# Maknee/minigpt4.cpp

Measured on AMD Instinct MI355X. Metric: decode tokens/sec, higher is better.
Workload: dtype i8; 1 GPU; MiniGPT4-13B f16 vision + Vicuna-13B Q5_K_M (wv/w2 Q6_K in 'more-bits' layers, output Q6_K), batch 1 per GPU, greedy decode through the C ABI; n_ctx=2048, context_at_mid_run=646, parallelism=dp1 (independent replicas)

## Files before the change

minigpt4.cpp_amd/csrc/attn_llm_body.hpp:

```cpp
    static_assert((FUSED || !BATCHED) && (BATCHED || !DRAFT), "BATCHED implies FUSED, DRAFT implies BATCHED");
    extern __shared__ __attribute__((aligned(16))) unsigned char smem[];
    constexpr int CH = HD / 8, P = AT_THREADS / CH, RM = DRAFT ? DRAFT_ROWS : 1;
    static_assert(!DRAFT || (RM <= P && RM * (HD / 2) <= AT_THREADS), "one prologue thread per (row, rotated pair); at most one LDS key per partition");
    const int h = blockIdx.x, t = blockIdx.y, tid = threadIdx.x;
    int pos_, p0_ = 0;
    if (BATCHED) {
        const int slot = row_slot[DRAFT ? 0 : t];
        p0_ = n_past[slot]; pos_ = DRAFT ? p0_ + t : p0_;
        if (DRAFT && pos_ >= n_ctx) return;
        kc += (size_t)slot * seq_stride; vc += (size_t)slot * seq_stride;
    } else pos_ = *n_past + t;
    const int pos = pos_, p0 = p0_, T = pos + 1;
    const int Tg = FUSED ? pos : T;
    const int Tpad = (T + 7) & ~7;
    float *sc = reinterpret_cast<float *>(smem);
    __half *ph = reinterpret_cast<__half *>(sc + Tpad);
    __half *qh = ph + Tpad;
    __half *knew = qh + HD, *vnew = knew + RM * HD;
    float *part = reinterpret_cast<float *>(vnew + RM * HD);
    __shared__ float s_red[AT_THREADS / 64];
    __shared__ double s_dred[AT_THREADS / 64];
    const float scale = 1.0f / sqrtf((float)HD);
    const size_t qo = (size_t)t * E + (size_t)h * HD;
    if (FUSED) {
        if (DRAFT) {
            if (tid < (t + 1) * (HD / 2)) {
                const int r = tid / (HD / 2), i = tid % (HD / 2), pr = p0 + r;
                const size_t ro = (size_t)r * E + (size_t)h * HD;
                const float c = cos_tab[(size_t)pr * (HD / 2) + i], s = sin_tab[(size_t)pr * (HD / 2) + i];
                const __half2 kr = rope_rot_h2(kin[ro + 2 * i], kin[ro + 2 * i + 1], c, s);
                const __half2 vr = __floats2half2_rn(vin[ro + 2 * i], vin[ro + 2 * i + 1]);
                st_h2(knew + r * HD + 2 * i, kr); st_h2(vnew + r * HD + 2 * i, vr);
                if (r == t) {
                    st_h2(qh + 2 * i, rope_rot_h2(q[qo + 2 * i], q[qo + 2 * i + 1], c, s));
                    const size_t co = (size_t)pos * E + (size_t)h * HD + 2 * i;
                    st_h2(kc + co, kr); st_h2(vc + co, vr);
                }
            }
        } else if (tid < HD / 2) {
            const int i = tid;
            const float c = cos_tab[(size_t)pos * (HD / 2) + i], s = sin_tab[(size_t)pos * (HD / 2) + i];
            const __half2 qr = rope_rot_h2(q[qo + 2 * i], q[qo + 2 * i + 1], c, s), kr = rope_rot_h2(kin[qo + 2 * i], kin[qo + 2 * i + 1], c, s);
            const __half2 vr = __floats2half2_rn(vin[qo + 2 * i], vin[qo + 2 * i + 1]);
            st_h2(qh + 2 * i, qr); st_h2(knew + 2 * i, kr); st_h2(vnew + 2 * i, vr);
            const size_t co = (size_t)pos * E + (size_t)h * HD + 2 * i;
            st_h2(kc + co, kr); st_h2(vc + co, vr);
        }
    } else {
        for (int i = tid; i < HD; i += AT_THREADS) qh[i] = f2h_rn(q[qo + i]);
    }
    __syncthreads();
    unsigned qreg[HD / 2];
#pragma unroll
    for (int i = 0; i < HD / 8; i++) { const int4 v4 = *reinterpret_cast<const int4 *>(qh + 8 * i); qreg[4 * i] = (unsigned)v4.x; qreg[4 * i + 1] = (unsigned)v4.y; qreg[4 * i + 2] = (unsigned)v4.z; qreg[4 * i + 3] = (unsigned)v4.w; }
    auto dot_row = [&](const __half *kr) {
        int4 kk[HD / 8];
#pragma unroll
        for (int i = 0; i < HD / 8; i++) kk[i] = ld16(kr + 8 * i);
        float s = 0.0f;
#pragma unroll
        for (int i = 0; i < HD / 8; i++) {
            const unsigned w[4] = {(unsigned)kk[i].x, (unsigned)kk[i].y, (unsigned)kk[i].z, (unsigned)kk[i].w};
#pragma unroll
            for (int e = 0; e < 4; e++) { s = fmaf(h2f_bits(w[e] & 0xFFFF), h2f_bits(qreg[4 * i + e] & 0xFFFF), s); s = fmaf(h2f_bits(w[e] >> 16), h2f_bits(qreg[4 * i + e] >> 16), s); }
        }
        return s * scale;
    };
    const int c = tid % CH, p = tid / CH;
    const __half *kb = kc + (size_t)h * HD + 8 * c, *vb = vc + (size_t)h * HD + 8 * c;
    constexpr int NPRE = 16;
    const int gmax = DRAFT ? max(p0 - 1, 0) : 0;
    int4 kpre[NPRE], vpre[NPRE];
#pragma unroll
    for (int i = 0; i < NPRE; i++) kpre[i] = ld16(kb + (size_t)min(p + i * P, DRAFT ? gmax : max(Tg - 1, 0)) * E);
#pragma unroll
    for (int i = 0; i < NPRE; i++) vpre[i] = ld16(vb + (size_t)min(p + i * P, DRAFT ? gmax : max(Tg - 1, 0)) * E);
    int jl = -1;
    int4 kl = make_int4(0, 0, 0, 0), vl = kl;
    if (DRAFT) {
        const int rl = (p - p0) & (P - 1);
        jl = rl < t ? p0 + rl : -1;
        kl = *reinterpret_cast<const int4 *>(knew + min(rl, RM - 1) * HD + 8 * c); vl = *reinterpret_cast<const int4 *>(vnew + min(rl, RM - 1) * HD + 8 * c);
    }
    float qd[8];
    unpack8(*reinterpret_cast<const int4 *>(qh + 8 * c), qd);
    float mx = -INFINITY;
#pragma unroll
    for (int i = 0; i < NPRE; i++) { const int j = p + i * P; const float s = dot16<CH>(DRAFT && j == jl ? kl : kpre[i], qd, scale); if (j < Tg) { if (c == 0) sc[j] = s; mx = fmaxf(mx, s); } }
    for (int j0 = p + NPRE * P; j0 < Tg; j0 += 8 * P) {
        int4 kk[8];
#pragma unroll
        for (int i = 0; i < 8; i++) kk[i] = ld16(kb + (size_t)min(j0 + i * P, DRAFT ? gmax : Tg - 1) * E);
#pragma unroll
        for (int i = 0; i < 8; i++) { const int j = j0 + i * P; const float s = dot16<CH>(DRAFT && j == jl ? kl : kk[i], qd, scale); if (j < Tg) { if (c == 0) sc[j] = s; mx = fmaxf(mx, s); } }
    }
    if (FUSED && tid == AT_THREADS - 1) { const float s = dot_row(knew + (DRAFT ? t : 0) * HD); sc[pos] = s; mx = fmaxf(mx, s); }
    mx = wave_max(mx);
    if ((tid & 63) == 0) s_red[tid >> 6] = mx;
    __syncthreads();
    mx = s_red[0];
#pragma unroll
    for (int i = 1; i < AT_THREADS / 64; i++) mx = fmaxf(mx, s_red[i]);
    double sum = 0.0;
    for (int j = tid; j < T; j += AT_THREADS) { const float v = exp_h(tb.exp, sc[j] - mx); sc[j] = v; sum += (double)v; }
    sum = wave_sum_d(sum);
    if ((tid & 63) == 0) s_dred[tid >> 6] = sum;
    __syncthreads();
    double tot = 0.0;
#pragma unroll
    for (int i = 0; i < AT_THREADS / 64; i++) tot += s_dred[i];
    const float inv = (float)(1.0 / tot);
    for (int j = tid; j < T; j += AT_THREADS) ph[j] = f2h_rn(sc[j] * inv);
    __syncthreads();
    float o[8] = {0, 0, 0, 0, 0, 0, 0, 0};
    auto pv_key = [&](const int4 &vv, const int j) { pv_acc(o, vv, __half2float(ph[j])); };
#pragma unroll
    for (int i = 0; i < NPRE; i++) { const int j = p + i * P; if (j < Tg) pv_key(DRAFT && j == jl ? vl : vpre[i], j); }
    for (int j0 = p + NPRE * P; j0 < Tg; j0 += 8 * P) {
        int4 vv[8];
#pragma unroll
        for (int i = 0; i < 8; i++) vv[i] = ld16(vb + (size_t)min(j0 + i * P, DRAFT ? gmax : Tg - 1) * E);
#pragma unroll
        for (int i = 0; i < 8; i++) { const int j = j0 + i * P; if (j < Tg) pv_key(DRAFT && j == jl ? vl : vv[i], j); }
    }
    if (FUSED && p == P - 1) {
        const float pj = __half2float(ph[pos]);
#pragma unroll
        for (int e = 0; e < 8; e++) o[e] = fmaf(__half2float(vnew[(DRAFT ? t : 0) * HD + 8 * c + e]), pj, o[e]);
    }
#pragma unroll
    for (int e = 0; e < 8; e++) part[p * HD + 8 * c + e] = o[e];
    __syncthreads();
    for (int i = tid; i < HD; i += AT_THREADS) { float s = 0.0f;
#pragma unroll 8
        for (int pp = 0; pp < P; pp++) s += part[pp * HD + i];
        out[qo + i] = s; }
```

minigpt4.cpp_amd/csrc/engine.cpp:

```cpp
#include "engine.hpp"
#include "dist.hpp"
#include "draft.hpp"
#include "quantize.hpp"
#include "imageio.hpp"

#include <algorithm>
#include <optional>
#include <unistd.h>
#include <chrono>
#include <thread>
#include <cmath>
#include <cstring>

namespace mg4 {

int device_count_noexcept() {
    int n = 0;
    if (hipGetDeviceCount(&n) != hipSuccess) { (void)hipGetLastError(); return 0; }
    return n;
}
void DeviceArena::alloc(size_t bytes) {
    release();
    if (virt) base = reinterpret_cast<uint8_t *>((uintptr_t)1 << 40);
    else { HIP_CHECK(hipMalloc((void **)&base, bytes)); HIP_CHECK(hipMemset(base, 0, bytes)); HIP_CHECK(hipDeviceSynchronize()); }
    cap = bytes; used = 0; layout_hash = 1469598103934665603ull;
}
void DeviceArena::release() { if (base && !virt) HIP_IGNORE(hipFree(base)); base = nullptr; cap = used = 0; }
uint8_t *DeviceArena::take(size_t bytes, size_t align) {
    const size_t off = (used + align - 1) / align * align;
    if (off + bytes > cap) throw HipError{hipErrorOutOfMemory, "arena overflow", __FILE__, __LINE__};
    used = off + bytes;
    for (uint64_t v : {(uint64_t)off, (uint64_t)bytes}) for (int i = 0; i < 8; i++) { layout_hash ^= (v >> (8 * i)) & 0xFF; layout_hash *= 1099511628211ull; }
    return base + off;
}
template <typename T> T *Engine::upload_raw(DeviceArena &a, const void *src, size_t bytes) {
    uint8_t *d = a.take(bytes);
    if (moves_data()) HIP_CHECK(hipMemcpy(d, src, bytes, hipMemcpyHostToDevice));
    return reinterpret_cast<T *>(d);
}

void preprocess_image_device(hipStream_t s, const uint8_t *rgb, int w, int h, float *out_chw) {
    constexpr int OUT = 224;
    const float mean[3] = {(float)0.48145466, (float)0.4578275, (float)0.40821073}, sd[3] = {(float)0.26862954, (float)0.26130258, (float)0.27577711};
    auto table = [&](int in, ResampleCoeffs &c) {
        if (in != OUT) { precompute_bicubic_8bpc(in, OUT, c); return; }
        c.in_size = c.out_size = OUT; c.ksize = 1; c.first.resize(OUT); c.count.assign(OUT, 1); c.kk.assign(OUT, 1 << 22);
        for (int i = 0; i < OUT; i++) c.first[(size_t)i] = i;
    };
    ResampleCoeffs ch, cv;
    table(w, ch); table(h, cv);
    struct Dev { void *p = nullptr; ~Dev() { if (p) HIP_IGNORE(hipFree(p)); } };
    Dev d_src, d_tmp, d_out, d_tab;
    const size_t src_bytes = (size_t)w * h * 3, tmp_bytes = (size_t)h * OUT * 3, out_bytes = (size_t)3 * OUT * OUT * 4;
    std::vector<int> tab;
    tab.insert(tab.end(), ch.first.begin(), ch.first.end()); tab.insert(tab.end(), ch.count.begin(), ch.count.end()); tab.insert(tab.end(), ch.kk.begin(), ch.kk.end());
    const size_t voff = tab.size();
    tab.insert(tab.end(), cv.first.begin(), cv.first.end()); tab.insert(tab.end(), cv.count.begin(), cv.count.end()); tab.insert(tab.end(), cv.kk.begin(), cv.kk.end());
    HIP_CHECK(hipMalloc(&d_src.p, src_bytes)); HIP_CHECK(hipMalloc(&d_tmp.p, tmp_bytes)); HIP_CHECK(hipMalloc(&d_out.p, out_bytes)); HIP_CHECK(hipMalloc(&d_tab.p, tab.size() * 4));
    HIP_CHECK(hipMemcpyAsync(d_src.p, rgb, src_bytes, hipMemcpyHostToDevice, s));
    HIP_CHECK(hipMemcpyAsync(d_tab.p, tab.data(), tab.size() * 4, hipMemcpyHostToDevice, s));
    const int *t = static_cast<const int *>(d_tab.p);
    launch_resample_h(static_cast<const uint8_t *>(d_src.p), w, h, t, t + OUT, t + 2 * OUT, ch.ksize, static_cast<uint8_t *>(d_tmp.p), OUT, s);
    launch_resample_v_norm(static_cast<const uint8_t *>(d_tmp.p), OUT, t + voff, t + voff + OUT, t + voff + 2 * OUT, cv.ksize, static_cast<float *>(d_out.p), OUT, mean, sd, s);
    HIP_CHECK(hipMemcpyAsync(out_chw, d_out.p, out_bytes, hipMemcpyDeviceToHost, s));
    HIP_CHECK(hipStreamSynchronize(s));
}

void Engine::release_buffers() {
    for (Conversation &c : conv_) { if (c.graph) HIP_IGNORE(hipGraphExecDestroy(c.graph)); c.graph = nullptr; }
    for (hipGraphExec_t &g : batch_graph_) { if (g) HIP_IGNORE(hipGraphExecDestroy(g)); g = nullptr; }
    spec_drop_graphs();
    if (h_argmax_) HIP_IGNORE(hipHostFree(h_argmax_));
    if (h_bstage_) HIP_IGNORE(hipHostFree(h_bstage_));
    if (h_logits_) HIP_IGNORE(hipHostFree(h_logits_));
    if (h_seg_) HIP_IGNORE(hipHostFree(h_seg_));
    h_argmax_ = nullptr; h_bstage_ = nullptr; h_logits_ = nullptr; h_seg_ = nullptr; logits_host_slot_ = -1;
    buf_arena_.release();
}
Engine::~Engine() {
    if (trace_file_) { fclose(trace_file_); trace_file_ = nullptr; }
    if (stream_hung_) {
        llm_arena_.abandon(); vis_arena_.abandon(); buf_arena_.abandon(); ri_arena_.abandon(); vgen_arena_.abandon();
        return;
    }
    if (stream_) HIP_IGNORE(hipStreamSynchronize(stream_));
    for (auto &e : site_events_) { HIP_IGNORE(hipEventDestroy(e.a)); HIP_IGNORE(hipEventDestroy(e.b)); }
    if (stage_) HIP_IGNORE(hipFree(stage_));
    prefix_free();
    score_free();
    topn_free();
    pen_free();
    spec_free();
    release_buffers();
    if (stream_) HIP_IGNORE(hipStreamDestroy(stream_));
}
void Engine::sync() { (void)flush(); HIP_CHECK(hipStreamSynchronize(stream_)); }

int Engine::init(const std::string &vision_path, const std::string &llm_path, int seed, int n_ctx, int n_batch) {
    const int ndev = device_count_noexcept();
    if (ndev <= 0) { set_last_error("no HIP device visible: the MI355X engine has no CPU fallback"); MG4_ERR("%s", last_error().c_str()); return E_LoadLanguageModel; }
    DistEnv dist; { std::string derr; if (parse_dist_env(dist, derr)) { set_last_error(derr); MG4_ERR("%s", derr.c_str()); return E_LoadLanguageModel; } }
    const char *dv = getenv("MINIGPT4_DEVICE");
    if (!dv) dv = getenv("LOCAL_RANK");
    device_ = dv ? atoi(dv) % ndev : (dist.active() && dist.world > 1 ? dist.rank % ndev : 0);
    if (!dv && dist.active() && dist.world > 1) MG4_INFO("no MINIGPT4_DEVICE / LOCAL_RANK: rank %d takes device %d", dist.rank, device_);
    HIP_CHECK(hipSetDevice(device_));
    hipDeviceProp_t prop;
    HIP_CHECK(hipGetDeviceProperties(&prop, device_));
    MG4_INFO("device %d: %s (%s), %d CUs, %.1f GiB", device_, prop.name, prop.gcnArchName, prop.multiProcessorCount, prop.totalGlobalMem / 1073741824.0);
    if (strncmp(prop.gcnArchName, "gfx950", 6) != 0) {
        set_last_error(std::string("device ") + prop.gcnArchName + " is not gfx950 (MI355X): this library carries gfx950 code objects only"); MG4_ERR("%s", last_error().c_str());
        return E_LoadLanguageModel;
    }
    HIP_CHECK(hipStreamCreateWithFlags(&stream_, hipStreamNonBlocking));
    n_ctx_ = n_ctx > 0 ? n_ctx : 2048;
    n_batch_ = n_batch > 0 ? n_batch : 512;
    max_rows_ = std::max(n_batch_, 32);
    use_graph_ = !(getenv("MINIGPT4_NO_GRAPH") && atoi(getenv("MINIGPT4_NO_GRAPH")));
    max_chunk_ = max_rows_;
    if (getenv("MINIGPT4_ATTN_PREFILL_W8")) set_attn_prefill_w8(atoi(getenv("MINIGPT4_ATTN_PREFILL_W8")));
    if (const char *dc = getenv("MINIGPT4_DEFER_COMBINE")) defer_combine_ = atoi(dc) != 0;
    if (const char *fp = getenv("MINIGPT4_F16_PAIR")) f16_pair_ = atoi(fp);
    batch_mix_ = !(getenv("MINIGPT4_BATCH_MIX") && atoi(getenv("MINIGPT4_BATCH_MIX")) == 0);
    if (const char *e = getenv("MINIGPT4_ATTN_SPLIT_T")) attn_split_t_ = atoi(e);
    n_cus_ = prop.multiProcessorCount;
    if (const char *e = getenv("MINIGPT4_MMQH")) set_mmqh(atoi(e));
    if (const char *e = getenv("MINIGPT4_COMPUTED_TABLES")) computed_tables_ = atoi(e) != 0;
    if (const char *e = getenv("MINIGPT4_RI_FUSE")) ri_fuse_ = atoi(e) != 0;
    if (const char *e = getenv("MINIGPT4_RI_W2")) ri_w2_ = atoi(e) != 0;
    if (const char *e = getenv("MINIGPT4_RI_WO")) ri_wo_ = atoi(e) != 0;
    if (const char *e = getenv("MINIGPT4_RI")) use_ri_ = atoi(e) != 0;
    set_ri_cus(prop.multiProcessorCount);
    if (const char *e = getenv("MINIGPT4_QF_FOLD")) qf_fold_ = atoi(e) != 0;
    if (const char *e = getenv("MINIGPT4_ATTN_QT")) set_attn_vit_qt(atoi(e));
    if (const char *e = getenv("MINIGPT4_SPLITK_XCD")) set_gemm_splitk_xcd(atoi(e));
    if (const char *e = getenv("MINIGPT4_SPLITK_PROJ")) splitk_proj_ = std::max(1, std::min(SPLITK_MAX, atoi(e)));
    if (const char *e = getenv("MINIGPT4_SPLITK_FC2")) splitk_fc2_ = std::max(1, std::min(SPLITK_MAX, atoi(e)));
    if (const char *e = getenv("MINIGPT4_FUSE")) fuse_mask_ = atoi(e);
    if (const char *e = getenv("MINIGPT4_F16_KS")) set_gemm_tuning(-1, atoi(e));
    if (const char *e = getenv("MINIGPT4_PAIR_SILU_COMPUTED")) pair_silu_computed_ = atoi(e) != 0;
    if (const char *e = getenv("MINIGPT4_COMPUTED_GELU")) computed_gelu_ = atoi(e) != 0;
    if (const char *e = getenv("MINIGPT4_QKV_HEAD_MAJOR")) qkv_head_major_ = atoi(e) != 0;
    if (const char *e = getenv("MINIGPT4_QF_SPLITK")) qf_splitk_ = atoi(e) != 0;
    if (const char *e = getenv("MINIGPT4_KV_HOIST")) kv_hoist_ = atoi(e) != 0;
    set_matvec_tuning(0, 0, prop.multiProcessorCount);
    if (const char *ns = getenv("MINIGPT4_CONVERSATIONS")) conv_.assign((size_t)std::max(1, std::min(MAX_CONVERSATIONS, atoi(ns))), Conversation{});
    sampler_.seed(seed);
    if (const char *tf = getenv("MINIGPT4_PARITY_TRACE")) { if (*tf) trace_file_ = fopen(tf, "wb"); }
    parity_ = trace_file_ || (getenv("MINIGPT4_PARITY") && atoi(getenv("MINIGPT4_PARITY")));
    pen_mode_ = getenv("MINIGPT4_PENALTIES") && atoi(getenv("MINIGPT4_PENALTIES"));
    if (const char *lm = getenv("MINIGPT4_LOAD")) load_mode_ = !strcmp(lm, "recv") ? LOAD_RECV : LOAD_FULL;
    if (dist.active()) load_mode_ = dist.rank != 0 ? LOAD_RECV : LOAD_FULL;
    int load_err = E_None;
    auto t0 = std::chrono::steady_clock::now();
    try {
        load_err = load_llm(llm_path);
        auto t1 = std::chrono::steady_clock::now();
        if (!load_err) MG4_INFO("LLM model init took %lld ms to complete", (long long)std::chrono::duration_cast<std::chrono::milliseconds>(t1 - t0).count());
        if (!load_err) load_err = load_vision(vision_path);
        auto t2 = std::chrono::steady_clock::now();
        if (!load_err) MG4_INFO("Loading minigpt4 model took %lld ms to complete", (long long)std::chrono::duration_cast<std::chrono::milliseconds>(t2 - t1).count());
        if (!load_err) { alloc_buffers(); if (load_mode_ == LOAD_FULL) { fold_qformer_constants(); if (conv_.size() > 1) build_ri_planes(); } }
    } catch (const HipError &e) {
        if (!dist.active()) throw;
        set_last_error(std::string("load failed: ") + e.what + " (" + hipGetErrorString(e.code) + ")"); load_err = E_LoadLanguageModel;
    }
    if (stage_) { HIP_IGNORE(hipFree(stage_)); stage_ = nullptr; stage_cap_ = 0; }
    if (dist.active()) { if (int e = native_broadcast(dist.world, dist.rank, dist.id_file, dist.timeout_s, load_err)) return load_err ? load_err : e; }
    return load_err;
}

int Engine::native_broadcast(int world, int rank, const std::string &id_file, int timeout_s, int local_err) {
    std::string err;
    auto fail = [&](const std::string &what) {
        if (rank == 0) unlink(id_file.c_str());
        set_last_error("weight broadcast (rank " + std::to_string(rank) + " of " + std::to_string(world) + "): " + what); MG4_ERR("%s", last_error().c_str()); return (int)E_LoadLanguageModel; };
    struct Holder { Rccl *r = new Rccl; ~Holder() { if (r && !r->poisoned()) delete r; } } holder;
    Rccl &rccl = *holder.r;
    if (rccl.open(err)) return fail(err);
    uint8_t id[128];
    if (rank == 0) { unlink(id_file.c_str()); if (rccl.unique_id(id, err) || publish_unique_id(id_file, id, err)) return fail(err); }
    else if (await_unique_id(id_file, id, timeout_s, err, process_start_epoch_s())) return fail(err);
    if (rccl.init(world, rank, id, timeout_s, err)) return fail(err);
    if (rank == 0) unlink(id_file.c_str());
    const auto t0 = std::chrono::steady_clock::now();
    auto wait_stream = [&](const char *what) -> bool {
        const auto w0 = std::chrono::steady_clock::now();
        for (;;) {
            const hipError_t q = hipStreamQuery(stream_);
            if (q == hipSuccess) return true;
            if (q != hipErrorNotReady) { (void)hipGetLastError(); err = std::string(what) + ": " + hipGetErrorString(q); return false; }
            if (std::chrono::steady_clock::now() - w0 > std::chrono::seconds(timeout_s)) {
                rccl.poison(); stream_hung_ = true;
                err = std::string(what) + " did not complete within " + std::to_string(timeout_s) + " s (a peer left the exchange?)"; return false;
            }
            std::this_thread::sleep_for(std::chrono::microseconds(200));
        }
    };
    struct Words { Rccl &r; unsigned long long *d = nullptr, *h = nullptr; ~Words() { if (r.poisoned()) return; if (d) HIP_IGNORE(hipFree(d)); if (h) HIP_IGNORE(hipHostFree(h)); } } words{rccl};
    HIP_CHECK(hipMalloc((void **)&words.d, 128));
    HIP_CHECK(hipHostMalloc((void **)&words.h, 256, hipHostMallocDefault));
    unsigned long long *const d_words = words.d;
    auto agree = [&](const unsigned long long mine[4], bool ok_here, const char *what) -> bool {
        unsigned long long *const v = words.h, *const r = words.h + 16;
        for (int i = 0; i < 4; i++) { v[i] = mine[i]; v[4 + i] = ~mine[i]; }
        v[8] = ok_here ? 0ull : 1ull;
        v[9] = ok_here ? 0ull : (unsigned long long)(rank + 1);
        HIP_CHECK(hipMemcpyAsync(d_words, v, 80, hipMemcpyHostToDevice, stream_));
        if (rccl.allreduce_max_u64(d_words, 10, stream_, err)) return false;
        HIP_CHECK(hipMemcpyAsync(r, d_words, 80, hipMemcpyDeviceToHost, stream_));
        if (!wait_stream(what)) return false;
        if (r[8]) { err = std::string("rank ") + std::to_string((long long)r[9] - 1) + " failed before \"" + what + "\"" + (ok_here ? "" : " (this rank: " + last_error() + ")"); return false; }
        for (int i = 0; i < 4; i++) if (r[i] != ~r[4 + i]) {
            char b[256]; snprintf(b, sizeof b, "%s differ between the ranks (word %d: max %llx, min %llx; this rank %llx)", what, i, r[i], ~r[4 + i], mine[i]); err = b; return false; }
        return true;
    };
    if (const char *st = getenv("MINIGPT4_DIST_TEST_STALL_MS")) launch_stall((unsigned)std::max(0, atoi(st)), stream_);
    const ArenaPlan pl = arena_plan();
    const unsigned long long plan_words[4] = {(unsigned long long)pl.llm_bytes, (unsigned long long)pl.vision_bytes, (unsigned long long)pl.llm_hash, (unsigned long long)pl.vision_hash};
    if (!agree(plan_words, local_err == 0, "arena layouts (sizes / layout hashes)")) return fail(err);
    if (rccl.broadcast(llm_arena_.base, llm_arena_.used, 0, stream_, err) || rccl.broadcast(vis_arena_.base, vis_arena_.used, 0, stream_, err)) return fail(err);
    if (!wait_stream("the arena broadcast")) return fail(err);
    dist_bcast_ms_ = std::chrono::duration<float, std::milli>(std::chrono::steady_clock::now() - t0).count();
    bool derived_ok = true;
    try { if (load_mode_ == LOAD_RECV) weights_received(); } catch (const HipError &e) { derived_ok = false; set_last_error(std::string("weights_received: ") + e.what); }
    unsigned long long sums[4] = {0ull, 0ull, 0ull, 0ull};
    if (derived_ok) { sums[0] = device_checksum(llm_arena_.base, llm_arena_.used, stream_); sums[1] = device_checksum(vis_arena_.base, vis_arena_.used, stream_); }
    if (!agree(sums, derived_ok, "arena contents (checksums) after the broadcast")) return fail(err);
    dist_world_ = world; dist_rank_ = rank;
    MG4_INFO("rank %d of %d: weight arenas %s in %.1f ms (%.2f GB, RCCL)", rank, world, rank ? "received" : "broadcast", dist_bcast_ms_, (llm_arena_.used + vis_arena_.used) / 1e9);
    return E_None;
}

int Engine::weights_received() {
    if (load_mode_ != LOAD_RECV) return 0;
    load_mode_ = LOAD_FULL;
    const size_t NQ = (size_t)v_nq_;
    for (size_t b = 0; b < (size_t)VISION_BATCH_MAX; b++) HIP_CHECK(hipMemcpy(vi_qtok_rep_ + b * NQ * 768, v_qtok_, NQ * 768 * 4, hipMemcpyDeviceToDevice));
    fold_qformer_constants();
    if (conv_.size() > 1) build_ri_planes();
    return 0;
}
int Engine::plan_arenas(const std::string &vision_path, const std::string &llm_path, ArenaPlan &out) {
    Engine e;
    e.load_mode_ = LOAD_PLAN;
    e.llm_arena_.virt = e.vis_arena_.virt = true;
    if (int err = e.load_llm(llm_path)) return err;
    if (int err = e.load_vision(vision_path)) return err;
    out = e.arena_plan();
    return 0;
}

static int effective_type(int t) { return t == GT_Q3_K ? GT_Q6_K : t; }
static bool tensor_type_loadable(int t) { return qweight_supported(effective_type(t)); }
static size_t effective_nbytes(const TensorMeta &t) { return t.type == GT_Q3_K ? t.nbytes / 110 * 210 : t.nbytes; }

void Engine::upload_qweight(const TensorMeta &t0, const uint8_t *file_base0, QWeight &w) {
    TensorMeta t = t0;
    const uint8_t *file_base = file_base0;
    std::vector<uint8_t> conv;
    if (t0.type == GT_Q3_K) {
        conv.resize(moves_data() ? effective_nbytes(t0) : 0);
        if (moves_data()) q3k_to_q6k(file_base0 + t0.offset, conv.data(), t0.nbytes / 110);
        t.type = GT_Q6_K; t.nbytes = effective_nbytes(t0); t.offset = 0; file_base = conv.data();
    }
    const int cols = (int)t.ne[0], rows = (int)t.ne[1];
    QWeight plan;
    const size_t need = plan_qweight(t.type, rows, cols, plan, nullptr);
    uint8_t *base = llm_arena_.take(need);
    plan_qweight(t.type, rows, cols, w, base);
    if (!moves_data()) return;
    if (t.type == GT_F16 || t.type == GT_F32) { HIP_CHECK(hipMemcpy(base, file_base + t.offset, t.nbytes, hipMemcpyHostToDevice)); return; }
    if (t.nbytes > stage_cap_) throw HipError{hipErrorOutOfMemory, "staging buffer too small", __FILE__, __LINE__};
    HIP_CHECK(hipMemcpy(stage_, file_base + t.offset, t.nbytes, hipMemcpyHostToDevice));
    launch_repack(stage_, w, stream_);
    HIP_CHECK(hipStreamSynchronize(stream_));
}

int Engine::load_llm(const std::string &path) {
    if (int e = llm_.load(path)) { MG4_ERR("failed to parse %s: %s", path.c_str(), last_error().c_str()); return e; }
    tok_.init(llm_);
    const int E = (int)llm_.n_embd, L = (int)llm_.n_layer, V = (int)llm_.n_vocab, F = (int)llm_.n_ff();
    const int hd = E / (int)llm_.n_head;
    if (!attn_head_size_supported(hd)) { set_last_error("unsupported head size (supported: 32, 64, 128)"); return E_LoadLanguageModel; }
    if (parity_) attn_ref_prepare();
    auto ctx_too_long = [&](const char *which, int lim) {
        set_last_error(std::string(which) + "n_ctx " + std::to_string(n_ctx_) + " exceeds what the attention kernel's LDS score rows hold (" + std::to_string(lim) + ")");
        MG4_ERR("%s", last_error().c_str());
        return (int)E_LoadLanguageModel;
    };
    if (parity_ && n_ctx_ > attn_ref_max_ctx(hd)) return ctx_too_long("MINIGPT4_PARITY (oracle-order kernel): ", attn_ref_max_ctx(hd));
    if (n_ctx_ > attn_max_ctx(hd)) return ctx_too_long("", attn_max_ctx(hd));
    MG4_INFO("llm: n_vocab %d n_embd %d n_head %u n_layer %d n_ff %d n_ctx %d", V, E, llm_.n_head, L, F, n_ctx_);
    auto need = [&](const std::string &name, int64_t ne0, int64_t ne1) -> const TensorMeta * {
        const TensorMeta *t = llm_.find(name);
        if (!t) { set_last_error("LLM file: missing tensor " + name); return nullptr; }
        if (t->ne[0] != ne0 || (ne1 ? (t->ne.size() != 2 || t->ne[1] != ne1) : t->ne.size() != 1)) { set_last_error("LLM file: bad shape for " + name); return nullptr; }
        if (ne1 == 0 && t->type != GT_F32) { set_last_error("LLM file: " + name + " must be f32"); return nullptr; }
        if (ne1 && !tensor_type_loadable(t->type)) { set_last_error(std::string("LLM file: tensor type ") + gt_name(t->type) + " of " + name + " is not supported by the gfx950 kernels"); return nullptr; }
        return t;
    };
    size_t total = 0, max_raw = 0;
    QWeight tmp;
    std::vector<std::pair<std::string, std::pair<int64_t, int64_t>>> mats;
    mats.push_back({"output.weight", {E, V}});
    for (int i = 0; i < L; i++) {
        const std::string p = "layers." + std::to_string(i) + ".";
        for (const char *w : {"attention.wq.weight", "attention.wk.weight", "attention.wv.weight", "attention.wo.weight"}) mats.push_back({p + w, {E, E}});
        mats.push_back({p + "feed_forward.w1.weight", {E, F}});
        mats.push_back({p + "feed_forward.w2.weight", {F, E}});
        mats.push_back({p + "feed_forward.w3.weight", {E, F}});
    }
    wbytes_token_ = 0;
    for (auto &m : mats) {
        const TensorMeta *t = need(m.first, m.second.first, m.second.second);
        if (!t) { MG4_ERR("%s", last_error().c_str()); return E_LoadLanguageModel; }
        total += plan_qweight(effective_type(t->type), (int)t->ne[1], (int)t->ne[0], tmp, nullptr) + 256;
        if (t->type != GT_F16 && t->type != GT_F32) max_raw = std::max(max_raw, effective_nbytes(*t));
        wbytes_token_ += effective_nbytes(*t);
    }
    const TensorMeta *tt = llm_.find("tok_embeddings.weight");
    if (!tt || tt->ne.size() != 2 || tt->ne[0] != E || tt->ne[1] != V || !tensor_type_loadable(tt->type)) { set_last_error("LLM file: bad tok_embeddings.weight"); MG4_ERR("%s", last_error().c_str()); return E_LoadLanguageModel; }
    total += effective_nbytes(*tt) + 256;
    wbytes_token_ += gt_nbytes(effective_type(tt->type), (size_t)E);
    for (int i = 0; i < L; i++) for (const char *n : {"attention_norm.weight", "ffn_norm.weight"}) if (!need("layers." + std::to_string(i) + "." + n, E, 0)) { MG4_ERR("%s", last_error().c_str()); return E_LoadLanguageModel; }
    if (!need("norm.weight", E, 0)) { MG4_ERR("%s", last_error().c_str()); return E_LoadLanguageModel; }
    total += (size_t)(2 * L + 1) * ((size_t)E * 4 + 256);
    wbytes_token_ += (size_t)(2 * L + 1) * E * 4;
    llm_arena_.alloc(total + 4096);
    if (max_raw && moves_data()) { HIP_CHECK(hipMalloc((void **)&stage_, max_raw)); stage_cap_ = max_raw; }
    const uint8_t *fb = llm_.mf.data;
    upload_qweight(*llm_.find("output.weight"), fb, output_);
    layers_.resize((size_t)L);
    for (int i = 0; i < L; i++) {
        const std::string p = "layers." + std::to_string(i) + ".";
        LayerW &lw = layers_[(size_t)i];
        upload_qweight(*llm_.find(p + "attention.wq.weight"), fb, lw.wq);
        upload_qweight(*llm_.find(p + "attention.wk.weight"), fb, lw.wk);
        upload_qweight(*llm_.find(p + "attention.wv.weight"), fb, lw.wv);
        upload_qweight(*llm_.find(p + "attention.wo.weight"), fb, lw.wo);
        upload_qweight(*llm_.find(p + "feed_forward.w1.weight"), fb, lw.w1);
        upload_qweight(*llm_.find(p + "feed_forward.w2.weight"), fb, lw.w2);
        upload_qweight(*llm_.find(p + "feed_forward.w3.weight"), fb, lw.w3);
        const TensorMeta *an = llm_.find(p + "attention_norm.weight"), *fn = llm_.find(p + "ffn_norm.weight");
        lw.attn_norm = upload_raw<float>(llm_arena_, fb + an->offset, an->nbytes);
        lw.ffn_norm = upload_raw<float>(llm_arena_, fb + fn->offset, fn->nbytes);
    }
    const TensorMeta *nt = llm_.find("norm.weight");
    norm_ = upload_raw<float>(llm_arena_, fb + nt->offset, nt->nbytes);
    if (tt->type == GT_Q3_K) {
        std::vector<uint8_t> conv(moves_data() ? effective_nbytes(*tt) : 0);
        if (moves_data()) q3k_to_q6k(fb + tt->offset, conv.data(), tt->nbytes / 110);
        tok_raw_ = upload_raw<uint8_t>(llm_arena_, conv.data(), effective_nbytes(*tt));
    } else tok_raw_ = upload_raw<uint8_t>(llm_arena_, fb + tt->offset, tt->nbytes);
    tok_type_ = effective_type(tt->type);
    MG4_INFO("llm weights: %.1f MB in HBM, %.3f GB streamed per decoded token", llm_arena_.used / 1048576.0, wbytes_token_ / 1e9);
    return E_None;
}

int Engine::load_vision(const std::string &path) {
    if (int e = vis_.load(path)) { MG4_ERR("failed to parse %s (%s)", path.c_str(), last_error().c_str()); return e; }
    auto fail = [&](const std::string &msg, int code) { set_last_error("vision file: " + msg); MG4_ERR("%s", last_error().c_str()); return code; };
    const TensorMeta *pos = vis_.find("visual_encoder", "pos_embed");
    if (!pos || pos->ne.size() != 2 || pos->type != GT_F32) return fail("missing/bad visual_encoder.pos_embed", E_LoadModelFileHeader);
    v_D_ = (int)pos->ne[0];
    if (pos->ne[1] != 257 || v_D_ % 88 || v_D_ % 16) return fail("pos_embed must be [D,257] with D a multiple of 88 and 16 (head size 88 is hard-coded in the reference, minigpt4.cpp:1271)", E_LoadModelFileHeader);
    v_heads_ = v_D_ / 88;
    if (vis_.config_int("encoder_width", v_D_) != v_D_) return fail("config Qformer.encoder_width disagrees with pos_embed", E_LoadModelFileHeader);
    v_depth_ = 0;
    while (vis_.find("visual_encoder", "blocks." + std::to_string(v_depth_) + ".norm1.weight")) v_depth_++;
    if (!v_depth_) return fail("no ViT blocks", E_LoadModelFileHeader);
    const TensorMeta *fc1 = vis_.find("visual_encoder", "blocks.0.mlp.fc1.weight");
    if (!fc1 || fc1->ne.size() != 2) return fail("missing blocks.0.mlp.fc1.weight", E_LoadModelFileHeader);
    v_M_ = (int)fc1->ne[1];
    const TensorMeta *qt = vis_.find("query_tokens", "weight");
    if (!qt || qt->ne.size() != 2 || qt->ne[0] != 768 || qt->type != GT_F32) return fail("bad query_tokens.weight", E_LoadModelFileHeader);
    v_nq_ = (int)qt->ne[1];
    if (vis_.config_int("query_length", v_nq_) != v_nq_) return fail("query_embeds_length != query_length", E_LoadModelFileHeader);
    {
        const long long ql = vis_.config_int("num_hidden_layers", 12);
        if (ql < 1 || ql > 64 || v_nq_ < 1 || v_nq_ > 256) return fail("num_hidden_layers / query_length out of range", E_LoadModelFileHeader);
        v_ql_ = (int)ql;
    }
    const TensorMeta *lp = vis_.find("llama_proj", "weight");
    if (!lp || lp->ne.size() != 2 || lp->ne[0] != 768) return fail("bad llama_proj.weight", E_LoadModelFileHeader);
    v_out_ = (int)lp->ne[1];
    const TensorMeta *iq = vis_.find("Qformer", "bert.encoder.layer.0.intermediate_query.dense.weight");
    if (!iq || iq->ne.size() != 2) return fail("missing intermediate_query", E_LoadModelFileHeader);
    v_qi_ = (int)iq->ne[1];
    if (v_M_ % 16 || v_qi_ % 16) return fail("MLP widths must be multiples of 16", E_LoadModelFileHeader);

    v_generic_ = false;
    for (auto &m : vis_.models) for (auto &t : m.second) {
        const TensorMeta &tm = t.second;
        const bool is_lin = tm.ne.size() == 2 && tm.name.size() >= 6 && tm.name.compare(tm.name.size() - 6, 6, "weight") == 0 && m.first != "query_tokens" && tm.name != "pos_embed" &&
                            tm.name.find("orm") == std::string::npos && tm.name != "patch_embed.proj.weight" && tm.name.find("embeddings") == std::string::npos;
        if (is_lin && tm.type != GT_F16) v_generic_ = true;
    }
    size_t total = 0;
    for (auto &m : vis_.models) for (auto &t : m.second) total += effective_nbytes(t.second) + 512 + (v_generic_ ? 2048 : 0);
    total += (size_t)v_D_ * 592 * 2 + (size_t)v_depth_ * 3 * v_D_ * 4 + (1 << 20);
    vis_arena_.alloc(total);
    const uint8_t *fb = vis_.mf.data;
    bool ok = true; std::string bad;
    auto f32v = [&](const std::string &model, const std::string &name, int64_t n) -> float * {
        const TensorMeta *t = vis_.find(model, name);
        if (!t || t->type != GT_F32 || t->nelements() != n) { ok = false; bad = model + "." + name; return nullptr; }
        return upload_raw<float>(vis_arena_, fb + t->offset, t->nbytes);
    };
    auto f16m = [&](const std::string &model, const std::string &name, int64_t n_in, int64_t n_out) -> const TensorMeta * {
        const TensorMeta *t = vis_.find(model, name);
        if (!t || t->ne.size() < 2 || t->nelements() != n_in * n_out) { ok = false; bad = model + "." + name; return nullptr; }
        if (t->type != GT_F16 && !v_generic_) { ok = false; bad = model + "." + name + " (unexpected type " + gt_name(t->type) + ")"; return nullptr; }
        return t;
    };
    auto up16 = [&](const TensorMeta *t) -> __half * { return t && !v_generic_ ? upload_raw<__half>(vis_arena_, fb + t->offset, t->nbytes) : nullptr; };
    auto concat16 = [&](const std::vector<const TensorMeta *> &ts) -> __half * {
        if (v_generic_) return nullptr;
        size_t bytes = 0; for (auto t : ts) { if (!t) return nullptr; bytes += t->nbytes; }
        uint8_t *d = vis_arena_.take(bytes); size_t off = 0;
        for (auto t : ts) { if (moves_data()) HIP_CHECK(hipMemcpy(d + off, fb + t->offset, t->nbytes, hipMemcpyHostToDevice)); off += t->nbytes; }
        return reinterpret_cast<__half *>(d);
    };
    auto concat32 = [&](const std::vector<std::pair<const char *, std::string>> &names, int64_t each) -> float * {
        uint8_t *d = vis_arena_.take((size_t)each * 4 * names.size()); size_t off = 0;
        for (auto &nm : names) { const TensorMeta *t = vis_.find(nm.first, nm.second);
            if (!t || t->type != GT_F32 || t->nelements() != each) { ok = false; bad = nm.second; return nullptr; }
            if (moves_data()) HIP_CHECK(hipMemcpy(d + off, fb + t->offset, t->nbytes, hipMemcpyHostToDevice)); off += t->nbytes; }
        return reinterpret_cast<float *>(d);
    };
    const int D = v_D_, M = v_M_;
    const char *VE = "visual_encoder";
    v_cls_ = f32v(VE, "cls_token", D);
    v_pos_ = f32v(VE, "pos_embed", (int64_t)D * 257);
    v_patch_b_ = f32v(VE, "patch_embed.proj.bias", D);
    const TensorMeta *pw = f16m(VE, "patch_embed.proj.weight", 588, D);
    if (pw && pw->type != GT_F16) { ok = false; bad = "visual_encoder.patch_embed.proj.weight (the conv kernel is always F16: convert.py:113-117, and minigpt4_quantize_model skips it)"; pw = nullptr; }
// ... 255 lines not shown
            const QWeight *Wp[1] = {W[i]}; float *Yp[1] = {y[i]}; const float *Rp[1] = {res ? res[i] : nullptr};
            if (!(N == 1 && use_v2_ && launch_matvec_set(Wp, Yp, Rp, 1, act_, s))) launch_mul_mat(*W[i], act_, N, y[i], ldy, res ? res[i] : nullptr, s);
        }
    }
    if (kept.ks > 1) {
        SlabSrc m = kept; m.mixed = true; m.n = 3;
        m.y[2] = y[0]; m.res[2] = res ? res[0] : nullptr;
        if (pend_.ks > 1) { m.mbase[2] = pend_.mbase[0]; m.mks[2] = pend_.mks[0]; } else { m.mbase[2] = y[0]; m.mks[2] = 1; }
        pend_ = m;
    }
    return silu_pair;
}
void Engine::mul_mat(const QWeight &W, int N, float *y, int ldy, const float *residual, hipStream_t s, const Prep *prep, bool fuse, const char *site, bool defer_ok, bool keep_pending) {
    const QWeight *Wp[1] = {&W}; float *Yp[1] = {y}; const float *Rp[1] = {residual};
    mul_mat_set(Wp, Yp, Rp, 1, N, ldy, s, prep, fuse, false, site, defer_ok, keep_pending);
}

bool Engine::mixed_qkv(const LayerW &L, hipStream_t s, bool fuse) {
    if (!use_v2_) return false;
    const int E = (int)llm_.n_embd;
    const QWeight *W1[2] = {&L.wq, &L.wk}, *W2[1] = {&L.wv}; float *Y1[2] = {q_, k_}, *Y2[1] = {v_};
    if (act_mask_for(L.wq.type) != ACT_Q8K || act_mask_for(L.wv.type) != ACT_Q8K) return false;
    SiteScope sc(this, "qkv", (double)(L.wq.bytes + L.wk.bytes + L.wv.bytes), s);
    if (fuse && matvec_prologue_supported(L.wq.type, E)) { if (launch_matvec_mixed(W1, Y1, 2, W2, Y2, 1, act_, s, 1, x_, L.attn_norm)) return true; }
    launch_rms_quant(x_, L.attn_norm, 1, E, act_, ACT_Q8K, s);
    if (launch_matvec_mixed(W1, Y1, 2, W2, Y2, 1, act_, s)) return true;
    const bool keep = prof_on_; prof_on_ = false;
    mul_mat_set(W1, Y1, nullptr, 2, 1, E, s, nullptr, false); mul_mat(L.wv, 1, v_, E, nullptr, s, nullptr, false);
    prof_on_ = keep;
    return true;
}

void Engine::forward_ref(const Pass &p, hipStream_t s) {
    if (p.seg) throw HipError{hipErrorInvalidValue, "forward_ref: a packed chunk reached the parity pass (parity mode evaluates one conversation per pass)", __FILE__, __LINE__};
    const int N = p.N;
    const int E = (int)llm_.n_embd, F = (int)llm_.n_ff(), H = (int)llm_.n_head, hd = E / H, V = (int)llm_.n_vocab;
    const size_t C = (size_t)n_ctx_, sl = (size_t)cur_;
    int *const d_npast = d_npast_ + sl, *const d_argmax = d_argmax_ + sl, *const d_feed = d_feed_ + sl;
    float *const logits = logits_ + sl * (size_t)V;
    launch_get_rows(tok_type_, tok_raw_, E, p.feed ? d_feed : d_tokens_, N, x_, s);
    auto tr = [&](const char *what, int il, const float *p, size_t n) {
        if (!trace_file_) return;
        hipStreamCaptureStatus st = hipStreamCaptureStatusNone; HIP_IGNORE(hipStreamIsCapturing(s, &st));
        if (st != hipStreamCaptureStatusNone) return;
        std::vector<float> h(n);
        HIP_CHECK(hipMemcpyAsync(h.data(), p, n * 4, hipMemcpyDeviceToHost, s)); HIP_CHECK(hipStreamSynchronize(s));
        char name[32]; memset(name, 0, sizeof name); snprintf(name, sizeof name, "%s.%d", what, il);
        const long long cnt = (long long)n;
        fwrite(name, 1, 32, trace_file_); fwrite(&cnt, 8, 1, trace_file_); fwrite(h.data(), 4, n, trace_file_); fflush(trace_file_);
    };
    tr("embd", -1, x_, (size_t)N * E);
    const int t_max = n_ctx_;
    auto ref_set = [&](std::initializer_list<const QWeight *> Ws, std::initializer_list<float *> Ys, const float *res) {
        const WeightSet m(Ws, Ys, res);
        for (int done = 0, run; done < m.n; done += run) {
            run = same_run(m.W, m.n, done);
            const float *const *R = res ? m.R + done : nullptr;
            const bool ok = N == 1 ? launch_mul_mat_ref_set(m.W + done, m.Y + done, R, run, act_, s)
                                   : N >= 5 && launch_mmq2_set(m.W + done, m.Y + done, R, run, act_, N, m.W[done]->rows, s, nullptr, 1);
            if (!ok) for (int i = 0; i < run; i++) launch_mul_mat_ref(*m.W[done + i], act_, N, m.Y[done + i], m.W[done + i]->rows, res, s);
        }
    };
    const bool fused_row = N == 1 && !trace_file_;
    auto fused_set = [&](std::initializer_list<const QWeight *> Ws, std::initializer_list<float *> Ys, const float *res, int pro, const float *px, const float *pw) -> bool {
        if (!fused_row) return false;
        WeightSet m(Ws, Ys, res);
        if (pro != 0 && !matvec_prologue_supported(m.W[0]->type, m.W[0]->cols)) return false;
        if (same_shape(m.W, m.n)) return launch_matvec_set(m.W, m.Y, res ? m.R : nullptr, m.n, act_, s, pro, px, pw, &tabs_, MATVEC_EPI_REF);
        if (m.n == 3 && !res && same_shape(m.W, 2) && m.W[2]->cols == m.W[0]->cols && (pro == 0 || pro == 1))
            return launch_matvec_mixed(m.W, m.Y, 2, m.W + 2, m.Y + 2, 1, act_, s, pro, px, pw, MATVEC_EPI_REF);
        return false;
    };
    for (size_t il = 0; il < layers_.size(); il++) {
        const LayerW &L = layers_[il];
        __half *kc = kc_ + (sl * layers_.size() + il) * C * E, *vc = vc_ + (sl * layers_.size() + il) * C * E;
        if (!fused_set({&L.wq, &L.wk, &L.wv}, {q_, k_, v_}, nullptr, 1, x_, L.attn_norm)) {
            launch_rms_quant(x_, L.attn_norm, N, E, act_, act_mask_for(L.wq.type) | act_mask_for(L.wk.type) | act_mask_for(L.wv.type), s, true);
            ref_set({&L.wq, &L.wk, &L.wv}, {q_, k_, v_}, nullptr);
        }
        tr("q", (int)il, q_, (size_t)N * E); tr("k", (int)il, k_, (size_t)N * E); tr("v", (int)il, v_, (size_t)N * E);
        if (N == 1 && !trace_file_) launch_attn_ref_fused(q_, k_, v_, kc, vc, H, hd, d_npast, t_max, cos_, sin_, tabs_, att_, s);
        else { launch_rope_kv(q_, k_, v_, N, H, hd, d_npast, cos_, sin_, kc, vc, s); launch_attn_ref(q_, kc, vc, N, H, hd, d_npast, t_max, tabs_, att_, s); }
        tr("q_rope", (int)il, q_, (size_t)N * E); tr("att", (int)il, att_, (size_t)N * E);
        if (!fused_set({&L.wo}, {x_}, x_, 2, att_, nullptr)) {
            launch_silu_mul_quant(att_, nullptr, N, E, act_, act_mask_for(L.wo.type), tabs_, s);
            ref_set({&L.wo}, {x_}, x_);
        }
        tr("x_attn", (int)il, x_, (size_t)N * E);
        if (!fused_set({&L.w1, &L.w3}, {h1_, h3_}, nullptr, 1, x_, L.ffn_norm)) {
            launch_rms_quant(x_, L.ffn_norm, N, E, act_, act_mask_for(L.w1.type) | act_mask_for(L.w3.type), s, true);
            ref_set({&L.w1, &L.w3}, {h1_, h3_}, nullptr);
        }
        tr("h1", (int)il, h1_, (size_t)N * F); tr("h3", (int)il, h3_, (size_t)N * F);
        launch_silu_mul_quant(h1_, h3_, N, F, act_, act_mask_for(L.w2.type), tabs_, s);
        if (!fused_set({&L.w2}, {x_}, x_, 0, nullptr, nullptr)) ref_set({&L.w2}, {x_}, x_);
        tr("x_ffn", (int)il, x_, (size_t)N * E);
    }
    if (p.score) score_rows(*p.score, s);
    if (!(N == 1 && fused_set({&output_}, {logits}, nullptr, 1, x_, norm_))) {
        launch_rms_quant(x_ + (size_t)(N - 1) * E, norm_, 1, E, act_, act_mask_for(output_.type), s, true);
        const QWeight *Wo[1] = {&output_}; float *Yo[1] = {logits};
        if (!launch_mul_mat_ref_set(Wo, Yo, nullptr, 1, act_, s)) launch_mul_mat_ref(output_, act_, 1, logits, V, nullptr, s);
    }
    launch_argmax(logits, V, d_argmax, d_scratch_, s);
    launch_advance(d_npast, N, d_feed, d_argmax, s);
    HIP_CHECK(hipMemcpyAsync(h_argmax_ + sl, d_argmax, 4, hipMemcpyDeviceToHost, s));
}
void Engine::set_parity(bool on) {
    if (on == parity_) return;
    if (on && llm_.n_head > 0) {
        const int hd = (int)(llm_.n_embd / llm_.n_head), lim = attn_ref_max_ctx(hd);
        if (n_ctx_ > lim) throw HipError{hipErrorInvalidValue, "parity mode: n_ctx exceeds what the oracle-order attention kernel's LDS rows hold (attn_ref_max_ctx)", __FILE__, __LINE__};
        attn_ref_prepare();
    }
    HIP_CHECK(hipStreamSynchronize(stream_));
    for (Conversation &c : conv_) { if (c.graph) HIP_IGNORE(hipGraphExecDestroy(c.graph)); c.graph = nullptr; }
    for (hipGraphExec_t &g : batch_graph_) { if (g) HIP_IGNORE(hipGraphExecDestroy(g)); g = nullptr; }
    spec_drop_graphs();
    parity_ = on;
    prefix_empty();
}

void Engine::forward(const Pass &p, hipStream_t s) {
    pend_ = SlabSrc{}; xh_override_ = nullptr;
    if (parity_) { forward_ref(p, s); return; }
    const int N = p.N;
    const int E = (int)llm_.n_embd, F = (int)llm_.n_ff(), H = (int)llm_.n_head, hd = E / H, V = (int)llm_.n_vocab;
    const size_t C = (size_t)n_ctx_, sl = (size_t)cur_;
    int *const d_npast = d_npast_ + sl, *const d_argmax = d_argmax_ + sl, *const d_feed = d_feed_ + sl;
    float *const logits = logits_ + sl * (size_t)V;
    const SegChunk *const sg = p.seg;
    const size_t seq_stride = layers_.size() * C * (size_t)E;
    const bool dec = N == 1 && !sg;
    { SiteScope sc(this, "embed", (double)gt_nbytes(tok_type_, (size_t)E) * N, s); launch_get_rows(tok_type_, tok_raw_, E, p.feed ? d_feed : d_tokens_, N, x_, s); }
    auto fz = [&](int bit) { return dec && (fuse_mask_ >> bit & 1); };
    for (size_t il = 0; il < layers_.size(); il++) {
        const LayerW &L = layers_[il];
        const size_t sl_c = sg ? 0 : sl;
        __half *kc = kc_ + (sl_c * layers_.size() + il) * C * E, *vc = vc_ + (sl_c * layers_.size() + il) * C * E;
        const Prep p_attn{1, x_, L.attn_norm}, p_att{2, att_, nullptr}, p_ffn{1, x_, L.ffn_norm}, p_silu{3, h1_, h3_};
        {
            const QWeight *W3[3] = {&L.wq, &L.wk, &L.wv}; float *Y3[3] = {q_, k_, v_};
            if (L.wv.type == L.wq.type) mul_mat_set(W3, Y3, nullptr, 3, N, E, s, &p_attn, fz(0), false, "qkv", !dec);
            else if (fz(6) && L.wk.type == L.wq.type && mixed_qkv(L, s, fz(0))) {}
            else if (act_mask_for(L.wv.type) == act_mask_for(L.wq.type) && !fz(0)) {
                prep_rms(x_, L.attn_norm, N, E, act_mask_for(L.wq.type), s);
                mul_mat_set(W3, Y3, nullptr, 2, N, E, s, nullptr, false, false, "qk", !dec); mul_mat(L.wv, N, v_, E, nullptr, s, nullptr, false, "v", !dec, !dec);
            } else { mul_mat_set(W3, Y3, nullptr, 2, N, E, s, &p_attn, fz(0), false, "qk"); mul_mat(L.wv, N, v_, E, nullptr, s, &p_attn, fz(0), "v"); }
        }
        bool att_in_xh = false;
        std::optional<SiteScope> att_sc;
        if (prof_on_) att_sc.emplace(this, "attention", 4.0 * (double)E * (sg ? sg->key_rows : (double)(conv_[sl].n_committed + N)), s);
        if (dec && p.split) launch_attn_llm_split(q_, k_, v_, kc, vc, H, hd, d_npast, n_ctx_, cos_, sin_, tabs_dec_, att_, attn_ws_, attn_splits_, s);
        else if (dec) launch_attn_llm(q_, k_, v_, kc, vc, 1, H, hd, d_npast, n_ctx_, cos_, sin_, tabs_dec_, att_, true, s);
        else {
            if (pend_.ks > 1 && pend_.n == 3 && pend_.y[0] == q_ && pend_.y[1] == k_ && pend_.y[2] == v_ && !pend_.res[0] && !pend_.res[1] && !pend_.res[2] && pend_.stride == (long long)N * E) {
                if (sg) launch_rope_kv_seg_slabs(pend_, N, H, hd, sg->rows, seq_stride, cos_, sin_, kc, vc, s);
                else launch_rope_kv_slabs(pend_, N, H, hd, d_npast, cos_, sin_, kc, vc, s);
                pend_ = SlabSrc{};
            } else {
                flush_pending(s);
                if (sg) launch_rope_kv_seg(q_, k_, v_, N, H, hd, sg->rows, seq_stride, cos_, sin_, kc, vc, s);
                else launch_rope_kv(q_, k_, v_, N, H, hd, d_npast, cos_, sin_, kc, vc, s);
            }
            const bool want_h = (f16_pair_ & 4) && L.wo.type == GT_F16 && N >= 512 && act_.xh && E % 128 == 0;
            if (sg) attn_segments(*sg, kc, vc, want_h, &att_in_xh, s);
            else if (!(attn_prefill_ && launch_attn_prefill(q_, kc, vc, N, H, hd, d_npast, conv_[sl].n_committed + N, tabs_, att_, s, want_h ? act_.xh : nullptr, &att_in_xh)))
                launch_attn_llm(q_, k_, v_, kc, vc, N, H, hd, d_npast, n_ctx_, cos_, sin_, tabs_, att_, false, s);
        }
        att_sc.reset();
        mul_mat(L.wo, N, x_, E, x_, s, att_in_xh ? nullptr : &p_att, fz(1), "wo", !dec);
        bool paired = false;
        bool pair16 = false;
        if (!dec && (f16_pair_ & 1) && N >= 512 && L.w1.type == GT_F16 && L.w3.type == GT_F16 && L.w1.rows == L.w3.rows && L.w1.cols == L.w3.cols && act_.xh &&
            L.w2.type == GT_F16 && E % 128 == 0 && F % 64 == 0) {
            prep_rms(x_, L.ffn_norm, N, E, act_mask_for(GT_F16), s);
            SiteScope sc(this, "w1w3", (double)(L.w1.bytes + L.w3.bytes), s);
            pair16 = launch_gemm_f16_silu_pair(act_.xh, E, reinterpret_cast<const __half *>(L.w1.qs), reinterpret_cast<const __half *>(L.w3.qs), N, F, E, pair_silu_computed_ ? tabs_dec_ : tabs_, nullptr,
                                               reinterpret_cast<__half *>(h1_), F, n_cus_, s);
        }
        if (pair16) {
            xh_override_ = reinterpret_cast<const __half *>(h1_);
            mul_mat(L.w2, N, x_, E, x_, s, nullptr, false, "w2", true);
            continue;
        }
        if (L.w1.type == L.w3.type) { const QWeight *W2[2] = {&L.w1, &L.w3}; float *Y2[2] = {h1_, h3_}; paired = mul_mat_set(W2, Y2, nullptr, 2, N, F, s, &p_ffn, fz(2), fz(5), "w1w3", !dec); }
        else if (act_mask_for(L.w1.type) == act_mask_for(L.w3.type) && !fz(2)) {
            prep_rms(x_, L.ffn_norm, N, E, act_mask_for(L.w1.type), s);
            mul_mat(L.w1, N, h1_, F, nullptr, s, nullptr, false, "w1"); mul_mat(L.w3, N, h3_, F, nullptr, s, nullptr, false, "w3");
        } else { mul_mat(L.w1, N, h1_, F, nullptr, s, &p_ffn, fz(2), "w1"); mul_mat(L.w3, N, h3_, F, nullptr, s, &p_ffn, fz(2), "w3"); }
        const Prep p_h{2, h1_, nullptr};
        mul_mat(L.w2, N, x_, E, x_, s, paired ? &p_h : &p_silu, fz(3), "w2", !dec);
    }
    flush_pending(s);
    if (p.score) score_rows(*p.score, s);
    if (sg) {
        if (sg->n_end > 0) {
            launch_gather_rows(x_, sg->last, sg->n_end, E, att_, s);
            const Prep p_last{1, att_, norm_};
            mul_mat(output_, sg->n_end, blogits_, V, nullptr, s, &p_last, false, "output");
            SiteScope sc(this, "finish", (double)V * 4 * sg->n_end, s);
            launch_seg_finish(blogits_, V, sg->n_end, sg->fin, d_npast_, d_argmax_, d_feed_, logits_, s);
        }
        return;
    }
    const Prep p_out{1, x_ + (size_t)(N - 1) * E, norm_};
    mul_mat(output_, 1, logits, V, nullptr, s, &p_out, fz(4), "output");
    { SiteScope sc(this, "argmax", (double)V * 4, s); launch_argmax(logits, V, d_argmax, d_scratch_, s); }
    { SiteScope sc(this, "advance", 0.0, s); launch_advance(d_npast, N, d_feed, d_argmax, s); }
    HIP_CHECK(hipMemcpyAsync(h_argmax_ + sl, d_argmax, 4, hipMemcpyDeviceToHost, s));
}

void Engine::forward_batch(int B, hipStream_t s, bool verify) {
    pend_ = SlabSrc{}; xh_override_ = nullptr;
    batch_path_ = BatchPath{}; batch_path_.rows = B;
    const int E = (int)llm_.n_embd, F = (int)llm_.n_ff(), H = (int)llm_.n_head, hd = E / H, V = (int)llm_.n_vocab;
    const size_t C = (size_t)n_ctx_, seq_stride = layers_.size() * C * (size_t)E;
    auto ri_serves = [&](std::initializer_list<const QWeight *> Ws) {
        if (!ri_ready_ || B < 3 || B > 4) return false;
        const QWeight *w0 = *Ws.begin();
        if (!same_shape(Ws.begin(), (int)Ws.size())) return false;
        int groups = 0;
        for (const QWeight *w : Ws) { if (!ri_of(w)) return false; groups += w->rows / 64; }
        if (ri_w2_ && B == 4 && Ws.size() == 1 && w0->cols >= 8192 && ri_ksplit(groups, w0->cols, ri_ws_) > 1) return true;
        return groups >= 128;
    };
    auto mm = [&](std::initializer_list<const QWeight *> Ws, std::initializer_list<float *> ys, const float *res0, int ld, const float *px = nullptr, const float *pw = nullptr) {
        WeightSet m(Ws, ys, res0);
        const int n = m.n;
        const QWeight *const *W = m.W; float *const *y = m.Y; const float *const *r = m.R;
        const bool same = same_shape(W, n);
        if (ri_wo_ && px && !pw && n == 1 && ri_ready_ && B >= 3 && B <= 4 && ri_of(W[0])) {
            const RiPlanes *rp[1] = {ri_of(W[0])};
            if (launch_matvec_ri(W, rp, y, res0 ? r : nullptr, 1, act_, B, ld, s, px, nullptr, W[0]->cols, RiWorkspace{})) { batch_path_.ri++; batch_path_.ri_plain++; return; }
        }
        if (ri_serves(Ws) && (!px || pw)) {
            const RiPlanes *rp[3]; for (int k = 0; k < n; k++) rp[k] = ri_of(W[k]);
            if (launch_matvec_ri(W, rp, y, res0 ? r : nullptr, n, act_, B, ld, s, px, pw, W[0]->cols, ri_ws_)) {
                batch_path_.ri++; if (ri_ksplit(n * (W[0]->rows / 64), W[0]->cols, ri_ws_) > 1) batch_path_.ri_ksplit++;
                return;
            }
        }
        if (same && B <= batch_rows_max_) {
            bool ok = true;
            for (int t0 = 0; t0 < B && ok; t0 += 4) {
                const int K = W[0]->cols;
                ActQ A = act_;
                A.q8k += (size_t)t0 * K; A.dk += (size_t)t0 * (K / 256); A.bsk += (size_t)t0 * (K / 16); A.bsq += (size_t)t0 * (K / 16); A.q80 += (size_t)t0 * K;
                A.d0 += (size_t)t0 * (K / 32); A.d1 += (size_t)t0 * (K / 32); A.s1 += (size_t)t0 * (K / 32); A.sum0 += (size_t)t0 * (K / 32);
                float *yo[3]; const float *ro[3];
                for (int k = 0; k < n; k++) { yo[k] = y[k] + (size_t)t0 * ld; ro[k] = r[k] ? r[k] + (size_t)t0 * ld : nullptr; }
                ok = launch_matvec_rows(W, yo, res0 ? ro : nullptr, n, A, std::min(4, B - t0), ld, s, px ? px + (size_t)t0 * K : nullptr, pw, K);
                if (!ok && t0) throw HipError{hipErrorInvalidValue, "multi-row mat-vec refused a pass it had accepted", __FILE__, __LINE__};
            }
            if (ok) { batch_path_.dot4++; return; }
        }
        if (px) {
            const int K = W[0]->cols; int mask = 0;
            for (int k = 0; k < n; k++) mask |= act_mask_for(W[k]->type);
            if (pw) launch_rms_quant(px, pw, B, K, act_, mask, s); else launch_silu_mul_quant(px, nullptr, B, K, act_, mask, tabs_, s);
        }
        for (int k = 0; k < n; k++) { launch_mul_mat(*W[k], act_, B, y[k], ld, r[k], s); batch_path_.mul_mat++; }
    };
    auto rows_pro = [&](std::initializer_list<const QWeight *> Ws, bool plain = false) {
        if (ri_serves(Ws)) return !plain && ri_fuse_;
        if (batch_fuse_ == 0 || B > batch_rows_max_ || B > 4 || (batch_fuse_ < 0 && B > 2 && !plain)) return false;
        const QWeight *w0 = *Ws.begin();
        return same_shape(Ws.begin(), (int)Ws.size()) && matvec_rows_prologue_ok(w0->type, w0->cols);
    };
    auto attn = [&](__half *kc, __half *vc) {
        if (verify) launch_attn_llm_draft(q_, k_, v_, kc, vc, B, H, hd, d_npast_, d_bslot_, seq_stride, n_ctx_, cos_, sin_, tabs_dec_, att_, s);
        else launch_attn_llm_batched(q_, k_, v_, kc, vc, B, H, hd, d_npast_, d_bslot_, seq_stride, n_ctx_, cos_, sin_, tabs_dec_, att_, s);
    };
    float *const row_logits = verify ? spec_logits_ : blogits_;
    launch_get_rows(tok_type_, tok_raw_, E, d_btok_, B, x_, s);
    for (size_t il = 0; il < layers_.size(); il++) {
        const LayerW &L = layers_[il];
        __half *kc = kc_ + il * C * E, *vc = vc_ + il * C * E;
        auto qkv_mixed = [&](bool pro) {
            if (!batch_mix_ || B > batch_rows_max_ || B > 4 || L.wk.type != L.wq.type || L.wv.type == L.wq.type) return false;
            const QWeight *W1[2] = {&L.wq, &L.wk}, *W2[1] = {&L.wv};
            float *y1[2] = {q_, k_}, *y2[1] = {v_};
            if (!pro && ri_ready_ && B >= 3 && ri_of(&L.wq) && ri_of(&L.wk) && ri_of(&L.wv) && (L.wq.rows + L.wk.rows + L.wv.rows) / 64 >= 128) {
                const RiPlanes *r1[2] = {ri_of(&L.wq), ri_of(&L.wk)}, *r2[1] = {ri_of(&L.wv)};
                if (launch_matvec_ri_mixed(W1, r1, y1, 2, W2, r2, y2, 1, act_, B, E, s)) { batch_path_.ri_mix++; return true; }
            }
            const bool ok = launch_matvec_rows_mixed(W1, y1, 2, W2, y2, 1, act_, B, E, s, pro ? x_ : nullptr, pro ? L.attn_norm : nullptr, E);
            if (ok) batch_path_.dot4_mix++;
            return ok;
        };
        if (B > batch_rows_max_ && batch_sets_) {
            batch_path_.sets++;
            const Prep p_attn{1, x_, L.attn_norm}, p_att{2, att_, nullptr}, p_ffn{1, x_, L.ffn_norm}, p_silu{3, h1_, h3_};
            const QWeight *W3[3] = {&L.wq, &L.wk, &L.wv}; float *Y3[3] = {q_, k_, v_};
            if (L.wv.type == L.wq.type && L.wk.type == L.wq.type) mul_mat_set(W3, Y3, nullptr, 3, B, E, s, &p_attn, false, false, "qkv");
            else {
                prep_rms(x_, L.attn_norm, B, E, act_mask_for(L.wq.type) | act_mask_for(L.wk.type) | act_mask_for(L.wv.type), s);
                if (L.wk.type == L.wq.type) { mul_mat_set(W3, Y3, nullptr, 2, B, E, s, nullptr, false, false, "qk"); mul_mat(L.wv, B, v_, E, nullptr, s, nullptr, false, "v"); }
                else { mul_mat(L.wq, B, q_, E, nullptr, s, nullptr, false, "q"); mul_mat(L.wk, B, k_, E, nullptr, s, nullptr, false, "k"); mul_mat(L.wv, B, v_, E, nullptr, s, nullptr, false, "v"); }
            }
            flush_pending(s);
            attn(kc, vc);
            mul_mat(L.wo, B, x_, E, x_, s, &p_att, false, "wo", true);
            if (L.w1.type == L.w3.type) { const QWeight *W2[2] = {&L.w1, &L.w3}; float *Y2[2] = {h1_, h3_}; mul_mat_set(W2, Y2, nullptr, 2, B, F, s, &p_ffn, false, false, "w1w3", true); }
            else { prep_rms(x_, L.ffn_norm, B, E, act_mask_for(L.w1.type) | act_mask_for(L.w3.type), s); mul_mat(L.w1, B, h1_, F, nullptr, s, nullptr, false, "w1"); mul_mat(L.w3, B, h3_, F, nullptr, s, nullptr, false, "w3"); }
            mul_mat(L.w2, B, x_, E, x_, s, &p_silu, false, "w2", true);
            continue;
        }
        if (L.wv.type == L.wq.type && L.wk.type == L.wq.type && rows_pro({&L.wq, &L.wk, &L.wv})) mm({&L.wq, &L.wk, &L.wv}, {q_, k_, v_}, nullptr, E, x_, L.attn_norm);
        else if (L.wk.type == L.wq.type && rows_pro({&L.wq, &L.wk}) && rows_pro({&L.wv})) {
            if (!qkv_mixed(true)) { mm({&L.wq, &L.wk}, {q_, k_}, nullptr, E, x_, L.attn_norm); mm({&L.wv}, {v_}, nullptr, E, x_, L.attn_norm); }
        } else {
            launch_rms_quant(x_, L.attn_norm, B, E, act_, act_mask_for(L.wq.type) | act_mask_for(L.wk.type) | act_mask_for(L.wv.type), s);
            if (L.wv.type == L.wq.type && L.wk.type == L.wq.type) mm({&L.wq, &L.wk, &L.wv}, {q_, k_, v_}, nullptr, E);
            else if (qkv_mixed(false)) {}
            else if (L.wk.type == L.wq.type) { mm({&L.wq, &L.wk}, {q_, k_}, nullptr, E); mm({&L.wv}, {v_}, nullptr, E); }
            else { mm({&L.wq}, {q_}, nullptr, E); mm({&L.wk}, {k_}, nullptr, E); mm({&L.wv}, {v_}, nullptr, E); }
        }
        attn(kc, vc);
        if (rows_pro({&L.wo}, true)) mm({&L.wo}, {x_}, x_, E, att_, nullptr);
        else { launch_silu_mul_quant(att_, nullptr, B, E, act_, act_mask_for(L.wo.type), tabs_, s); mm({&L.wo}, {x_}, x_, E); }
        if (L.w1.type == L.w3.type && rows_pro({&L.w1, &L.w3})) mm({&L.w1, &L.w3}, {h1_, h3_}, nullptr, F, x_, L.ffn_norm);
        else {
            launch_rms_quant(x_, L.ffn_norm, B, E, act_, act_mask_for(L.w1.type) | act_mask_for(L.w3.type), s);
            if (L.w1.type == L.w3.type) mm({&L.w1, &L.w3}, {h1_, h3_}, nullptr, F);
            else { mm({&L.w1}, {h1_}, nullptr, F); mm({&L.w3}, {h3_}, nullptr, F); }
        }
        launch_silu_mul_quant(h1_, h3_, B, F, act_, act_mask_for(L.w2.type), tabs_dec_, s);
        mm({&L.w2}, {x_}, x_, E);
    }
    if (B <= batch_rows_max_ && ri_fuse_ && ri_serves({&output_})) mm({&output_}, {row_logits}, nullptr, V, x_, norm_);
    else {
        prep_rms(x_, norm_, B, E, act_mask_for(output_.type), s);
        mm({&output_}, {row_logits}, nullptr, V);
    }
    if (verify) launch_draft_finish(spec_logits_, V, B, d_btok_, d_bslot_, d_npast_, d_argmax_, d_feed_, logits_, spec_res_, s);
    else launch_batch_finish(blogits_, V, B, d_bslot_, d_npast_, d_argmax_, d_feed_, logits_, s);
}

template <class F> void Engine::capture_graph(hipGraphExec_t &out, F &&enqueue) {
    hipGraph_t g = nullptr;
    HIP_CHECK(hipStreamBeginCapture(stream_, hipStreamCaptureModeThreadLocal));
    try { enqueue(); }
    catch (...) { HIP_IGNORE(hipStreamEndCapture(stream_, &g)); if (g) HIP_IGNORE(hipGraphDestroy(g)); out = nullptr; throw; }
    HIP_CHECK(hipStreamEndCapture(stream_, &g));
    HIP_CHECK(hipGraphInstantiate(&out, g, nullptr, nullptr, 0));
    HIP_CHECK(hipGraphDestroy(g));
}
size_t Engine::upload_embd_runs(const int *tok, int m, const float *embd, float *x_dst) {
    const size_t E = llm_.n_embd;
    size_t er = 0;
    for (int i = 0; i < m;) {
        if (tok[i] >= 0) { i++; continue; }
        int j = i; while (j < m && tok[j] < 0) j++;
        HIP_CHECK(hipMemcpyAsync(x_dst + (size_t)i * E, embd + er * E, (size_t)(j - i) * E * 4, hipMemcpyHostToDevice, stream_));
        er += (size_t)(j - i); i = j;
    }
    return er;
}

bool Engine::weights_missing() const {
    if (load_mode_ != LOAD_RECV) return false;
    set_last_error("the context was loaded in receive mode (MINIGPT4_LOAD=recv) and its weight arenas have not been filled: broadcast them, then call minigpt4_amd_weights_received");
    MG4_ERR("%s", last_error().c_str());
    return true;
}
int Engine::eval_chunk(const int *row_tok, int N, const float *embd, const ScoreReq *score) {
    if (N <= 0) return 0;
    if (weights_missing()) return 1;
    Conversation &cv = conv_[(size_t)cur_];
    if (logits_host_slot_ == cur_) logits_host_slot_ = -1;
    launch_set_int(d_npast_ + cur_, cv.n_committed, stream_);
    if (N == 1 && row_tok[0] >= 0) {
        launch_set_int(d_feed_ + cur_, row_tok[0], stream_);
        const Pass p = decode_pass(cv, score);
        if (use_graph_ && !prof_on_ && !trace_file_ && !score) {
            if (cv.graph && cv.graph_split != p.split) { HIP_IGNORE(hipGraphExecDestroy(cv.graph)); cv.graph = nullptr; }
            cv.graph_split = p.split;
            if (!cv.graph) capture_graph(cv.graph, [&] { forward(p, stream_); });
            HIP_CHECK(hipGraphLaunch(cv.graph, stream_));
        } else {
            forward(p, stream_);
        }
    } else {
        HIP_CHECK(hipMemcpyAsync(d_tokens_, row_tok, (size_t)N * 4, hipMemcpyHostToDevice, stream_));
        upload_embd_runs(row_tok, N, embd, x_);
        HIP_CHECK(hipStreamSynchronize(stream_));
        Pass p{N}; p.score = score;
        forward(p, stream_);
    }
    cv.n_committed += N; cv.has_logits = true;
    cv.hist.insert(cv.hist.end(), row_tok, row_tok + N);
    return 0;
}

int Engine::flush() {
    Conversation &cv = conv_[(size_t)cur_];
    if (cv.pend_tok.empty()) return 0;
    const int E = (int)llm_.n_embd;
    const PrefixPlan plan = prefix_lookup(&cur_, 1);
    size_t er = 0;
    for (size_t i = (size_t)plan.m[0]; i < cv.pend_tok.size(); i += (size_t)max_chunk_) {
        const int n = (int)std::min((size_t)max_chunk_, cv.pend_tok.size() - i);
        size_t ne = 0; for (int k = 0; k < n; k++) ne += cv.pend_tok[i + k] < 0;
        const int rc = eval_chunk(cv.pend_tok.data() + i, n, cv.pend_embd.data() + er * E);
        er += ne;
        if (rc) { cv.drop_queue(); return rc; }
    }
    cv.pend_tok.clear(); cv.pend_embd.clear();
    prefix_commit(plan);
    return 0;
}

int Engine::set_prefix_cache(int max_rows) {
    if (max_rows < 0) { set_last_error("set_prefix_cache: max_rows < 0"); return 1; }
    max_rows = std::min(max_rows, n_ctx_);
    HIP_CHECK(hipStreamSynchronize(stream_));
    prefix_empty(); pfx_ = PrefixInfo{};
    if (max_rows == pfx_max_) return 0;
    prefix_free();
    if (max_rows == 0) return 0;
    const size_t bytes = layers_.size() * (size_t)max_rows * llm_.n_embd * sizeof(__half);
    HIP_CHECK(hipMalloc((void **)&pfx_k_, bytes));
    if (hipError_t e = hipMalloc((void **)&pfx_v_, bytes); e != hipSuccess) { HIP_IGNORE(hipFree(pfx_k_)); pfx_k_ = nullptr; HIP_CHECK(e); }
    pfx_max_ = max_rows;
// ... 1010 lines not shown
```

minigpt4.cpp_amd/csrc/engine.hpp:

```cpp
#pragma once
#include <memory>
#include <string>
#include <vector>

#include "common.hpp"
#include "formats.hpp"
#include "kernels.hpp"
#include "sampler.hpp"

namespace mg4 {

struct DeviceArena {
    uint8_t *base = nullptr;
    size_t cap = 0, used = 0;
    bool virt = false;
    uint64_t layout_hash = 1469598103934665603ull;
    void alloc(size_t bytes);
    void release();
    uint8_t *take(size_t bytes, size_t align = 256);
    void abandon() { base = nullptr; cap = used = 0; }
    ~DeviceArena() { release(); }
};


// ... 69 lines not shown

    static constexpr int DRAFT_MAX = DRAFT_ROWS - 1;
    int set_speculation(int max_draft);
    int verify_draft(const int *draft, int n_draft, int *ids_out, int *n_out, int *row_greedy, int *n_sent = nullptr);
    int decode_lookup(const int *corpus, int n_corpus, int max_tokens, int ngram_max, int ngram_min, int n_draft, int *tokens_out, int *n_tokens, int *stats);

    void set_penalties(bool on) { pen_mode_ = on; }
    bool penalties() const { return pen_mode_; }
    int set_conversation_penalties(int slot, const PenParams &p);
    int set_logit_bias(const int *ids, const float *bias, int n);
    int token_history(int *out, int cap);
    struct PenInfo { int mode = 0, launches = 0, host_rows = 0, last_entries = 0; };
    PenInfo penalty_info() const { PenInfo i = pen_info_; i.mode = pen_mode_; return i; }

    int decode_loop(int steps, int *tokens_out, float *ms_total);
    int profile_sites(int steps, std::string &json);
    float last_encode_ms() const { return last_encode_ms_; }
    void set_parity(bool on);
    bool parity() const { return parity_; }

private:
    int load_llm(const std::string &path);
    int load_vision(const std::string &path);
    void alloc_buffers();
    void forward_batch(int B, hipStream_t s, bool verify = false);
    int spec_max_ = 0; float *spec_logits_ = nullptr; int *spec_res_ = nullptr, *spec_hres_ = nullptr; std::vector<hipGraphExec_t> spec_graph_;
    bool pen_mode_ = false; PenInfo pen_info_;
    uint8_t *pen_d_ = nullptr, *pen_h_ = nullptr; int *pen_out_d_ = nullptr, *pen_out_h_ = nullptr;
    std::vector<float> pen_row_;
    void pen_alloc();
    void pen_free();
    struct Conversation;
    int pen_table(const Conversation &cv, std::vector<PenEntry> &tab) const;
    void pen_pick(const int *slots, int n, int *ids);
    int greedy_raw();
    void spec_drop_graphs();
    void spec_free();
    struct SegChunk {
        int n_seg = 0, n_end = 0;
        int h_segs[4 * MAX_CONVERSATIONS];
        AttnSegs att;
        const int *rows = nullptr, *fin = nullptr, *last = nullptr;
        double key_rows = 0;
    };
    struct ScoreReq { const int *targets = nullptr; float *logprob = nullptr; int *greedy = nullptr; float *greedy_logprob = nullptr; int first = 0, end = 0; float *h_logits = nullptr;
                      int top_n = 0; };
    struct Pass { int N; bool feed = false; bool split = false; const SegChunk *seg = nullptr; const ScoreReq *score = nullptr; };
    void forward(const Pass &p, hipStream_t s);
    void forward_ref(const Pass &p, hipStream_t s);
    int eval_chunk(const int *row_tok, int N, const float *embd, const ScoreReq *score = nullptr);
    ScoreReq score_request(const std::vector<int> &targets, int top_n, float *h_logits);
    size_t upload_embd_runs(const int *tok, int m, const float *embd, float *x_dst);
    template <class F> void capture_graph(hipGraphExec_t &out, F &&enqueue);
    struct SelectScope { Engine *e; int keep; explicit SelectScope(Engine *e_) : e(e_), keep(e_->cur_) {} ~SelectScope() { e->cur_ = keep; } };
    int check_slots(const int *slots, int n) const;
    void drop_queues(const int *slots, int n) { for (int i = 0; i < n; i++) conv_[(size_t)slots[i]].drop_queue(); }
    float *score_buf_ = nullptr, *score_lp_ = nullptr, *score_glp_ = nullptr; int *score_tgt_ = nullptr, *score_greedy_ = nullptr; int score_cap_ = 0;
    void score_alloc();
    void score_free();
    void score_rows(const ScoreReq &rq, hipStream_t s);
    void score_entry0(int slot, int idx, int target, float *logprob, int *greedy, float *greedy_logprob, float *logits_out, const TopOut *top = nullptr);
    int score_tokens_impl(const char *name, const int *tokens, int n, float *logprob, int *greedy, float *greedy_logprob, float *logits_out, const TopOut *top);
    int *topn_d_ = nullptr, *topn_h_ = nullptr, *topn_in_ = nullptr, *topn_hin_ = nullptr; int topn_cap_ = 0; hipEvent_t topn_ev_ = nullptr;
    int topn_map_[MAX_CONVERSATIONS], topn_m_ = 0;
    int *topn_ids() const { return topn_d_; }
    float *topn_lp() const { return reinterpret_cast<float *>(topn_d_ + (size_t)topn_cap_ * TOPN_MAX); }
    int *topn_rank() const { return topn_d_ + 2 * (size_t)topn_cap_ * TOPN_MAX; }
    float *topn_tlp() const { return reinterpret_cast<float *>(topn_rank() + topn_cap_); }
    void topn_alloc();
    void topn_free();
    void topn_slots_launch(const int *slots, int n, int top_n, const int *targets);
    void topn_slots_collect(int n, int top_n, int *top_ids, float *top_lp, float *logprob, int *rank);
    struct ScoreOut { int off[MAX_CONVERSATIONS]; float *logprob; int *greedy; float *greedy_logprob; };
    int prefill_packed(const int *slots, int n, const ScoreOut *so = nullptr);
    void attn_segments(const SegChunk &sg, __half *kc, __half *vc, bool want_h, bool *att_in_xh, hipStream_t s);
    static constexpr int SEG_FIN = 4 * MAX_CONVERSATIONS, SEG_LAST = SEG_FIN + 2 * MAX_CONVERSATIONS, SEG_ROWS = SEG_LAST + MAX_CONVERSATIONS;
    size_t seg_ints() const { return (size_t)SEG_ROWS + 2 * (size_t)max_rows_ + 4 * ((size_t)max_rows_ + MAX_CONVERSATIONS); }
    int *d_seg_ = nullptr, *h_seg_ = nullptr;
    struct Prep { int kind; const float *x; const float *w; };
    void mul_mat(const QWeight &W, int N, float *y, int ldy, const float *residual, hipStream_t s, const Prep *prep, bool fuse, const char *site = "matmul", bool defer_ok = false, bool keep_pending = false);
    bool mul_mat_set(const QWeight *const *W, float *const *y, const float *const *res, int n, int N, int ldy, hipStream_t s, const Prep *prep, bool fuse, bool silu_pair = false, const char *site = "matmul", bool defer_ok = false, bool keep_pending = false);
    SlabSrc pend_; bool defer_combine_ = true;
    const __half *xh_override_ = nullptr; int f16_pair_ = 7;
    bool batch_sets_ = true;
    void flush_pending(hipStream_t s);
    void prep_rms(const float *x, const float *w, int N, int K, int mask, hipStream_t s);
    void upload_qweight(const TensorMeta &t, const uint8_t *file_base, QWeight &w);
    template <typename T> T *upload_raw(DeviceArena &a, const void *src, size_t bytes);


    int native_broadcast(int world, int rank, const std::string &id_file, int timeout_s, int local_err = 0);
    int dist_world_ = 1, dist_rank_ = 0; float dist_bcast_ms_ = 0.0f;
    LoadMode load_mode_ = LOAD_FULL;
    bool moves_data() const { return load_mode_ == LOAD_FULL; }
    bool weights_missing() const;
    int device_ = 0;
    hipStream_t stream_ = nullptr;
    int n_ctx_ = 2048, n_batch_ = 512, max_rows_ = 512;
    struct Conversation {
        int n_past = 0;
        int n_committed = 0;
        std::vector<int> pend_tok; std::vector<float> pend_embd;
        hipGraphExec_t graph = nullptr;
        bool graph_split = false;
        std::vector<int> hist;
        PenParams pen; std::vector<int> bias_id; std::vector<float> bias_val;
        bool has_logits = false;
        void drop_queue() { pend_tok.clear(); pend_embd.clear(); n_past = n_committed; }
    };
    std::vector<Conversation> conv_ = std::vector<Conversation>(1);
    Pass decode_pass(const Conversation &cv, const ScoreReq *score = nullptr) const { Pass p{1, true, attn_split_t_ > 0 && cv.n_committed + 1 > attn_split_t_}; p.score = score; return p; }
    int cur_ = 0;
    int shift_keep_ = -1;
    __half *pfx_k_ = nullptr, *pfx_v_ = nullptr; int pfx_max_ = 0; std::vector<int> pfx_ids_; PrefixInfo pfx_;
    void prefix_empty() { pfx_ids_.clear(); }
    void prefix_free();
    static int token_run(const Conversation &cv) { int r = 0; while (r < (int)cv.pend_tok.size() && cv.pend_tok[(size_t)r] >= 0) r++; return r; }
    struct PrefixPlan { int m[MAX_CONVERSATIONS] = {0}, hit[MAX_CONVERSATIONS], n_hit = 0, rows = 0, reused = 0; bool looked = false; int cap_slot = -1; std::vector<int> cap_ids; };
    PrefixPlan prefix_lookup(const int *slots, int n);
    void prefix_commit(const PrefixPlan &plan);
    void prefix_copy_in(const int *slots, int n, int n_rows);
    void prefix_capture(int slot, const std::vector<int> &ids);
    bool shift_allows(int n) const { return shift_keep_ >= 0 && n <= n_ctx_ - shift_keep_; }
    int make_room(int n);
    bool defer_ = true; int max_chunk_ = 512;
    void release_buffers();

    LLMFile llm_;
    Tokenizer tok_;
    Sampler sampler_;
    struct LayerW { float *attn_norm = nullptr, *ffn_norm = nullptr; QWeight wq, wk, wv, wo, w1, w2, w3; };
    bool mixed_qkv(const LayerW &L, hipStream_t s, bool fuse);
    std::vector<LayerW> layers_;
    float *norm_ = nullptr;
    QWeight output_;
    uint8_t *tok_raw_ = nullptr; int tok_type_ = -1;
    DeviceArena llm_arena_, vis_arena_, buf_arena_;
    bool stream_hung_ = false;
    uint8_t *stage_ = nullptr; size_t stage_cap_ = 0;
    size_t wbytes_token_ = 0;
    __half *kc_ = nullptr, *vc_ = nullptr;
    float *cos_ = nullptr, *sin_ = nullptr;
    Tables tabs_;
    Tables tabs_dec_, tabs_vis_;
    float *x_ = nullptr, *q_ = nullptr, *k_ = nullptr, *v_ = nullptr, *att_ = nullptr, *h1_ = nullptr, *h3_ = nullptr, *logits_ = nullptr;
    ActQ act_;
    int *d_npast_ = nullptr, *d_argmax_ = nullptr, *d_feed_ = nullptr;
    int *d_tokens_ = nullptr; void *d_scratch_ = nullptr;
    int *d_btok_ = nullptr, *d_bslot_ = nullptr, *d_bpos_ = nullptr; float *blogits_ = nullptr;
    std::vector<hipGraphExec_t> batch_graph_;
    int *h_argmax_ = nullptr, *h_bstage_ = nullptr; float *h_logits_ = nullptr; int logits_host_slot_ = -1;
    bool use_graph_ = true, use_v2_ = true, attn_prefill_ = true, parity_ = false;
    FILE *trace_file_ = nullptr;
    void *attn_ws_ = nullptr; int attn_splits_ = 6; int attn_split_t_ = 768; int attn_splits_forced_ = 0;
    int batch_rows_max_ = 4; int batch_fuse_ = -1; int n_cus_ = 256;
    bool computed_tables_ = true;
    bool pair_silu_computed_ = true;
    bool computed_gelu_ = true;
    bool ri_w2_ = true;
    bool ri_wo_ = false;
    bool use_ri_ = true, ri_ready_ = false, ri_fuse_ = false;
    DeviceArena ri_arena_;
    BatchPath batch_path_;
    RiWorkspace ri_ws_;
    std::vector<std::pair<const QWeight *, RiPlanes>> ri_map_;
    const RiPlanes *ri_of(const QWeight *w) const { for (const auto &e : ri_map_) if (e.first == w) return &e.second; return nullptr; }
    void build_ri_planes();
    bool batch_mix_ = true;
    static constexpr int FUSE_DEFAULT = 87; int fuse_mask_ = FUSE_DEFAULT;
    bool prof_on_ = false;
    struct SiteEv { hipEvent_t a, b; const char *site; std::string kernel; double bytes; size_t p0 = 0, p1 = 0; };
    std::vector<SiteEv> site_events_;
    void site_begin(const char *site, double bytes, hipStream_t s);
    void site_end(hipStream_t s) noexcept;
    struct SiteScope { Engine *e; hipStream_t s; SiteScope(Engine *e_, const char *site, double bytes, hipStream_t s_) : e(e_), s(s_) { e->site_begin(site, bytes, s); } ~SiteScope() { e->site_end(s); } };

    VisionFile vis_;
    int v_D_ = 0, v_depth_ = 0, v_M_ = 0, v_heads_ = 0, v_ql_ = 0, v_qi_ = 0, v_nq_ = 32, v_out_ = 0;
    struct VBlock { float *n1w, *n1b, *n2w, *n2b, *qkv_b, *proj_b, *fc1_b, *fc2_b; __half *qkv_w, *proj_w, *fc1_w, *fc2_w; };
    struct QAtt { __half *q_w = nullptr, *kv_w = nullptr, *dense_w = nullptr; float *q_b = nullptr, *kv_b = nullptr, *dense_b = nullptr, *ln_w = nullptr, *ln_b = nullptr; };
    struct QLayer { QAtt self, cross; bool has_cross = false; int cross_idx = -1; __half *inter_w, *out_w; float *inter_b, *out_b, *oln_w, *oln_b; };
    std::vector<VBlock> vblocks_;
    std::vector<QLayer> qlayers_;
    float *v_cls_ = nullptr, *v_pos_ = nullptr, *v_patch_b_ = nullptr, *v_lnv_w_ = nullptr, *v_lnv_b_ = nullptr, *v_qtok_ = nullptr, *v_qeln_w_ = nullptr, *v_qeln_b_ = nullptr, *v_proj_b_ = nullptr;
    __half *v_patch_w_ = nullptr, *v_proj_w_ = nullptr;
    static constexpr int SPLITK_MAX = 12; int splitk_proj_ = 1, splitk_fc2_ = 4;
    float *vi_slab_ = nullptr, *vi_qtok_rep_ = nullptr;
    float *vi_img_ = nullptr, *vi_pe_ = nullptr, *vi_x_ = nullptr, *vi_qkv_ = nullptr, *vi_hs_ = nullptr, *vi_a1_ = nullptr, *vi_a2_ = nullptr, *vi_d_ = nullptr, *vi_qq_ = nullptr, *vi_kv_ = nullptr, *vi_out_ = nullptr;
    __half *vi_patches_ = nullptr, *vi_ln_h_ = nullptr, *vi_att_h_ = nullptr, *vi_mlp_h_ = nullptr, *vi_img_h_ = nullptr, *vi_hs_h_ = nullptr, *vi_a1_h_ = nullptr, *vi_a2_h_ = nullptr, *vi_ctx_h_ = nullptr, *vi_im_h_ = nullptr;
    float last_encode_ms_ = 0;
    bool qf_skinny_ = true;
    __half *v_kv_all_w_ = nullptr; float *v_kv_all_b_ = nullptr; int v_ncross_ = 0;
    float *vi_c_a1_ = nullptr, *vi_c_qq_ = nullptr; __half *vi_c_a1_h_ = nullptr;
    bool qf_fold_ = true, qf_folded_ = false, kv_hoist_ = true;
    void fold_qformer_constants();
    bool qf_splitk_ = true;
    bool qkv_head_major_ = true;
    void qf_dense_ln(const __half *A, int lda, const __half *W, int K, const float *bias, const float *residual, const float *ln_w, const float *ln_b, float *out, __half *out_h,
                     int rows, hipStream_t s);

    bool v_generic_ = false;
    struct GLin { QWeight w; };
    struct GBlock { GLin qkv, proj, fc1, fc2; };
    struct GAtt { GLin q, k, v, dense; };
    struct GQLayer { GAtt self, cross; GLin inter, out; };
    std::vector<GBlock> gblocks_; std::vector<GQLayer> gql_; GLin gproj_;
    DeviceArena vgen_arena_;
    ActQ vact_;
    float *vg_ln_ = nullptr, *vg_att_ = nullptr, *vg_mlp_ = nullptr, *vg_img_ = nullptr, *vg_tmp_ = nullptr, *vg_ctx_ = nullptr, *vg_im_ = nullptr;
    int load_vision_generic();
    void alloc_vision_generic();
    int encode_images_generic(const float *const *chw, int B, float *const *out);
    int encode_images_ref(const float *const *chw, int B, float *const *out);
    void build_vision_views();
    void glinear(const GLin &L, const float *x, int rows, const float *bias, bool gelu, const float *residual, float *out, hipStream_t s);
};

int device_count_noexcept();

void preprocess_image_device(hipStream_t s, const uint8_t *rgb, int w, int h, float *out_chw);

}
```

minigpt4.cpp_amd/csrc/kernels.hpp:

```cpp
#pragma once
#include <vector>

#include "common.hpp"
#include "penalty.hpp"

namespace mg4 {

struct Tables {
    const __half *gelu = nullptr, *silu = nullptr, *exp = nullptr;
    int exp_neg_n = 0;
};

size_t plan_qweight(int type, int rows, int cols, QWeight &w, uint8_t *base);
void launch_repack(const uint8_t *raw, const QWeight &w, hipStream_t s);
bool qweight_supported(int type);

void launch_rms_quant(const float *x, const float *w, int N, int K, const ActQ &A, int mask, hipStream_t s, bool sequential_sum = false);
void launch_silu_mul_quant(const float *a, const float *b, int N, int K, const ActQ &A, int mask, const Tables &tb, hipStream_t s);

void launch_mul_mat(const QWeight &W, const ActQ &A, int N, float *y, int ldy, const float *residual, hipStream_t s);

void launch_mul_mat_ref(const QWeight &W, const ActQ &A, int N, float *y, int ldy, const float *residual, hipStream_t s);
bool launch_mul_mat_ref_set(const QWeight *const *W, float *const *y, const float *const *res, int n, const ActQ &A, hipStream_t s);
bool matvec_prologue_supported(int type, int cols);
void set_mmq_enabled(int v);
int mmq_enabled();
bool mmq2_supported(int type, int rows, int cols);
struct SlabSrc { const float *ws = nullptr; int ks = 0; long long stride = 0; int n = 0; float *y[3] = {nullptr, nullptr, nullptr}; const float *res[3] = {nullptr, nullptr, nullptr};
                 const float *mbase[3] = {nullptr, nullptr, nullptr}; int mks[3] = {0, 0, 0}; bool mixed = false; };
void launch_slab_flush(const SlabSrc &src, hipStream_t s);
void launch_rms_quant_slabs(const SlabSrc &src, const float *w, int N, int K, const ActQ &A, int mask, hipStream_t s);
void launch_silu_mul_quant_slabs(const SlabSrc &src, int N, int K, const ActQ &A, int mask, const Tables &tb, hipStream_t s);
void launch_rope_kv_slabs(const SlabSrc &src, int N, int n_head, int hd, const int *n_past, const float *cos_tab, const float *sin_tab, __half *kcache, __half *vcache, hipStream_t s);
bool launch_mmq2_set(const QWeight *const *W, float *const *y, const float *const *residual, int n, const ActQ &A, int N, int ldy, hipStream_t s, SlabSrc *defer = nullptr,
                     int force_ks = 0);
void set_mmq2_cus(int cus);
void set_mmqh(int v);
int mmqh_enabled();
bool mmq3_supported(int type, int rows, int cols);
size_t mmq3_plane_bytes(int rows, int cols, size_t *hi_off = nullptr);
void launch_mmq3_build(const QWeight &W, uint8_t *planes, hipStream_t s);
bool launch_mmq3_set(const QWeight *const *W, const uint8_t *const *planes, float *const *y, const float *const *residual, int n, const ActQ &A, int N, int ldy, hipStream_t s, SlabSrc *defer = nullptr);
int probe_tn_mfma(int rows, int cols, int TN, int iters, int n_sets, int check, int cus, float *us_per_launch, float *rel_diff);
void set_mmq3_waves(int nw);
void set_mmq3_tuning(int cus, int ks);
void set_mmq2_tuning(int tt, int fill_pct, int ks);
void set_gemm_splitk_xcd(int on);
void set_gemm_tuning(int big_min_m, int f16_ks, int arm = -1, int sk_arm = -1);
void set_f16_gemm(int v);
void launch_slab_reduce(const float *slabs, int n_slabs, long long slab_stride, const float *residual, float *y, size_t n, hipStream_t s);
bool launch_gemm_f16_silu_pair(const __half *A, int lda, const __half *W1, const __half *W3, int M, int N, int K, const Tables &tb, float *out, __half *out_h, int ldo, int cus, hipStream_t s);
bool launch_gemm_f16_set(const __half *A, int lda, const __half *const *W, int n, int M, int N, int K, float *const *y, const float *const *residual, int ldo, float *ws,
                         size_t ws_floats, int cus, hipStream_t s, SlabSrc *defer = nullptr);

bool launch_matvec_set(const QWeight *const *W, float *const *y, const float *const *residual, int n, const ActQ &A, hipStream_t s, int pro = 0, const float *px = nullptr,
                       const float *pw = nullptr, const Tables *tb = nullptr, int epi = 0);
constexpr int MATVEC_EPI_REF = 2;
bool matvec_silu_pair_supported(int type, int cols);
bool launch_matvec_rows(const QWeight *const *W, float *const *y, const float *const *residual, int n, const ActQ &A, int N, int ldy, hipStream_t s, const float *px = nullptr,
                        const float *pw = nullptr, int ldx = 0);
bool matvec_rows_prologue_ok(int type, int K);
bool ri_supported(int type, int rows, int cols);
size_t ri_plan(int type, int rows, int cols, RiPlanes &p, uint8_t *base);
void launch_ri_build(const QWeight &w, const RiPlanes &p, hipStream_t s);
struct RiWorkspace { float *slabs = nullptr; size_t slab_floats = 0; unsigned *tickets = nullptr; int n_tickets = 0; };
bool launch_matvec_ri(const QWeight *const *W, const RiPlanes *const *ri, float *const *y, const float *const *residual, int n, const ActQ &A, int N, int ldy, hipStream_t s,
                      const float *px = nullptr, const float *pw = nullptr, int ldx = 0, const RiWorkspace &ws = RiWorkspace{});
bool launch_matvec_ri_mixed(const QWeight *const *Wa, const RiPlanes *const *ria, float *const *ya, int na, const QWeight *const *Wb, const RiPlanes *const *rib, float *const *yb, int nb,
                            const ActQ &A, int N, int ldy, hipStream_t s);
void set_ri_cus(int cus);
int ri_ksplit(int total_groups, int K, const RiWorkspace &ws);
bool launch_matvec_mixed(const QWeight *const *W1, float *const *y1, int n1, const QWeight *const *W2, float *const *y2, int n2, const ActQ &A, hipStream_t s, int pro = 0,
                         const float *px = nullptr, const float *pw = nullptr, int epi = 0);
bool launch_matvec_rows_mixed(const QWeight *const *W1, float *const *y1, int n1, const QWeight *const *W2, float *const *y2, int n2, const ActQ &A, int N, int ldy, hipStream_t s,
                              const float *px = nullptr, const float *pw = nullptr, int ldx = 0);
void set_matvec_tuning(int waves_per_cu, int fat_threads, int cus);
void kernel_name_tracing(bool on);
const char *last_kernel_name();
void reset_kernel_name();
size_t launch_probe_count();
float launch_probe_us(size_t first, size_t last);
int read_matvec_timeline(unsigned long long *out, int max_workgroups);
int read_attn_timeline(unsigned long long *out, int max_workgroups);
int read_vision_timeline(unsigned long long *out, int max_workgroups);

void launch_get_rows(int type, const uint8_t *raw_table, int K, const int *tokens, int N, float *out, hipStream_t s);

void launch_rope_kv(float *q, const float *k, const float *v, int N, int n_head, int hd, const int *n_past, const float *cos_tab,
                    const float *sin_tab, __half *kcache, __half *vcache, hipStream_t s);
void rope_tables(int n_ctx, int hd, std::vector<float> &cos_out, std::vector<float> &sin_out);
void launch_kv_shift(__half *kc_slot, __half *vc_slot, int n_layer, int n_ctx, int E, int hd, int n_keep, int n_discard, int n_rows, const float *cos_tab,
                     const float *sin_tab, hipStream_t s);
constexpr int KV_COPY_MAX_DST = 64;
struct KvCopyDst { __half *k[KV_COPY_MAX_DST]; __half *v[KV_COPY_MAX_DST]; };
void launch_kv_copy(const __half *src_k, const __half *src_v, int src_rows, const KvCopyDst &dst, int n_dst, int dst_rows, int n_layer, int E, int n_rows, hipStream_t s);
void launch_attn_llm(float *q, const float *k, const float *v, __half *kcache, __half *vcache, int N, int n_head, int hd, const int *n_past, int n_ctx,
                     const float *cos_tab, const float *sin_tab, const Tables &tb, float *out, bool fused, hipStream_t s);
size_t attn_split_workspace_bytes(int n_head, int hd, int n_ctx, int splits);
int attn_split_count(int n_head, int cus);
void launch_attn_llm_split(float *q, const float *k, const float *v, __half *kcache, __half *vcache, int n_head, int hd, const int *n_past, int n_ctx, const float *cos_tab,
                           const float *sin_tab, const Tables &tb, float *out, void *ws, int splits, hipStream_t s);
void launch_attn_llm_batched(float *q, const float *k, const float *v, __half *kcache, __half *vcache, int B, int n_head, int hd, const int *n_past, const int *row_slot,
                             size_t seq_stride, int n_ctx, const float *cos_tab, const float *sin_tab, const Tables &tb, float *out, hipStream_t s);
void launch_batch_finish(const float *logits, int n_vocab, int B, const int *row_slot, int *n_past, int *argmax, int *feed, float *slot_logits, hipStream_t s);
void launch_batch_begin(int *n_past, const int *row_slot, const int *row_pos, int B, hipStream_t s);
constexpr int DRAFT_ROWS = 8;
void launch_attn_llm_draft(float *q, const float *k, const float *v, __half *kcache, __half *vcache, int R, int n_head, int hd, const int *n_past, const int *row_slot,
                           size_t seq_stride, int n_ctx, const float *cos_tab, const float *sin_tab, const Tables &tb, float *out, hipStream_t s);
void launch_draft_begin(int *n_past, const int *row_slot, const int *row_pos, hipStream_t s);
void launch_draft_finish(const float *logits, int n_vocab, int R, const int *tok, const int *row_slot, int *n_past, int *argmax, int *feed, float *slot_logits, int *res, hipStream_t s);
void launch_rope_kv_seg(float *q, const float *k, const float *v, int N, int n_head, int hd, const int *rows, size_t seq_stride, const float *cos_tab, const float *sin_tab,
                        __half *kcache, __half *vcache, hipStream_t s);
void launch_rope_kv_seg_slabs(const SlabSrc &src, int N, int n_head, int hd, const int *rows, size_t seq_stride, const float *cos_tab, const float *sin_tab, __half *kcache, __half *vcache,
                              hipStream_t s);
struct AttnSegs { const int *segs = nullptr; const int *tiles[2] = {nullptr, nullptr}; int n_tiles[2] = {0, 0}; int t_max = 0; size_t seq_stride = 0; };
int attn_seg_tiles(const int *segs, int n_seg, int qt, int *out);
bool launch_attn_prefill_seg(const float *q, const __half *kcache, const __half *vcache, const AttnSegs &sg, int n_head, int hd, const Tables &tb, float *out, hipStream_t s,
                             __half *out_h = nullptr, bool *wrote_h = nullptr);
void launch_seg_finish(const float *logits, int n_vocab, int B, const int *fin, int *n_past, int *argmax, int *feed, float *slot_logits, hipStream_t s);
void launch_gather_rows(const float *src, const int *idx, int n, int E, float *dst, hipStream_t s);
void launch_logprob_rows(const float *logits, int ld, int n_vocab, int rows, const int *targets, float *logprob, int *greedy, float *greedy_logprob, hipStream_t s);
constexpr int TOPN_MAX = 64;
bool launch_topn_rows(const float *logits, int ld, int n_vocab, int rows, const int *row_index, int top_n, const int *targets, int *ids, float *logprobs, int *rank,
                      float *target_logprob, hipStream_t s);
bool launch_pen_pick(const float *logits, int ld, int n_vocab, int n_rows, const PenRow *rows, const PenEntry *table, int *picked, float *adjusted, hipStream_t s);
bool launch_attn_prefill(const float *q, const __half *kcache, const __half *vcache, int N, int n_head, int hd, const int *n_past, int t_max, const Tables &tb, float *out, hipStream_t s, __half *out_h = nullptr, bool *wrote_h = nullptr);
void launch_attn_ref(const float *q, const __half *kcache, const __half *vcache, int N, int n_head, int hd, const int *n_past, int t_max, const Tables &tb, float *out, hipStream_t s);
void launch_attn_ref_fused(const float *q, const float *k, const float *v, __half *kcache, __half *vcache, int n_head, int hd, const int *n_past, int t_max, const float *cos_tab, const float *sin_tab,
                           const Tables &tb, float *out, hipStream_t s);
void set_attn_prefill_f16(int v);
int attn_prefill_form();
int attn_prefill_f16();
void set_attn_prefill_form(int v);
void set_attn_prefill_w8(int v);
bool attn_head_size_supported(int hd);
void attn_ref_prepare();
int attn_ref_max_ctx(int hd);
int attn_max_ctx(int hd);
int attn_draft_max_ctx(int hd);
void launch_argmax(const float *logits, int n, int *out, void *scratch , hipStream_t s);
void launch_add_inplace(float *x, const float *y, size_t n, hipStream_t s);
void launch_set_int(int *p, int v, hipStream_t s);
void launch_stall(unsigned ms, hipStream_t s);
uint64_t device_checksum(const void *p, size_t bytes, hipStream_t s);
void launch_fill_u16(void *p, size_t n, unsigned short v, hipStream_t s);
void launch_advance(int *n_past, int n, int *tok0, const int *argmax, hipStream_t s);
void launch_delay(int us, hipStream_t s);

void launch_gemm_f16(const __half *A, int lda, const __half *W, int ldw, int M, int N, int K, const float *bias, const float *residual,
                     bool gelu, const Tables &tb, float *out, __half *out_h, int ldo, hipStream_t s);
void launch_gemm_f16_head_major(const __half *A, int lda, const __half *W, int ldw, int M, int N, int K, const float *bias, const Tables &tb, float *out, int D, int hd, hipStream_t s);
bool launch_gemm_f16_skinny(const __half *A, int lda, const __half *W, int ldw, int M, int N, int K, const float *bias, const float *residual, bool gelu, const Tables &tb,
                            float *out, __half *out_h, int ldo, hipStream_t s);
bool launch_gemm_f16_skinny_splitk(const __half *A, int lda, const __half *W, int ldw, int M, int N, int K, int slices, float *slabs, size_t slab_stride, int ldo, hipStream_t s);
void launch_lin_epilogue(const float *y, const float *bias, const float *residual, bool gelu, const Tables &tb, int rows, int n, float *out, __half *out_h, hipStream_t s);
void launch_layernorm(const float *x, const float *w, const float *b, int rows, int n, float *out, __half *out_h, hipStream_t s, bool sequential_sums = false);
void launch_attn_vref(const float *q, int ldq, const float *k, const float *v, int ldk, int nq, int nk, int heads, int hd, float q_prescale, float score_div, const Tables &tb,
                      float *out, int ldo, hipStream_t s, int batch = 1);
bool launch_gemm_f16_arm(int arm, const __half *A, int lda, const __half *W, int ldw, int M, int N, int K, const float *bias, const float *residual, bool gelu, const Tables &tb,
                         float *out, __half *out_h, int ldo, hipStream_t s);
bool launch_gemm_f16_splitk_arm(int arm, const __half *A, int lda, const __half *W, int ldw, int M, int N, int K, int slices, float *slabs, size_t slab_stride, int ldo, hipStream_t s);
int gemm_split_slices(int K, int want);
void launch_gemm_f16_splitk(const __half *A, int lda, const __half *W, int ldw, int M, int N, int K, int slices, float *slabs, size_t slab_stride, int ldo, hipStream_t s);
void launch_splitk_reduce_ln(const float *slabs, int n_slabs, size_t slab_stride, const float *bias, const float *residual, int rows, int n, float *x_out, const float *ln_w,
                             const float *ln_b, float *ln_out, __half *ln_out_h, hipStream_t s);
void set_attn_vit_qt(int qt);
void launch_attn_f32(const float *q, int ldq, const float *k, const float *v, int ldk, int nq, int nk, int heads, int hd, float q_prescale,
                     float score_div, const Tables &tb, float *out, __half *out_h, int ldo, hipStream_t s, int batch = 1, int head_stride_q = 0, int head_stride_kv = 0)   ;
void launch_im2col(const float *image, __half *patches, int ldp, hipStream_t s, int batch = 1);
void launch_assemble_embeddings(const float *cls, const float *pe, const float *pos, int D, float *x, hipStream_t s, int batch = 1);
void launch_f32_to_f16(const float *x, __half *y, size_t n, hipStream_t s);

void launch_resample_h(const uint8_t *src, int W, int H, const int *first, const int *count, const int *kk, int ksize, uint8_t *dst, int OW, hipStream_t s);
void launch_resample_v_norm(const uint8_t *src, int OW, const int *first, const int *count, const int *kk, int ksize, float *out, int OH, const float mean[3], const float std[3],
                            hipStream_t s);

}
```

minigpt4.cpp_amd/csrc/llm_kernels.hip:

```cpp
#include "kernels.hpp"
#include "devutil.hpp"

#include <algorithm>
#include <cstdarg>
#include <cstring>
#include <tuple>
#include <type_traits>
#include <vector>
#include <hip/hip_ext.h>

namespace mg4 {

static bool g_kname_on = false;
static char g_kname[192] = "";
struct LaunchProbe { hipEvent_t start, stop; };
static std::vector<LaunchProbe> g_probes;
static size_t g_probe_next = 0;
void kernel_name_tracing(bool on) {
    g_kname_on = on; g_kname[0] = 0;
    if (on) { for (auto &p : g_probes) { HIP_IGNORE(hipEventDestroy(p.start)); HIP_IGNORE(hipEventDestroy(p.stop)); } g_probes.clear(); g_probe_next = 0; }
}
void reset_kernel_name() { g_kname[0] = 0; }
const char *last_kernel_name() { return g_kname; }
size_t launch_probe_count() { return g_probes.size(); }
// ... 1433 lines not shown
}
void rope_tables(int n_ctx, int hd, std::vector<float> &c, std::vector<float> &s) {
    const size_t C = (size_t)n_ctx, P = (size_t)hd / 2;
    c.assign(C * P, 0.0f); s.assign(C * P, 0.0f);
    const float theta_scale = powf(10000.0f, -2.0f / (float)hd);
    for (size_t p = 0; p < C; p++) { float theta = (float)p; for (size_t i = 0; i < P; i++) { c[p * P + i] = cosf(theta); s[p * P + i] = sinf(theta); theta *= theta_scale; } }
}

constexpr int KV_SHIFT_ROWS = 8, KV_SHIFT_THREADS = 64;
__global__ __launch_bounds__(KV_SHIFT_THREADS) void k_kv_shift(__half *__restrict__ kc, __half *__restrict__ vc, int n_layer, int n_ctx, int E, int hd, int n_keep,
                                                             int n_discard, int n_rows, const float *__restrict__ cos_tab, const float *__restrict__ sin_tab) {
    const int G = E / 8;
    const long long per = (long long)n_layer * G;
    const long long lane = (long long)blockIdx.x * KV_SHIFT_THREADS + threadIdx.x;
    if (lane >= 2 * per) return;
    const bool is_k = lane < per;
    const long long lg = is_k ? lane : lane - per;
    const int layer = (int)(lg / G), g = (int)(lg % G);
    __half *col = (is_k ? kc : vc) + (size_t)layer * n_ctx * E + (size_t)g * 8;
    float c[4] = {1.0f, 1.0f, 1.0f, 1.0f}, s[4] = {0.0f, 0.0f, 0.0f, 0.0f};
    if (is_k) {
        const size_t t0 = (size_t)n_discard * (hd / 2) + (size_t)((g * 8) % hd) / 2;
#pragma unroll
        for (int j = 0; j < 4; j++) { c[j] = cos_tab[t0 + j]; s[j] = sin_tab[t0 + j]; }
    }
    const int b = min(n_discard, KV_SHIFT_ROWS);
    for (int r0 = n_keep + n_discard; r0 < n_rows; r0 += b) {
        const int nb = min(b, n_rows - r0);
        uint4 buf[KV_SHIFT_ROWS];
#pragma unroll
        for (int t = 0; t < KV_SHIFT_ROWS; t++) if (t < nb) buf[t] = *reinterpret_cast<const uint4 *>(col + (size_t)(r0 + t) * E);
#pragma unroll
        for (int t = 0; t < KV_SHIFT_ROWS; t++) {
            if (t >= nb) continue;
            uint4 u = buf[t];
            if (is_k) {
                unsigned w[4] = {u.x, u.y, u.z, u.w};
#pragma unroll
                for (int j = 0; j < 4; j++) {
                    const float2 kf = __half22float2(*reinterpret_cast<const __half2 *>(&w[j]));
                    const double k0 = kf.x, k1 = kf.y, cj = c[j], sj = s[j];
                    const __half2 r = __floats2half2_rn((float)(k0 * cj + k1 * sj), (float)(k1 * cj - k0 * sj));
                    w[j] = *reinterpret_cast<const unsigned *>(&r);
                }
                u = make_uint4(w[0], w[1], w[2], w[3]);
            }
            *reinterpret_cast<uint4 *>(col + (size_t)(r0 + t - n_discard) * E) = u;
        }
    }
}
void launch_kv_shift(__half *kc_slot, __half *vc_slot, int n_layer, int n_ctx, int E, int hd, int n_keep, int n_discard, int n_rows, const float *cos_tab,
                     const float *sin_tab, hipStream_t s) {
    if (n_discard < 1 || n_keep < 0 || n_keep + n_discard >= n_rows) return;
    if (n_rows > n_ctx || n_discard > n_ctx - 1 || E % 8 || hd % 8 || E % hd) throw HipError{hipErrorInvalidValue, "launch_kv_shift: bad shape", __FILE__, __LINE__};
    note_kernel("k_kv_shift");
    const long long lanes = 2LL * n_layer * (E / 8);
    hipLaunchKernelGGL(k_kv_shift, dim3((unsigned)((lanes + KV_SHIFT_THREADS - 1) / KV_SHIFT_THREADS)), dim3(KV_SHIFT_THREADS), 0, s, kc_slot, vc_slot, n_layer, n_ctx, E, hd,
                       n_keep, n_discard, n_rows, cos_tab, sin_tab);
}

constexpr int KV_COPY_PIECES = 4, KV_COPY_THREADS = 256;
struct KvPiece { uint4 data; size_t off; int sel; };
__device__ __forceinline__ KvPiece kv_piece_load(const __half *src_k, const __half *src_v, unsigned i0, unsigned total, unsigned per, unsigned n_layer, unsigned src_rows,
                                                 unsigned dst_rows, unsigned E) {
    const unsigned i = i0 < total ? i0 : 0u;
    const unsigned run = i / per, within = i - run * per;
    const bool is_v = run >= n_layer;
    const unsigned layer = is_v ? run - n_layer : run;
    KvPiece p;
    p.data = *reinterpret_cast<const uint4 *>((is_v ? src_v : src_k) + (size_t)layer * src_rows * E + (size_t)within * 8);
    p.off = (size_t)layer * dst_rows * E + (size_t)within * 8;
    p.sel = i0 < total ? (is_v ? 2 : 1) : 0;
    return p;
}
__device__ __forceinline__ void kv_piece_store(const KvPiece &p, __half *dk, __half *dv) {
    if (p.sel) *reinterpret_cast<uint4 *>((p.sel == 2 ? dv : dk) + p.off) = p.data;
}
__global__ __launch_bounds__(KV_COPY_THREADS) void k_kv_copy(const __half *src_k, const __half *src_v, unsigned src_rows, const KvCopyDst dst, int n_dst, unsigned dst_rows,
                                                           unsigned n_layer, unsigned E, unsigned n_rows) {
    static_assert(KV_COPY_PIECES == 4, "the four pieces are named");
    const unsigned per = n_rows * (E / 8);
    const unsigned total = 2u * n_layer * per;
    const unsigned first = blockIdx.x * (KV_COPY_PIECES * KV_COPY_THREADS) + threadIdx.x;
    const KvPiece p0 = kv_piece_load(src_k, src_v, first, total, per, n_layer, src_rows, dst_rows, E);
    const KvPiece p1 = kv_piece_load(src_k, src_v, first + KV_COPY_THREADS, total, per, n_layer, src_rows, dst_rows, E);
    const KvPiece p2 = kv_piece_load(src_k, src_v, first + 2 * KV_COPY_THREADS, total, per, n_layer, src_rows, dst_rows, E);
    const KvPiece p3 = kv_piece_load(src_k, src_v, first + 3 * KV_COPY_THREADS, total, per, n_layer, src_rows, dst_rows, E);
    for (int d = 0; d < n_dst; d++) {
        __half *const dk = dst.k[d], *const dv = dst.v[d];
        kv_piece_store(p0, dk, dv); kv_piece_store(p1, dk, dv); kv_piece_store(p2, dk, dv); kv_piece_store(p3, dk, dv);
    }
}
void launch_kv_copy(const __half *src_k, const __half *src_v, int src_rows, const KvCopyDst &dst, int n_dst, int dst_rows, int n_layer, int E, int n_rows, hipStream_t s) {
    auto bad = [](const char *what) { throw HipError{hipErrorInvalidValue, what, __FILE__, __LINE__}; };
    if (!src_k || !src_v || n_dst < 1 || n_dst > KV_COPY_MAX_DST || n_layer < 1 || E < 8 || E % 8 || src_rows < 1 || dst_rows < 1 || n_rows < 0) bad("launch_kv_copy: bad shape");
    if (n_rows > src_rows || n_rows > dst_rows) bad("launch_kv_copy: n_rows exceeds a region's row count");
    auto aligned = [](const __half *p) { return (uintptr_t)p % 16 == 0; };
    if (!aligned(src_k) || !aligned(src_v)) bad("launch_kv_copy: a region is not 16-byte aligned");
    const size_t src_n = (size_t)n_layer * src_rows * E, dst_n = (size_t)n_layer * dst_rows * E;
    auto overlap = [](const __half *a, size_t na, const __half *b, size_t nb) { const uintptr_t x = (uintptr_t)a, y = (uintptr_t)b; return x < y + 2 * nb && y < x + 2 * na; };
    for (int d = 0; d < n_dst; d++) {
        if (!dst.k[d] || !dst.v[d]) bad("launch_kv_copy: bad shape");
        if (!aligned(dst.k[d]) || !aligned(dst.v[d])) bad("launch_kv_copy: a region is not 16-byte aligned");
        for (const __half *p : {dst.k[d], dst.v[d]}) if (overlap(p, dst_n, src_k, src_n) || overlap(p, dst_n, src_v, src_n)) bad("launch_kv_copy: a destination overlaps the source");
    }
    if (n_rows == 0) return;
    const unsigned long long total = 2ull * n_layer * n_rows * (E / 8);
    if (total >= (1ull << 31)) bad("launch_kv_copy: bad shape");
    note_kernel("k_kv_copy");
    const unsigned per_block = KV_COPY_PIECES * KV_COPY_THREADS;
    hipLaunchKernelGGL(k_kv_copy, dim3((unsigned)((total + per_block - 1) / per_block)), dim3(KV_COPY_THREADS), 0, s, src_k, src_v, (unsigned)src_rows, dst, n_dst, (unsigned)dst_rows,
                       (unsigned)n_layer, (unsigned)E, (unsigned)n_rows);
}

constexpr int AT_THREADS = 512;
__device__ __forceinline__ float2 rope_rot(float x0, float x1, float c, float s) { return make_float2(x0 * c - x1 * s, x0 * s + x1 * c); }
__device__ __forceinline__ __half2 rope_rot_h2(float x0, float x1, float c, float s) { const float2 r = rope_rot(x0, x1, c, s); return __floats2half2_rn(r.x, r.y); }
__device__ __forceinline__ void st_h2(__half *p, __half2 v) { *reinterpret_cast<__half2 *>(p) = v; }
__device__ __forceinline__ void unpack8(const int4 &v, float (&f)[8]) {
    const unsigned w[4] = {(unsigned)v.x, (unsigned)v.y, (unsigned)v.z, (unsigned)v.w};
#pragma unroll
    for (int e = 0; e < 4; e++) { f[2 * e] = h2f_bits(w[e] & 0xFFFF); f[2 * e + 1] = h2f_bits(w[e] >> 16); }
}
template <int CH> __device__ __forceinline__ float dot16(const int4 &kk, const float (&qd)[8], float scale) {
    float kf[8], s = 0.0f;
    unpack8(kk, kf);
#pragma unroll
    for (int e = 0; e < 8; e++) s = fmaf(kf[e], qd[e], s);
    s += dpp_f<0xB1>(s); s += dpp_f<0x4E>(s);
    if (CH >= 8) s += dpp_f<0x141>(s);
    if (CH >= 16) s += dpp_f<0x140>(s);
    return s * scale;
}
__device__ __forceinline__ void pv_acc(float (&o)[8], const int4 &vv, float pj) {
    const unsigned w[4] = {(unsigned)vv.x, (unsigned)vv.y, (unsigned)vv.z, (unsigned)vv.w};
#pragma unroll
    for (int e = 0; e < 4; e++) { o[2 * e] = fmaf(h2f_bits(w[e] & 0xFFFF), pj, o[2 * e]); o[2 * e + 1] = fmaf(h2f_bits(w[e] >> 16), pj, o[2 * e + 1]); }
}
static size_t attn_lds_bytes(int n_ctx, int hd, int rows) {
    const int Tpad = (n_ctx + 7) & ~7;
    return (size_t)Tpad * 6 + (size_t)hd * 2 + (size_t)2 * rows * hd * 2 + (size_t)(AT_THREADS / (hd / 8)) * hd * 4 + 64;
}
static int attn_ctx_that_fits(int hd, int rows) { int n = 0; while (attn_lds_bytes(n + 8, hd, rows) + 256  <= 160 * 1024) n += 8; return n; }
int attn_max_ctx(int hd) { return attn_ctx_that_fits(hd, 1); }
int attn_draft_max_ctx(int hd) { return attn_ctx_that_fits(hd, DRAFT_ROWS); }

template <int HD, bool FUSED, bool BATCHED = false>
__global__ __launch_bounds__(AT_THREADS) void k_attn_llm(float *__restrict__ q, const float *__restrict__ kin, const float *__restrict__ vin, __half *__restrict__ kc,
                                                         __half *__restrict__ vc, int E, const int *__restrict__ n_past, const float *__restrict__ cos_tab,
                                                         const float *__restrict__ sin_tab, const Tables tb, float *__restrict__ out, const int *__restrict__ row_slot = nullptr,
                                                         size_t seq_stride = 0) {
    constexpr bool DRAFT = false;
    constexpr int n_ctx = 0;
#include "attn_llm_body.hpp"
}
template <int HD>
__global__ __launch_bounds__(AT_THREADS) void k_attn_llm_draft(float *__restrict__ q, const float *__restrict__ kin, const float *__restrict__ vin, __half *__restrict__ kc,
                                                               __half *__restrict__ vc, int E, const int *__restrict__ n_past, int n_ctx, const float *__restrict__ cos_tab,
                                                               const float *__restrict__ sin_tab, const Tables tb, float *__restrict__ out, const int *__restrict__ row_slot,
                                                               size_t seq_stride) {
    constexpr bool FUSED = true, BATCHED = true, DRAFT = true;
#include "attn_llm_body.hpp"
}

template <class F> static bool attn_for_head_size(int hd, F &&f) {
    switch (hd) {
    case 32: f(std::integral_constant<int, 32>{}); return true;
    case 64: f(std::integral_constant<int, 64>{}); return true;
    case 128: f(std::integral_constant<int, 128>{}); return true;
    default: return false;
    }
}
template <class F> static void attn_for_head_size_or_throw(int hd, F &&f) {
    if (!attn_for_head_size(hd, f)) throw HipError{hipErrorInvalidValue, "unsupported head size", __FILE__, __LINE__};
}
template <int HD, bool BATCHED, bool DRAFT>
static void launch_attn_body(bool fused, float *q, const float *k, const float *v, __half *kc, __half *vc, int rows, int n_head, const int *n_past, const int *row_slot,
                             size_t seq_stride, int n_ctx, const float *cos_tab, const float *sin_tab, const Tables &tb, float *out, hipStream_t s) {
    const size_t lds = attn_lds_bytes(n_ctx, HD, DRAFT ? DRAFT_ROWS : 1);
    const dim3 grid((unsigned)n_head, (unsigned)rows);
    static bool attr = false;
    if constexpr (DRAFT) {
        if (!attr) { HIP_IGNORE(lds_optin_max(&k_attn_llm_draft<HD>)); attr = true; }
        note_kernel("k_attn_llm_draft<%d>", HD);
        hipLaunchKernelGGL((k_attn_llm_draft<HD>), grid, dim3(AT_THREADS), lds, s, q, k, v, kc, vc, n_head * HD, n_past, n_ctx, cos_tab, sin_tab, tb, out, row_slot, seq_stride);
    } else if constexpr (BATCHED) {
        if (!attr) { HIP_IGNORE(lds_optin_max(&k_attn_llm<HD, true, true>)); attr = true; }
        hipLaunchKernelGGL((k_attn_llm<HD, true, true>), grid, dim3(AT_THREADS), lds, s, q, k, v, kc, vc, n_head * HD, n_past, cos_tab, sin_tab, tb, out, row_slot, seq_stride);
    } else {
        if (!attr) { HIP_IGNORE(lds_optin_max(&k_attn_llm<HD, true>));
                     HIP_IGNORE(lds_optin_max(&k_attn_llm<HD, false>)); attr = true; }
        note_kernel("k_attn_llm<%d, %s, false>", HD, fused ? "true" : "false");
        hipLaunchKernelGGL((fused ? k_attn_llm<HD, true> : k_attn_llm<HD, false>), grid, dim3(AT_THREADS), lds, s, q, k, v, kc, vc, n_head * HD, n_past, cos_tab, sin_tab, tb, out,
                           row_slot, seq_stride);
    }
}
void launch_attn_llm(float *q, const float *k, const float *v, __half *kcache, __half *vcache, int N, int n_head, int hd, const int *n_past, int n_ctx,
                     const float *cos_tab, const float *sin_tab, const Tables &tb, float *out, bool fused, hipStream_t s) {
    attn_for_head_size_or_throw(hd, [&](auto tag) {
        launch_attn_body<decltype(tag)::value, false, false>(fused, q, k, v, kcache, vcache, fused ? 1 : N, n_head, n_past, nullptr, 0, n_ctx, cos_tab, sin_tab, tb, out, s); });
}
void launch_attn_llm_batched(float *q, const float *k, const float *v, __half *kcache, __half *vcache, int B, int n_head, int hd, const int *n_past, const int *row_slot,
                             size_t seq_stride, int n_ctx, const float *cos_tab, const float *sin_tab, const Tables &tb, float *out, hipStream_t s) {
    attn_for_head_size_or_throw(hd, [&](auto tag) {
        launch_attn_body<decltype(tag)::value, true, false>(true, q, k, v, kcache, vcache, B, n_head, n_past, row_slot, seq_stride, n_ctx, cos_tab, sin_tab, tb, out, s); });
}
void launch_attn_llm_draft(float *q, const float *k, const float *v, __half *kcache, __half *vcache, int R, int n_head, int hd, const int *n_past, const int *row_slot,
                           size_t seq_stride, int n_ctx, const float *cos_tab, const float *sin_tab, const Tables &tb, float *out, hipStream_t s) {
    if (R < 1 || R > DRAFT_ROWS) throw HipError{hipErrorInvalidValue, "launch_attn_llm_draft: row count out of range", __FILE__, __LINE__};
    attn_for_head_size_or_throw(hd, [&](auto tag) {
        launch_attn_body<decltype(tag)::value, true, true>(true, q, k, v, kcache, vcache, R, n_head, n_past, row_slot, seq_stride, n_ctx, cos_tab, sin_tab, tb, out, s); });
}
constexpr int AS_THREADS = 256;
template <int HD>
__global__ __launch_bounds__(AS_THREADS) void k_attn_split_scores(const float *__restrict__ q, const float *__restrict__ kin, const float *__restrict__ vin, __half *__restrict__ kc,
                                                                   __half *__restrict__ vc, int E, const int *__restrict__ n_past, const float *__restrict__ cos_tab,
                                                                   const float *__restrict__ sin_tab, float *__restrict__ scores, int ld_scores, __half *__restrict__ qrot) {
    constexpr int CH = HD / 8, P = AS_THREADS / CH;
    constexpr int NR = 16;
    const int h = blockIdx.x, sp = blockIdx.y, S = gridDim.y, tid = threadIdx.x;
    const int pos = *n_past, Tg = pos;
    __shared__ __attribute__((aligned(16))) __half qh[HD];
    __shared__ __attribute__((aligned(16))) __half knew[HD];
    const float scale = 1.0f / sqrtf((float)HD);
    const size_t qo = (size_t)h * HD;
    const int c = tid % CH, p = tid / CH;
    const int per = ((Tg + S - 1) / S + P - 1) / P * P;
    const int j_lo = sp * per, j_hi = min(Tg, j_lo + per), j_cl = max(j_hi - 1, 0);
    const __half *kb = kc + (size_t)h * HD + 8 * c;
    int4 kk[NR];
#pragma unroll
    for (int i = 0; i < NR; i++) kk[i] = ld16(kb + (size_t)min(j_lo + p + i * P, j_cl) * E);
    if (tid < HD / 2) {
        const int i = tid;
        const float cs = cos_tab[(size_t)pos * (HD / 2) + i], sn = sin_tab[(size_t)pos * (HD / 2) + i];
        const float2 qf = rope_rot(q[qo + 2 * i], q[qo + 2 * i + 1], cs, sn), kf = rope_rot(kin[qo + 2 * i], kin[qo + 2 * i + 1], cs, sn);
        const __half2 qr = __halves2half2(f2h_rn(qf.x), f2h_rn(qf.y)), kr = __halves2half2(f2h_rn(kf.x), f2h_rn(kf.y));
        st_h2(qh + 2 * i, qr); st_h2(knew + 2 * i, kr);
        if (sp == 0) {
            const __half2 vr = __halves2half2(f2h_rn(vin[qo + 2 * i]), f2h_rn(vin[qo + 2 * i + 1]));
            const size_t co = (size_t)pos * E + (size_t)h * HD + 2 * i;
            st_h2(kc + co, kr); st_h2(vc + co, vr);
            st_h2(qrot + qo + 2 * i, qr);
        }
    }
    __syncthreads();
    float qd[8];
    unpack8(*reinterpret_cast<const int4 *>(qh + 8 * c), qd);
    float *srow = scores + (size_t)h * ld_scores;
    for (int j0 = j_lo + p; j0 < j_hi; j0 += NR * P) {
        int4 nx[NR];
        const bool more = j0 + NR * P < j_hi;
#pragma unroll
        for (int i = 0; i < NR; i++) nx[i] = ld16(kb + (size_t)min(j0 + (NR + i) * P, j_cl) * E);
#pragma unroll
        for (int i = 0; i < NR; i++) { const int j = j0 + i * P; const float s = dot16<CH>(kk[i], qd, scale); if (j < j_hi && c == 0) srow[j] = s; }
        (void)more;
#pragma unroll
        for (int i = 0; i < NR; i++) kk[i] = nx[i];
    }
    if (sp == S - 1 && tid == 0) {
        float s = 0.0f;
        for (int i = 0; i < HD; i++) s = fmaf(__half2float(knew[i]), __half2float(qh[i]), s);
        srow[pos] = s * scale;
    }
}
template <int HD>
__global__ __launch_bounds__(AS_THREADS) void k_attn_split_pv(const float *__restrict__ scores, int ld_scores, const __half *__restrict__ vc, int E, const int *__restrict__ n_past,
                                                               const Tables tb, float *__restrict__ partial, unsigned *__restrict__ arrive, float *__restrict__ out) {
    extern __shared__ __attribute__((aligned(16))) unsigned char smem_sp[];
    constexpr int CH = HD / 8, P = AS_THREADS / CH;
    const int h = blockIdx.x, sp = blockIdx.y, S = gridDim.y, tid = threadIdx.x;
    const int pos = *n_past, T = pos + 1;
    float *sc = reinterpret_cast<float *>(smem_sp);
    float *part = sc + ((T + 3) & ~3);
    __shared__ float s_red[AS_THREADS / 64];
    __shared__ double s_dred[AS_THREADS / 64];
    __shared__ int s_last;
    constexpr int NR = 16;
    const int per = ((T + S - 1) / S + P - 1) / P * P;
    const int j_lo = sp * per, j_hi = min(T, j_lo + per), j_cl = max(j_hi - 1, 0);
    const int c = tid % CH, p = tid / CH;
    const __half *vb = vc + (size_t)h * HD + 8 * c;
    int4 vv[NR];
#pragma unroll
    for (int i = 0; i < NR; i++) vv[i] = ld16(vb + (size_t)min(j_lo + p + i * P, j_cl) * E);
    const float *srow = scores + (size_t)h * ld_scores;
    float mx = -INFINITY;
    for (int j = tid; j < T; j += AS_THREADS) { const float s = srow[j]; sc[j] = s; mx = fmaxf(mx, s); }
    mx = wave_max(mx);
    if ((tid & 63) == 0) s_red[tid >> 6] = mx;
    __syncthreads();
    mx = fmaxf(fmaxf(s_red[0], s_red[1]), fmaxf(s_red[2], s_red[3]));
    double sum = 0.0;
    for (int j0 = tid; j0 < T; j0 += 4 * AS_THREADS) {
        float v[4];
#pragma unroll
        for (int u = 0; u < 4; u++) { const int j = j0 + u * AS_THREADS; v[u] = j < T ? exp_h(tb.exp, sc[j] - mx) : 0.0f; }
#pragma unroll
        for (int u = 0; u < 4; u++) { const int j = j0 + u * AS_THREADS; if (j < T) { sc[j] = v[u]; sum += (double)v[u]; } }
    }
    sum = wave_sum_d(sum);
    if ((tid & 63) == 0) s_dred[tid >> 6] = sum;
    __syncthreads();
    const float inv = (float)(1.0 / (((s_dred[0] + s_dred[1]) + s_dred[2]) + s_dred[3]));
    float o[8] = {0, 0, 0, 0, 0, 0, 0, 0};
    for (int j0 = j_lo + p; j0 < j_hi; j0 += NR * P) {
        int4 nx[NR];
#pragma unroll
        for (int i = 0; i < NR; i++) nx[i] = ld16(vb + (size_t)min(j0 + (NR + i) * P, j_cl) * E);
#pragma unroll
        for (int i = 0; i < NR; i++) {
            const int j = j0 + i * P;
            if (j < j_hi) pv_acc(o, vv[i], __half2float(f2h_rn(sc[j] * inv)));
        }
#pragma unroll
        for (int i = 0; i < NR; i++) vv[i] = nx[i];
    }
#pragma unroll
    for (int e = 0; e < 8; e++) part[p * HD + 8 * c + e] = o[e];
    __syncthreads();
    float *mine = partial + ((size_t)h * S + sp) * HD;
    for (int i = tid; i < HD; i += AS_THREADS) {
        float s = 0.0f;
#pragma unroll 8
        for (int pp = 0; pp < P; pp++) s += part[pp * HD + i];
        __hip_atomic_store(mine + i, s, __ATOMIC_RELAXED, __HIP_MEMORY_SCOPE_AGENT);
    }
    asm volatile("s_waitcnt vmcnt(0)" ::: "memory");
    __syncthreads();
    if (tid == 0) s_last = __hip_atomic_fetch_add(arrive + h, 1u, __ATOMIC_RELAXED, __HIP_MEMORY_SCOPE_AGENT) == (unsigned)(S - 1);
    __syncthreads();
    if (!s_last) return;
    for (int i = tid; i < HD; i += AS_THREADS) {
        float s = 0.0f;
        for (int k = 0; k < S; k++) s += __hip_atomic_load(partial + ((size_t)h * S + k) * HD + i, __ATOMIC_RELAXED, __HIP_MEMORY_SCOPE_AGENT);
        out[(size_t)h * HD + i] = s;
    }
    if (tid == 0) __hip_atomic_store(arrive + h, 0u, __ATOMIC_RELAXED, __HIP_MEMORY_SCOPE_AGENT);
}
size_t attn_split_workspace_bytes(int n_head, int hd, int n_ctx, int splits) {
    return (size_t)n_head * (size_t)((n_ctx + 3) & ~3) * 4 + (size_t)n_head * splits * hd * 4 + (size_t)n_head * hd * 2 + (size_t)n_head * 4 + 1024;
}
int attn_split_count(int n_head, int cus) { return std::max(2, std::min(16, (cus - cus / 16) / std::max(1, n_head))); }
template <int HD>
static void launch_attn_split_hd(float *q, const float *k, const float *v, __half *kc, __half *vc, int n_head, const int *n_past, int n_ctx, const float *cos_tab, const float *sin_tab,
                                 const Tables &tb, float *out, void *ws, int splits, hipStream_t s) {
    const int ld = (n_ctx + 3) & ~3;
    float *scores = reinterpret_cast<float *>(ws);
    float *partial = scores + (size_t)n_head * ld;
    __half *qrot = reinterpret_cast<__half *>(partial + (size_t)n_head * splits * HD);
    unsigned *arrive = reinterpret_cast<unsigned *>(reinterpret_cast<unsigned char *>(qrot) + (((size_t)n_head * HD * 2 + 255) & ~(size_t)255));
    note_kernel("k_attn_split_scores<%d>", HD);
    hipLaunchKernelGGL((k_attn_split_scores<HD>), dim3((unsigned)n_head, (unsigned)splits), dim3(AS_THREADS), 0, s, q, k, v, kc, vc, n_head * HD, n_past, cos_tab, sin_tab, scores, ld, qrot);
    const size_t lds = (size_t)ld * 4 + (size_t)(AS_THREADS / (HD / 8)) * HD * 4 + 64;
    static bool attr = false;
    if (!attr) { HIP_IGNORE(lds_optin_max(&k_attn_split_pv<HD>)); attr = true; }
    note_kernel("k_attn_split_pv<%d>", HD);
    hipLaunchKernelGGL((k_attn_split_pv<HD>), dim3((unsigned)n_head, (unsigned)splits), dim3(AS_THREADS), lds, s, scores, ld, vc, n_head * HD, n_past, tb, partial, arrive, out);
}
void launch_attn_llm_split(float *q, const float *k, const float *v, __half *kcache, __half *vcache, int n_head, int hd, const int *n_past, int n_ctx, const float *cos_tab,
                           const float *sin_tab, const Tables &tb, float *out, void *ws, int splits, hipStream_t s) {
    attn_for_head_size_or_throw(hd, [&](auto tag) { launch_attn_split_hd<decltype(tag)::value>(q, k, v, kcache, vcache, n_head, n_past, n_ctx, cos_tab, sin_tab, tb, out, ws, splits, s); });
}
// ... 947 lines not shown
```

minigpt4.cpp_amd/minigpt4_library.py:

```python
from __future__ import annotations

import ctypes
import enum
import os
from typing import Iterator, List, Optional, Sequence

import numpy as np


class DataType(enum.IntEnum):
    F16 = 0; F32 = 1; I32 = 2; L64 = 3; Q4_0 = 4; Q4_1 = 5; Q5_0 = 6; Q5_1 = 7; Q8_0 = 8; Q8_1 = 9
    Q2_K = 10; Q3_K = 11; Q4_K = 12; Q5_K = 13; Q6_K = 14; Q8_K = 15

    def __str__(self):
        return str(self.name)


class Verbosity(enum.IntEnum):
    SILENT = 0; ERR = 1; INFO = 2; DEBUG = 3


class ImageFormat(enum.IntEnum):
    UNKNOWN = 0; F32 = 1; U8 = 2

# ... 64 lines not shown
            self._declare_test(test)
        return self._test

    @property
    def test_hooks(self):
        return self._hooks()

    def _last_error(self):
        a = self._product.minigpt4_amd_last_error() or b""
        b = (self._test.minigpt4_amd_last_error() or b"") if self._test is not None else b""
        return a + (b" | " if a and b else b"") + b

    def __getattr__(self, name):
        if name == "minigpt4_amd_last_error":
            return self._last_error
        if name in self._hook_names:
            return getattr(self._hooks(), name)
        return getattr(self._product, name)


class MiniGPT4SharedLibrary:

    def __init__(self, shared_library_path: str, test_library_path: Optional[str] = None):
        product = ctypes.cdll.LoadLibrary(shared_library_path)
        if test_library_path is None:
            test_library_path = os.environ.get("MINIGPT4_TEST_LIBRARY", shared_library_path[:-3] + "_test.so" if shared_library_path.endswith(".so") else shared_library_path + "_test")
        self.library = _Symbols(product, test_library_path, self._declare_test_hooks)
        L = product
        P = ctypes.POINTER
        L.minigpt4_model_load.argtypes = [CHAR_PTR, CHAR_PTR, I32, I32, I32, I32, ctypes.c_bool]
        L.minigpt4_model_load.restype = VOID_PTR
        L.minigpt4_image_load_from_file.argtypes = [VOID_PTR, CHAR_PTR, P(MiniGPT4Image), I32]
        L.minigpt4_preprocess_image.argtypes = [VOID_PTR, P(MiniGPT4Image), P(MiniGPT4Image), I32]
        L.minigpt4_encode_image.argtypes = [VOID_PTR, P(MiniGPT4Image), P(MiniGPT4Embedding), SIZE_T]
        L.minigpt4_begin_chat_image.argtypes = [VOID_PTR, P(MiniGPT4Embedding), CHAR_PTR, SIZE_T]
        L.minigpt4_end_chat_image.argtypes = [VOID_PTR, P(ctypes.c_char_p)] + _CHAT_ARGS
        L.minigpt4_system_prompt.argtypes = [VOID_PTR, SIZE_T]
        L.minigpt4_begin_chat.argtypes = [VOID_PTR, CHAR_PTR, SIZE_T]
        L.minigpt4_end_chat.argtypes = [VOID_PTR, P(ctypes.c_char_p)] + _CHAT_ARGS
        L.minigpt4_reset_chat.argtypes = [VOID_PTR]
        L.minigpt4_contains_eos_token.argtypes = [CHAR_PTR]
        L.minigpt4_is_eos.argtypes = [CHAR_PTR]
        L.minigpt4_free.argtypes = [VOID_PTR]
        L.minigpt4_free_image.argtypes = [P(MiniGPT4Image)]
        L.minigpt4_free_embedding.argtypes = [P(MiniGPT4Embedding)]
        L.minigpt4_error_code_to_string.argtypes = [I32]
        L.minigpt4_error_code_to_string.restype = CHAR_PTR
        L.minigpt4_quantize_model.argtypes = [CHAR_PTR, CHAR_PTR, I32]
        L.minigpt4_set_verbosity.argtypes = [I32]
        L.minigpt4_set_verbosity.restype = None
        for name in ("image_load_from_file", "preprocess_image", "encode_image", "begin_chat_image", "end_chat_image", "system_prompt",
                     "begin_chat", "end_chat", "reset_chat", "contains_eos_token", "is_eos", "free", "free_image", "free_embedding", "quantize_model"):
            getattr(L, "minigpt4_" + name).restype = I32
        L.minigpt4_amd_device_count.restype = I32
        L.minigpt4_amd_last_error.restype = CHAR_PTR
        L.minigpt4_amd_build_info.restype = CHAR_PTR
        L.minigpt4_amd_decode_image.argtypes = [CHAR_PTR, SIZE_T, P(MiniGPT4Image)]
        L.minigpt4_amd_decode_image.restype = I32
        for name in ("n_vocab", "n_embd", "n_past", "sync"):
            getattr(L, "minigpt4_amd_" + name).argtypes = [VOID_PTR]
            getattr(L, "minigpt4_amd_" + name).restype = I32
        L.minigpt4_amd_eval_tokens.argtypes = [VOID_PTR, INT_PTR, I32]
        L.minigpt4_amd_eval_embd.argtypes = [VOID_PTR, FLOAT_PTR, I32]
        L.minigpt4_amd_get_logits.argtypes = [VOID_PTR, FLOAT_PTR, SIZE_T]
        L.minigpt4_amd_tokenize.argtypes = [VOID_PTR, CHAR_PTR, I32, INT_PTR, I32]
        L.minigpt4_amd_sample.argtypes = [VOID_PTR, INT_PTR, F32, I32, F32, F32, F32, I32, F32, F32]
        L.minigpt4_amd_decode_loop.argtypes = [VOID_PTR, I32, INT_PTR, FLOAT_PTR]
        L.minigpt4_amd_profile_sites.argtypes = [VOID_PTR, I32, ctypes.c_char_p, SIZE_T]
        L.minigpt4_amd_weight_bytes_per_token.argtypes = [VOID_PTR]
        L.minigpt4_amd_weight_bytes_per_token.restype = ctypes.c_double
        L.minigpt4_amd_last_encode_ms.argtypes = [VOID_PTR]
        L.minigpt4_amd_last_encode_ms.restype = F32
        for name in ("minigpt4_amd_encode_images", "minigpt4_encode_images"):
            getattr(L, name).argtypes = [VOID_PTR, P(MiniGPT4Images), P(MiniGPT4Embeddings), SIZE_T]
        for name in ("minigpt4_amd_free_embeddings", "minigpt4_free_embeddings"):
            getattr(L, name).argtypes = [P(MiniGPT4Embeddings)]
        L.minigpt4_amd_weight_arena.argtypes = [VOID_PTR, I32, P(VOID_PTR), P(SIZE_T)]
        U64P, SZP = P(ctypes.c_uint64), P(ctypes.c_size_t)
        L.minigpt4_amd_plan_arenas.argtypes = [CHAR_PTR, CHAR_PTR, SZP, SZP, U64P, U64P]
        L.minigpt4_amd_arena_plan.argtypes = [VOID_PTR, SZP, SZP, U64P, U64P]
        L.minigpt4_amd_load_mode.argtypes = [VOID_PTR]
        L.minigpt4_amd_weights_received.argtypes = [VOID_PTR]
        L.minigpt4_amd_arena_checksum.argtypes = [VOID_PTR, I32, U64P]
        L.minigpt4_amd_set_parity.argtypes = [VOID_PTR, I32]
        L.minigpt4_amd_dist_info.argtypes = [VOID_PTR, P(I32), P(I32), P(F32)]
        L.minigpt4_amd_dist_info.restype = I32
        L.minigpt4_amd_parity.argtypes = [VOID_PTR]
        L.minigpt4_amd_set_conversations.argtypes = [VOID_PTR, I32]
        L.minigpt4_amd_select_conversation.argtypes = [VOID_PTR, I32]
        L.minigpt4_amd_n_conversations.argtypes = [VOID_PTR]
        L.minigpt4_amd_end_chat_batch.argtypes = [VOID_PTR, INT_PTR, I32, P(ctypes.c_char_p), F32, I32, F32, F32, F32, I32, F32, F32]
        L.minigpt4_amd_eval_batch.argtypes = [VOID_PTR, INT_PTR, I32, INT_PTR, INT_PTR]
        L.minigpt4_amd_prefill_batch.argtypes = [VOID_PTR, INT_PTR, I32]
        L.minigpt4_amd_batch_path.argtypes = [VOID_PTR, INT_PTR]
        L.minigpt4_amd_shift_context.argtypes = [VOID_PTR, I32, I32]
        L.minigpt4_amd_set_context_shift.argtypes = [VOID_PTR, I32]
        L.minigpt4_amd_fork_conversation.argtypes = [VOID_PTR, I32, INT_PTR, I32, I32]
        L.minigpt4_amd_set_prefix_cache.argtypes = [VOID_PTR, I32]
        L.minigpt4_amd_prefix_cache_info.argtypes = [VOID_PTR, INT_PTR]
        L.minigpt4_amd_score_tokens.argtypes = [VOID_PTR, INT_PTR, I32, FLOAT_PTR, INT_PTR, FLOAT_PTR, FLOAT_PTR]
        L.minigpt4_amd_score_batch.argtypes = [VOID_PTR, INT_PTR, I32, INT_PTR, INT_PTR, FLOAT_PTR, INT_PTR, FLOAT_PTR]
        L.minigpt4_amd_token_piece.argtypes = [VOID_PTR, I32]
        L.minigpt4_amd_token_piece.restype = ctypes.c_char_p
        L.minigpt4_amd_top_logprobs.argtypes = [VOID_PTR, INT_PTR, I32, I32, INT_PTR, INT_PTR, FLOAT_PTR, FLOAT_PTR, INT_PTR]
        L.minigpt4_amd_end_chat_batch_top.argtypes = [VOID_PTR, INT_PTR, I32, P(ctypes.c_char_p), F32, I32, F32, F32, F32, I32, F32, F32, I32, INT_PTR, FLOAT_PTR, INT_PTR, INT_PTR,
                                                      FLOAT_PTR]
        L.minigpt4_amd_score_tokens_top.argtypes = [VOID_PTR, INT_PTR, I32, I32, FLOAT_PTR, INT_PTR, INT_PTR, FLOAT_PTR]
        L.minigpt4_amd_set_speculation.argtypes = [VOID_PTR, I32]
        L.minigpt4_amd_verify_draft.argtypes = [VOID_PTR, INT_PTR, I32, INT_PTR, INT_PTR, INT_PTR]
        L.minigpt4_amd_decode_lookup.argtypes = [VOID_PTR, INT_PTR, I32, I32, I32, I32, I32, INT_PTR, INT_PTR, INT_PTR]
        L.minigpt4_amd_set_penalties.argtypes = [VOID_PTR, I32]
        L.minigpt4_amd_conversation_penalties.argtypes = [VOID_PTR, I32, I32, F32, F32, F32, I32]
        L.minigpt4_amd_set_logit_bias.argtypes = [VOID_PTR, INT_PTR, FLOAT_PTR, I32]
        L.minigpt4_amd_token_history.argtypes = [VOID_PTR, INT_PTR, I32]
        L.minigpt4_amd_penalty_info.argtypes = [VOID_PTR, INT_PTR]

    @staticmethod
    def _declare_test_hooks(L):
        P = ctypes.POINTER
        U64P = P(ctypes.c_uint64)
        L.minigpt4_amd_convert_q3k_q6k.argtypes = [VOID_PTR, VOID_PTR, ctypes.c_int64]
        L.minigpt4_amd_test_mul_mat.argtypes = [I32, VOID_PTR, ctypes.c_int64, ctypes.c_int64, FLOAT_PTR, ctypes.c_int64, FLOAT_PTR]
        L.minigpt4_amd_test_mul_mat_ref.argtypes = L.minigpt4_amd_test_mul_mat.argtypes
        L.minigpt4_amd_test_mmq2.argtypes = [I32, VOID_PTR, I32, ctypes.c_int64, ctypes.c_int64, FLOAT_PTR, ctypes.c_int64, FLOAT_PTR, I32, I32, FLOAT_PTR]
        L.minigpt4_amd_test_matvec.argtypes = [I32, VOID_PTR, I32, I32, VOID_PTR, I32, ctypes.c_int64, ctypes.c_int64, FLOAT_PTR, FLOAT_PTR, I32, I32, I32, FLOAT_PTR, FLOAT_PTR]
        L.minigpt4_amd_test_matvec_rows.argtypes = [I32, VOID_PTR, I32, ctypes.c_int64, ctypes.c_int64, FLOAT_PTR, I32, FLOAT_PTR, FLOAT_PTR]
        L.minigpt4_amd_test_quantize.argtypes = [FLOAT_PTR, FLOAT_PTR, ctypes.c_int64, ctypes.c_int64, VOID_PTR, VOID_PTR, VOID_PTR, VOID_PTR, VOID_PTR]
        L.minigpt4_amd_test_gemm_f16.argtypes = [FLOAT_PTR, FLOAT_PTR, FLOAT_PTR, I32, I32, I32, I32, FLOAT_PTR]
        L.minigpt4_amd_test_gemm_f16_skinny.argtypes = L.minigpt4_amd_test_gemm_f16.argtypes
        L.minigpt4_amd_test_gemm_f16_ex.argtypes = [FLOAT_PTR, FLOAT_PTR, FLOAT_PTR, I32, I32, I32, I32, I32, VOID_PTR, FLOAT_PTR]
        L.minigpt4_amd_test_matvec_ex.argtypes = L.minigpt4_amd_test_matvec.argtypes[:-1] + [VOID_PTR, FLOAT_PTR]
        L.minigpt4_amd_test_f16_silu_pair.argtypes = [FLOAT_PTR, VOID_PTR, ctypes.c_int64, ctypes.c_int64, ctypes.c_int64, VOID_PTR, FLOAT_PTR]
        L.minigpt4_amd_test_f16_silu_pair_ex.argtypes = [FLOAT_PTR, VOID_PTR, ctypes.c_int64, ctypes.c_int64, ctypes.c_int64, VOID_PTR, VOID_PTR, FLOAT_PTR]
        L.minigpt4_amd_test_layernorm.argtypes = [FLOAT_PTR, FLOAT_PTR, FLOAT_PTR, I32, I32, I32, FLOAT_PTR, VOID_PTR]
        L.minigpt4_amd_test_splitk_reduce_ln.argtypes = [FLOAT_PTR, I32, ctypes.c_int64, FLOAT_PTR, FLOAT_PTR, I32, I32, I32, FLOAT_PTR, FLOAT_PTR, FLOAT_PTR, FLOAT_PTR, VOID_PTR]
        L.minigpt4_amd_test_gemm_f16_splitk.argtypes = [FLOAT_PTR, FLOAT_PTR, I32, I32, I32, I32, I32, FLOAT_PTR, INT_PTR]
        L.minigpt4_amd_test_gemm_f16_head_major.argtypes = [FLOAT_PTR, FLOAT_PTR, FLOAT_PTR, I32, I32, I32, I32, FLOAT_PTR]
        L.minigpt4_amd_test_im2col.argtypes = [FLOAT_PTR, I32, I32, VOID_PTR]
        L.minigpt4_amd_test_assemble.argtypes = [FLOAT_PTR, FLOAT_PTR, FLOAT_PTR, I32, I32, FLOAT_PTR]
        L.minigpt4_amd_test_lin_epilogue.argtypes = [FLOAT_PTR, FLOAT_PTR, FLOAT_PTR, VOID_PTR, I32, I32, FLOAT_PTR, VOID_PTR]
        L.minigpt4_amd_test_set_gemm_arm.argtypes = [I32, I32]
        L.minigpt4_amd_test_set_gemm_arm.restype = None
        L.minigpt4_amd_test_set_splitk_xcd.argtypes = [I32]
        L.minigpt4_amd_test_set_splitk_xcd.restype = None
        L.minigpt4_amd_test_activation.argtypes = [I32, VOID_PTR, VOID_PTR]
        L.minigpt4_amd_test_attn_f32.argtypes = [FLOAT_PTR, FLOAT_PTR, FLOAT_PTR, I32, I32, I32, I32, I32, F32, F32, I32, I32, VOID_PTR, FLOAT_PTR, VOID_PTR]
        L.minigpt4_amd_test_kv_shift.argtypes = [I32, I32, I32, I32, I32, I32, I32, VOID_PTR, VOID_PTR, FLOAT_PTR]
        L.minigpt4_amd_test_kv_copy.argtypes = [I32, I32, I32, I32, I32, INT_PTR, I32, I32, I32, VOID_PTR, VOID_PTR, FLOAT_PTR]
        L.minigpt4_amd_test_logprob_rows.argtypes = [FLOAT_PTR, I32, I32, I32, INT_PTR, FLOAT_PTR, INT_PTR, FLOAT_PTR, FLOAT_PTR]
        L.minigpt4_amd_test_topn_rows.argtypes = [FLOAT_PTR, I32, I32, I32, INT_PTR, I32, I32, INT_PTR, INT_PTR, FLOAT_PTR, INT_PTR, FLOAT_PTR, FLOAT_PTR]
        L.minigpt4_amd_test_penalise_host.argtypes = [FLOAT_PTR, I32, INT_PTR, I32, I32, I32, F32, F32, F32, I32, INT_PTR, FLOAT_PTR, I32, INT_PTR, I32, INT_PTR]
        L.minigpt4_amd_test_pen_pick.argtypes = [FLOAT_PTR, I32, I32, I32, INT_PTR, I32, INT_PTR, I32, INT_PTR, FLOAT_PTR, FLOAT_PTR]
        L.minigpt4_amd_test_attn_draft.argtypes = [I32, I32, I32, I32, I32, I32, I32, I32, I32, FLOAT_PTR, FLOAT_PTR, FLOAT_PTR, VOID_PTR, VOID_PTR, FLOAT_PTR]
        L.minigpt4_amd_test_ngram_draft.argtypes = [INT_PTR, I32, I32, I32, I32, INT_PTR]
        L.minigpt4_amd_test_attn_prefill_seg.argtypes = [I32, I32, I32, I32, VOID_PTR, VOID_PTR, I32, INT_PTR, FLOAT_PTR, I32, FLOAT_PTR, FLOAT_PTR, INT_PTR, VOID_PTR, VOID_PTR, INT_PTR]
        L.minigpt4_amd_test_rope_kv_seg.argtypes = [I32, I32, I32, I32, I32, INT_PTR, FLOAT_PTR, FLOAT_PTR, FLOAT_PTR, I32, FLOAT_PTR, VOID_PTR, VOID_PTR, FLOAT_PTR, VOID_PTR, VOID_PTR]
        L.minigpt4_amd_last_error.restype = CHAR_PTR
        L.minigpt4_amd_vocab_load.argtypes = [CHAR_PTR]
        L.minigpt4_amd_vocab_load.restype = VOID_PTR
        L.minigpt4_amd_vocab_free.argtypes = [VOID_PTR]
        L.minigpt4_amd_vocab_free.restype = None
        L.minigpt4_amd_vocab_size.argtypes = [VOID_PTR]
        L.minigpt4_amd_vocab_piece.argtypes = [VOID_PTR, I32, INT_PTR]
        L.minigpt4_amd_vocab_piece.restype = VOID_PTR
        L.minigpt4_amd_vocab_tokenize.argtypes = [VOID_PTR, CHAR_PTR, I32, INT_PTR, I32]
        L.minigpt4_amd_inspect_files.argtypes = [CHAR_PTR, CHAR_PTR, INT_PTR, INT_PTR, P(ctypes.c_int64)]
        L.minigpt4_amd_sample_logits.argtypes = [FLOAT_PTR, I32, I32, F32, I32, F32, F32, F32, I32, F32, F32]
        L.minigpt4_amd_resample_coeffs.argtypes = [I32, I32, INT_PTR, INT_PTR, INT_PTR, INT_PTR, SIZE_T]
        L.minigpt4_amd_copy_arenas.argtypes = [VOID_PTR, VOID_PTR]
        L.minigpt4_amd_llm_file_digest.argtypes = [CHAR_PTR, U64P, I32]
        L.minigpt4_amd_quantize_chunk.argtypes = [I32, FLOAT_PTR, VOID_PTR, ctypes.c_int64]
        L.minigpt4_amd_quantize_chunk.restype = ctypes.c_int64
        L.minigpt4_amd_probe_valu.restype = F32
        L.minigpt4_amd_probe_grid_barrier.restype = F32

    def panic_if_error(self, error_code: int) -> None:
        if error_code != 0:
            raise RuntimeError(self.library.minigpt4_error_code_to_string(I32(error_code)))

    def minigpt4_model_load(self, model_path: str, llm_model_path: str, verbosity: int = 1, seed: int = 1337, n_ctx: int = 2048,
                            n_batch: int = 512, numa: int = 0) -> MiniGPT4Context:
        ptr = self.library.minigpt4_model_load(model_path.encode(), llm_model_path.encode(), int(verbosity), seed, n_ctx, n_batch, bool(numa))
        if not ptr:
            raise RuntimeError("minigpt4_model_load failed: " + (self.library.minigpt4_amd_last_error() or b"").decode(errors="replace"))
        return MiniGPT4Context(ptr)

    def minigpt4_image_load_from_file(self, ctx: MiniGPT4Context, path: str, flags: int = 0) -> MiniGPT4Image:
        image = MiniGPT4Image()
        self.panic_if_error(self.library.minigpt4_image_load_from_file(ctx.ptr, path.encode(), ctypes.pointer(image), flags))
        return image

    def minigpt4_preprocess_image(self, ctx: MiniGPT4Context, image: MiniGPT4Image, flags: int = 0) -> MiniGPT4Image:
        out = MiniGPT4Image()
        self.panic_if_error(self.library.minigpt4_preprocess_image(ctx.ptr, ctypes.pointer(image), ctypes.pointer(out), flags))
        return out

    def minigpt4_encode_image(self, ctx: MiniGPT4Context, image: MiniGPT4Image, n_threads: int = 0) -> MiniGPT4Embedding:
        embedding = MiniGPT4Embedding()
        self.panic_if_error(self.library.minigpt4_encode_image(ctx.ptr, ctypes.pointer(image), ctypes.pointer(embedding), n_threads))
        return embedding

    def minigpt4_begin_chat_image(self, ctx: MiniGPT4Context, image_embedding: MiniGPT4Embedding, s: str, n_threads: int = 0):
        self.panic_if_error(self.library.minigpt4_begin_chat_image(ctx.ptr, ctypes.pointer(image_embedding), s.encode(), n_threads))

    def _end(self, fn, ctx, n_threads, temp, top_k, top_p, tfs_z, typical_p, repeat_last_n, repeat_penalty, alpha_presence, alpha_frequency,
             mirostat, mirostat_tau, mirostat_eta, penalize_nl) -> str:
        token = ctypes.c_char_p()
        self.panic_if_error(fn(ctx.ptr, ctypes.byref(token), n_threads, temp, top_k, top_p, tfs_z, typical_p, repeat_last_n, repeat_penalty,
                               alpha_presence, alpha_frequency, mirostat, mirostat_tau, mirostat_eta, penalize_nl))
        return (token.value or b"").decode("utf-8", errors="replace")

    def minigpt4_end_chat_image(self, ctx, n_threads=0, temp=0.8, top_k=40, top_p=0.9, tfs_z=1.0, typical_p=1.0, repeat_last_n=64,
                                repeat_penalty=1.1, alpha_presence=1.0, alpha_frequency=1.0, mirostat=0, mirostat_tau=5.0, mirostat_eta=1.0,
                                penalize_nl=1) -> str:
        return self._end(self.library.minigpt4_end_chat_image, ctx, n_threads, temp, top_k, top_p, tfs_z, typical_p, repeat_last_n, repeat_penalty,
                         alpha_presence, alpha_frequency, mirostat, mirostat_tau, mirostat_eta, penalize_nl)

    def minigpt4_system_prompt(self, ctx: MiniGPT4Context, n_threads: int = 0):
        self.panic_if_error(self.library.minigpt4_system_prompt(ctx.ptr, n_threads))

    def minigpt4_begin_chat(self, ctx: MiniGPT4Context, s: str, n_threads: int = 0):
        self.panic_if_error(self.library.minigpt4_begin_chat(ctx.ptr, s.encode(), n_threads))

    def minigpt4_end_chat(self, ctx, n_threads=0, temp=0.8, top_k=40, top_p=0.9, tfs_z=1.0, typical_p=1.0, repeat_last_n=64, repeat_penalty=1.1,
                          alpha_presence=1.0, alpha_frequency=1.0, mirostat=0, mirostat_tau=5.0, mirostat_eta=1.0, penalize_nl=1) -> str:
        return self._end(self.library.minigpt4_end_chat, ctx, n_threads, temp, top_k, top_p, tfs_z, typical_p, repeat_last_n, repeat_penalty,
                         alpha_presence, alpha_frequency, mirostat, mirostat_tau, mirostat_eta, penalize_nl)

    def minigpt4_reset_chat(self, ctx: MiniGPT4Context):
        self.panic_if_error(self.library.minigpt4_reset_chat(ctx.ptr))

    def minigpt4_contains_eos_token(self, s: str) -> bool:
        return bool(self.library.minigpt4_contains_eos_token(s.encode()))

    def minigpt4_is_eos(self, s: str) -> bool:
        return bool(self.library.minigpt4_is_eos(s.encode()))

    def minigpt4_free(self, ctx: MiniGPT4Context) -> None:
        self.panic_if_error(self.library.minigpt4_free(ctx.ptr))
        ctx.ptr = None

    def minigpt4_free_image(self, image: MiniGPT4Image) -> None:
        self.panic_if_error(self.library.minigpt4_free_image(ctypes.pointer(image)))

    def minigpt4_free_embedding(self, embedding: MiniGPT4Embedding) -> None:
        self.panic_if_error(self.library.minigpt4_free_embedding(ctypes.pointer(embedding)))

    def minigpt4_error_code_to_string(self, error_code: int) -> str:
        return self.library.minigpt4_error_code_to_string(error_code).decode()

    def minigpt4_quantize_model(self, in_path: str, out_path: str, data_type: DataType):
        self.panic_if_error(self.library.minigpt4_quantize_model(in_path.encode(), out_path.encode(), int(data_type)))

    def minigpt4_set_verbosity(self, verbosity: Verbosity):
        self.library.minigpt4_set_verbosity(int(verbosity))

    def amd_device_count(self) -> int:
        return int(self.library.minigpt4_amd_device_count())

    def amd_plan_arenas(self, vision_path: str, llm_path: str) -> dict:
        lb, vb, lh, vh = ctypes.c_size_t(), ctypes.c_size_t(), ctypes.c_uint64(), ctypes.c_uint64()
        rc = self.library.minigpt4_amd_plan_arenas(vision_path.encode(), llm_path.encode(), ctypes.byref(lb), ctypes.byref(vb), ctypes.byref(lh), ctypes.byref(vh))
        if rc:
            raise RuntimeError(f"plan_arenas failed ({rc}): " + self.library.minigpt4_amd_last_error().decode())
        return {"llm_bytes": lb.value, "vision_bytes": vb.value, "llm_hash": lh.value, "vision_hash": vh.value}

    def amd_arena_plan(self, ctx) -> dict:
        lb, vb, lh, vh = ctypes.c_size_t(), ctypes.c_size_t(), ctypes.c_uint64(), ctypes.c_uint64()
        assert self.library.minigpt4_amd_arena_plan(ctx.ptr, ctypes.byref(lb), ctypes.byref(vb), ctypes.byref(lh), ctypes.byref(vh)) == 0
        return {"llm_bytes": lb.value, "vision_bytes": vb.value, "llm_hash": lh.value, "vision_hash": vh.value}

    def amd_arena_checksum(self, ctx, which: int) -> int:
        v = ctypes.c_uint64()
        assert self.library.minigpt4_amd_arena_checksum(ctx.ptr, which, ctypes.byref(v)) == 0
        return int(v.value)

    def amd_dist_info(self, ctx) -> dict:
        w, r, ms = I32(), I32(), F32()
        assert self.library.minigpt4_amd_dist_info(ctx.ptr, ctypes.byref(w), ctypes.byref(r), ctypes.byref(ms)) == 0
        return {"world": w.value, "rank": r.value, "bcast_ms": ms.value}

    def amd_set_parity(self, ctx, on: bool):
        if self.library.minigpt4_amd_set_parity(ctx.ptr, 1 if on else 0):
            raise RuntimeError("minigpt4_amd_set_parity failed")

    def amd_set_conversations(self, ctx, n: int):
        if self.library.minigpt4_amd_set_conversations(ctx.ptr, n):
            raise RuntimeError("set_conversations failed: " + self.library.minigpt4_amd_last_error().decode())

    def amd_select_conversation(self, ctx, slot: int):
        if self.library.minigpt4_amd_select_conversation(ctx.ptr, slot):
            raise RuntimeError("select_conversation: index out of range")

    def amd_end_chat_batch(self, ctx, slots: Sequence[int], temp=0.8, top_k=40, top_p=0.9, tfs_z=1.0, typical_p=1.0, mirostat=0, mirostat_tau=5.0,
                           mirostat_eta=1.0) -> List[str]:
        sl = np.ascontiguousarray(slots, np.int32)
        toks = (ctypes.c_char_p * len(sl))()
        rc = self.library.minigpt4_amd_end_chat_batch(ctx.ptr, sl.ctypes.data_as(INT_PTR), len(sl), toks, temp, top_k, top_p, tfs_z, typical_p, mirostat, mirostat_tau, mirostat_eta)
        if rc:
            raise RuntimeError("end_chat_batch failed: " + self.library.minigpt4_amd_last_error().decode())
        return [(t or b"").decode("utf-8", errors="replace") for t in toks]

    def amd_prefill_batch(self, ctx, slots: Sequence[int]):
        sl = np.ascontiguousarray(slots, np.int32)
        rc = self.library.minigpt4_amd_prefill_batch(ctx.ptr, sl.ctypes.data_as(INT_PTR), len(sl))
        if rc:
# ... 141 lines not shown

    def amd_token_piece(self, ctx, token_id: int) -> Optional[str]:
        p = self.library.minigpt4_amd_token_piece(ctx.ptr, int(token_id))
        return None if p is None else p.decode("utf-8", errors="replace")

    def amd_top_logprobs(self, ctx, slots: Sequence[int], top_n: int = 5, targets: Optional[Sequence[int]] = None) -> dict:
        sl = np.ascontiguousarray(slots, np.int32)
        n, k = len(sl), max(int(top_n), 1)
        tg = None if targets is None else np.ascontiguousarray(targets, np.int32)
        if tg is not None and tg.shape != (n,):
            raise RuntimeError("top_logprobs failed: top_logprobs: one target per slot is required")
        ti, tl, lp, rk = np.zeros((max(n, 1), k), np.int32), np.zeros((max(n, 1), k), np.float32), np.zeros(max(n, 1), np.float32), np.zeros(max(n, 1), np.int32)
        if self.library.minigpt4_amd_top_logprobs(ctx.ptr, sl.ctypes.data_as(INT_PTR), n, int(top_n), None if tg is None else tg.ctypes.data_as(INT_PTR),
                                                  ti.ctypes.data_as(INT_PTR), tl.ctypes.data_as(FLOAT_PTR), lp.ctypes.data_as(FLOAT_PTR), rk.ctypes.data_as(INT_PTR)):
            raise RuntimeError("top_logprobs failed: " + self.library.minigpt4_amd_last_error().decode("utf-8", errors="replace"))
        return dict(top_ids=ti[:n], top_logprobs=tl[:n], logprob=lp[:n], rank=rk[:n])

    def amd_end_chat_batch_top(self, ctx, slots: Sequence[int], top_n: int = 5, temp=0.8, top_k=40, top_p=0.9, tfs_z=1.0, typical_p=1.0, mirostat=0, mirostat_tau=5.0,
                               mirostat_eta=1.0) -> dict:
        sl = np.ascontiguousarray(slots, np.int32)
        n, k = len(sl), max(int(top_n), 1)
        toks = (ctypes.c_char_p * max(n, 1))()
        ids, lp, rk = np.zeros(max(n, 1), np.int32), np.zeros(max(n, 1), np.float32), np.zeros(max(n, 1), np.int32)
        ti, tl = np.zeros((max(n, 1), k), np.int32), np.zeros((max(n, 1), k), np.float32)
        if self.library.minigpt4_amd_end_chat_batch_top(ctx.ptr, sl.ctypes.data_as(INT_PTR), n, toks, temp, top_k, top_p, tfs_z, typical_p, mirostat, mirostat_tau, mirostat_eta,
                                                        int(top_n), ids.ctypes.data_as(INT_PTR), lp.ctypes.data_as(FLOAT_PTR), rk.ctypes.data_as(INT_PTR),
                                                        ti.ctypes.data_as(INT_PTR), tl.ctypes.data_as(FLOAT_PTR)):
            raise RuntimeError("end_chat_batch_top failed: " + self.library.minigpt4_amd_last_error().decode("utf-8", errors="replace"))
        return dict(pieces=[(t or b"").decode("utf-8", errors="replace") for t in toks[:n]], ids=ids[:n], logprob=lp[:n], rank=rk[:n], top_ids=ti[:n], top_logprobs=tl[:n])

    def amd_score_batch(self, ctx, slots: Sequence[int], token_lists: Sequence[Sequence[int]]) -> List[dict]:
        sl = np.ascontiguousarray(slots, np.int32)
        lists = [np.ascontiguousarray(t, np.int32).reshape(-1) for t in token_lists]
        cnt = np.ascontiguousarray([len(t) for t in lists], np.int32)
        tk = np.ascontiguousarray(np.concatenate(lists) if lists else np.zeros(0), np.int32)
        n = max(int(tk.size), 1)
        lp, gr, glp = np.zeros(n, np.float32), np.zeros(n, np.int32), np.zeros(n, np.float32)
        if len(lists) != len(sl):
            raise RuntimeError("score_batch failed: score_batch: one token list per slot is required")
        if self.library.minigpt4_amd_score_batch(ctx.ptr, sl.ctypes.data_as(INT_PTR), len(sl), tk.ctypes.data_as(INT_PTR), cnt.ctypes.data_as(INT_PTR),
                                                 lp.ctypes.data_as(FLOAT_PTR), gr.ctypes.data_as(INT_PTR), glp.ctypes.data_as(FLOAT_PTR)):
            raise RuntimeError("score_batch failed: " + self.library.minigpt4_amd_last_error().decode("utf-8", errors="replace"))
        ends = np.cumsum(cnt)
        return [dict(logprob=lp[e - c:e].copy(), greedy=gr[e - c:e].copy(), greedy_logprob=glp[e - c:e].copy()) for e, c in zip(ends, cnt)]

    def amd_test_logprob_rows(self, logits: np.ndarray, targets: Sequence[int], n_vocab: Optional[int] = None):
        lg = np.ascontiguousarray(logits, np.float32)
        assert lg.ndim == 2
        rows, ld = lg.shape
        nv = ld if n_vocab is None else int(n_vocab)
        tg = np.ascontiguousarray(targets, np.int32)
        assert tg.shape == (rows,)
        lp, gr, glp, ms = np.zeros(rows, np.float32), np.zeros(rows, np.int32), np.zeros(rows, np.float32), ctypes.c_float()
        rc = self.library.minigpt4_amd_test_logprob_rows(lg.ctypes.data_as(FLOAT_PTR), rows, nv, ld, tg.ctypes.data_as(INT_PTR), lp.ctypes.data_as(FLOAT_PTR),
                                                         gr.ctypes.data_as(INT_PTR), glp.ctypes.data_as(FLOAT_PTR), ctypes.byref(ms))
        if rc:
            raise RuntimeError(f"test_logprob_rows rc={rc}: " + self.library.minigpt4_amd_last_error().decode("utf-8", errors="replace"))
        return lp, gr, glp, float(ms.value)

    def amd_test_topn_rows(self, logits: np.ndarray, top_n: int, targets: Sequence[int], n_vocab: Optional[int] = None, row_index: Optional[Sequence[int]] = None):
        lg = np.ascontiguousarray(logits, np.float32)
        assert lg.ndim == 2
        buf_rows, ld = lg.shape
        nv = ld if n_vocab is None else int(n_vocab)
        tg = np.ascontiguousarray(targets, np.int32)
        ri = None if row_index is None else np.ascontiguousarray(row_index, np.int32)
        rows = int(tg.shape[0])
        assert tg.ndim == 1 and (ri is None or ri.shape == (rows,))
        k = max(int(top_n), 1)
        ids, lps = np.zeros((max(rows, 1), k), np.int32), np.zeros((max(rows, 1), k), np.float32)
        rk, tlp, ms = np.zeros(max(rows, 1), np.int32), np.zeros(max(rows, 1), np.float32), ctypes.c_float()
        rc = self.library.minigpt4_amd_test_topn_rows(lg.ctypes.data_as(FLOAT_PTR), buf_rows, nv, ld, None if ri is None else ri.ctypes.data_as(INT_PTR), rows, int(top_n),
                                                      tg.ctypes.data_as(INT_PTR), ids.ctypes.data_as(INT_PTR), lps.ctypes.data_as(FLOAT_PTR), rk.ctypes.data_as(INT_PTR),
                                                      tlp.ctypes.data_as(FLOAT_PTR), ctypes.byref(ms))
        if rc:
            raise RuntimeError(f"test_topn_rows rc={rc}: " + self.library.minigpt4_amd_last_error().decode("utf-8", errors="replace"))
        return ids[:rows], lps[:rows], rk[:rows], tlp[:rows], float(ms.value)

    def amd_test_kv_copy(self, k: np.ndarray, v: np.ndarray, src: int, dsts: Sequence[int], n_rows: int, src_rows: int = 0):
        k = np.ascontiguousarray(k, np.float16).copy()
        v = np.ascontiguousarray(v, np.float16).copy()
        assert k.ndim == 4 and k.shape == v.shape
        d = np.ascontiguousarray(dsts, np.int32)
        ms = ctypes.c_float()
        rc = self.library.minigpt4_amd_test_kv_copy(k.shape[0], k.shape[1], k.shape[2], k.shape[3], int(src), d.ctypes.data_as(INT_PTR), len(d), int(n_rows), int(src_rows),
                                                    k.ctypes.data_as(VOID_PTR), v.ctypes.data_as(VOID_PTR), ctypes.byref(ms))
        if rc:
            raise RuntimeError(f"test_kv_copy rc={rc}: " + self.library.minigpt4_amd_last_error().decode("utf-8", errors="replace"))
        return k, v, float(ms.value)

    def amd_test_kv_copy_ms(self, n_slot: int, n_layer: int, rows: int, n_embd: int, src: int, dsts: Sequence[int], n_rows: int, src_rows: int = 0) -> float:
        d = np.ascontiguousarray(dsts, np.int32)
        ms = ctypes.c_float()
        rc = self.library.minigpt4_amd_test_kv_copy(n_slot, n_layer, rows, n_embd, int(src), d.ctypes.data_as(INT_PTR), len(d), int(n_rows), int(src_rows), None, None, ctypes.byref(ms))
        if rc:
            raise RuntimeError(f"test_kv_copy rc={rc}: " + self.library.minigpt4_amd_last_error().decode("utf-8", errors="replace"))
        return float(ms.value)

    def amd_test_kv_shift(self, k: np.ndarray, v: np.ndarray, n_head: int, n_rows: int, n_keep: int, n_discard: int):
        k = np.ascontiguousarray(k, np.float16).copy()
        v = np.ascontiguousarray(v, np.float16).copy()
        assert k.ndim == 3 and k.shape == v.shape
        ms = ctypes.c_float()
        rc = self.library.minigpt4_amd_test_kv_shift(k.shape[0], k.shape[1], k.shape[2], n_head, n_rows, n_keep, n_discard, k.ctypes.data_as(VOID_PTR),
                                                     v.ctypes.data_as(VOID_PTR), ctypes.byref(ms))
        if rc:
            raise RuntimeError(f"test_kv_shift rc={rc}: " + self.library.minigpt4_amd_last_error().decode("utf-8", errors="replace"))
        return k, v, float(ms.value)

    def amd_test_attn_prefill_seg(self, kc: np.ndarray, vc: np.ndarray, n_head: int, segs, q: np.ndarray, form: int = 0, fp16_rows: bool = False):
        kc, vc = np.ascontiguousarray(kc, np.float16), np.ascontiguousarray(vc, np.float16)
        assert kc.ndim == 3 and kc.shape == vc.shape
        S, C, E = kc.shape
        sg = np.ascontiguousarray(segs, np.int32).reshape(-1, 3)
        q = np.ascontiguousarray(q, np.float32)
        a, b, one = np.zeros_like(q), np.zeros_like(q), ctypes.c_int32()
        ha, hb, wrote = (np.zeros(q.shape, np.uint16), np.zeros(q.shape, np.uint16), (ctypes.c_int32 * 2)()) if fp16_rows else (None, None, None)
        hp = [x.ctypes.data_as(VOID_PTR) if x is not None else None for x in (ha, hb)]
        rc = self.library.minigpt4_amd_test_attn_prefill_seg(n_head, E // n_head, C, S, kc.ctypes.data_as(VOID_PTR), vc.ctypes.data_as(VOID_PTR), len(sg), sg.ctypes.data_as(INT_PTR),
                                                             q.ctypes.data_as(FLOAT_PTR), form, a.ctypes.data_as(FLOAT_PTR), b.ctypes.data_as(FLOAT_PTR), ctypes.byref(one),
                                                             hp[0], hp[1], wrote)
        if rc:
            raise RuntimeError(f"test_attn_prefill_seg rc={rc}: " + self.library.minigpt4_amd_last_error().decode("utf-8", errors="replace"))
        if fp16_rows:
            return a, b, bool(one.value), ha, hb, (bool(wrote[0]), bool(wrote[1]))
        return a, b, bool(one.value)

    def amd_test_rope_kv_seg(self, n_head: int, n_ctx: int, n_slots: int, segs, q: np.ndarray, k: np.ndarray, v: np.ndarray, ks: int = 1):
        q, k, v = (np.ascontiguousarray(x, np.float32) for x in (q, k, v))
        N, E = q.shape
        sg = np.ascontiguousarray(segs, np.int32).reshape(-1, 3)
        out = [np.zeros_like(q), np.zeros((n_slots, n_ctx, E), np.float16), np.zeros((n_slots, n_ctx, E), np.float16),
               np.zeros_like(q), np.zeros((n_slots, n_ctx, E), np.float16), np.zeros((n_slots, n_ctx, E), np.float16)]
        ptr = [o.ctypes.data_as(FLOAT_PTR) if o.dtype == np.float32 else o.ctypes.data_as(VOID_PTR) for o in out]
        rc = self.library.minigpt4_amd_test_rope_kv_seg(n_head, E // n_head, n_ctx, n_slots, len(sg), sg.ctypes.data_as(INT_PTR), q.ctypes.data_as(FLOAT_PTR), k.ctypes.data_as(FLOAT_PTR),
                                                        v.ctypes.data_as(FLOAT_PTR), ks, *ptr)
        if rc:
            raise RuntimeError(f"test_rope_kv_seg rc={rc}: " + self.library.minigpt4_amd_last_error().decode("utf-8", errors="replace"))
        return tuple(out[:3]), tuple(out[3:])

    def amd_test_attn_draft(self, mode: int, q: np.ndarray, k: np.ndarray, v: np.ndarray, kc: np.ndarray, vc: np.ndarray, n_head: int, slot: int, n_past: int,
                            computed_exp: bool = True):
        q, k, v = (np.ascontiguousarray(x, np.float32) for x in (q, k, v))
        kc, vc = np.array(kc, np.uint16, order="C"), np.array(vc, np.uint16, order="C")
        R, E = q.shape
        S, C, _ = kc.shape
        out = np.zeros_like(q)
        rc = self.library.minigpt4_amd_test_attn_draft(int(mode), n_head, E // n_head, C, S, slot, n_past, R, int(computed_exp), q.ctypes.data_as(FLOAT_PTR), k.ctypes.data_as(FLOAT_PTR),
                                                       v.ctypes.data_as(FLOAT_PTR), kc.ctypes.data_as(VOID_PTR), vc.ctypes.data_as(VOID_PTR), out.ctypes.data_as(FLOAT_PTR))
        if rc:
            raise RuntimeError(f"test_attn_draft rc={rc}: " + self.library.minigpt4_amd_last_error().decode("utf-8", errors="replace"))
        return out, kc, vc

    def amd_test_ngram_draft(self, history: Sequence[int], ngram_max: int, ngram_min: int, n_draft: int) -> List[int]:
        h = np.ascontiguousarray(history, np.int32)
        out = np.zeros(max(int(n_draft), 1), np.int32)
        n = self.library.minigpt4_amd_test_ngram_draft(h.ctypes.data_as(INT_PTR) if len(h) else None, len(h), int(ngram_max), int(ngram_min), int(n_draft), out.ctypes.data_as(INT_PTR))
        if n < 0:
            raise ValueError("test_ngram_draft: bad arguments")
        return [int(x) for x in out[:n]]

    def amd_batch_path(self, ctx) -> dict:
        out = (ctypes.c_int32 * 8)()
        if self.library.minigpt4_amd_batch_path(ctx.ptr, out):
            raise RuntimeError("minigpt4_amd_batch_path failed")
        return dict(zip(("rows", "ri", "ri_mix", "ri_ksplit", "dot4", "dot4_mix", "mul_mat", "sets"), [int(x) for x in out]))

    def amd_encode_images(self, ctx, images: Sequence[np.ndarray]) -> List[np.ndarray]:
        arrs = [np.ascontiguousarray(i, dtype=np.float32) for i in images]
        structs = (MiniGPT4Image * len(arrs))(*[array_to_image_struct(a) for a in arrs])
        batch, out = MiniGPT4Images(structs, len(arrs)), MiniGPT4Embeddings()
        self.panic_if_error(self.library.minigpt4_amd_encode_images(ctx.ptr, ctypes.byref(batch), ctypes.byref(out), 0))
        try:
            return [np.ctypeslib.as_array(out.embeddings[i].data, shape=(out.embeddings[i].n_embeddings,)).copy().reshape(32, -1) for i in range(out.n_embeddings)]
        finally:
            self.library.minigpt4_amd_free_embeddings(ctypes.byref(out))

    def amd_decode_image(self, data: bytes) -> MiniGPT4Image:
        image = MiniGPT4Image()
        self.panic_if_error(self.library.minigpt4_amd_decode_image(data, len(data), ctypes.pointer(image)))
        return image

    def amd_eval_tokens(self, ctx, tokens: Sequence[int]):
        t = np.ascontiguousarray(tokens, np.int32)
        self.panic_if_error(self.library.minigpt4_amd_eval_tokens(ctx.ptr, t.ctypes.data_as(INT_PTR), len(t)))

    def amd_eval_embd(self, ctx, embd: np.ndarray):
        e = np.ascontiguousarray(embd, np.float32)
        n_embd = self.library.minigpt4_amd_n_embd(ctx.ptr)
        self.panic_if_error(self.library.minigpt4_amd_eval_embd(ctx.ptr, e.ctypes.data_as(FLOAT_PTR), e.size // n_embd))

    def amd_logits(self, ctx) -> np.ndarray:
        out = np.empty(self.library.minigpt4_amd_n_vocab(ctx.ptr), np.float32)
        assert self.library.minigpt4_amd_get_logits(ctx.ptr, out.ctypes.data_as(FLOAT_PTR), out.size) == 0
        return out

    def amd_tokenize(self, ctx, text: bytes, add_bos: bool = True) -> List[int]:
        cap = len(text) + 8
        out = (ctypes.c_int32 * cap)()
        n = self.library.minigpt4_amd_tokenize(ctx.ptr, text, int(add_bos), out, cap)
        return list(out[:n])

    def amd_decode_loop(self, ctx, steps: int):
        toks = np.zeros(steps, np.int32)
        ms = ctypes.c_float()
        rc = self.library.minigpt4_amd_decode_loop(ctx.ptr, steps, toks.ctypes.data_as(INT_PTR), ctypes.byref(ms))
        if rc:
            raise RuntimeError("decode_loop failed: " + self.library.minigpt4_amd_last_error().decode())
        return toks, float(ms.value)

    def amd_profile_sites(self, ctx, steps: int) -> dict:
        import json as _json
        buf = ctypes.create_string_buffer(1 << 16)
        rc = self.library.minigpt4_amd_profile_sites(ctx.ptr, steps, buf, len(buf))
        if rc:
            raise RuntimeError("profile_sites failed")
        return _json.loads(buf.value.decode())

    def amd_test_mul_mat(self, ggml_type: int, raw_w: np.ndarray, n_in: int, n_out: int, x: np.ndarray, ref: bool = False) -> np.ndarray:
        x = np.ascontiguousarray(x, np.float32).reshape(-1, n_in)
        raw_w = np.ascontiguousarray(raw_w)
        y = np.empty((x.shape[0], n_out), np.float32)
        fn = self.library.minigpt4_amd_test_mul_mat_ref if ref else self.library.minigpt4_amd_test_mul_mat
        rc = fn(ggml_type, raw_w.ctypes.data_as(VOID_PTR), n_in, n_out, x.ctypes.data_as(FLOAT_PTR), x.shape[0],
                                                    y.ctypes.data_as(FLOAT_PTR))
        if rc:
            raise RuntimeError(f"test_mul_mat rc={rc}: " + self.library.minigpt4_amd_last_error().decode())
        return y

    def amd_test_mmq2(self, ggml_type: int, raw_w: np.ndarray, n_mat: int, n_in: int, n_out: int, x: np.ndarray, residual: Optional[np.ndarray] = None, ks: int = 0,
                      generation: int = 2) -> np.ndarray:
        x = np.ascontiguousarray(x, np.float32).reshape(-1, n_in)
        raw_w = np.ascontiguousarray(raw_w)
        N = x.shape[0]
        y = np.empty((n_mat, N, n_out), np.float32)
        r = np.ascontiguousarray(residual, np.float32) if residual is not None else None
        rc = self.library.minigpt4_amd_test_mmq2(ggml_type, raw_w.ctypes.data_as(VOID_PTR), n_mat, n_in, n_out, x.ctypes.data_as(FLOAT_PTR), N,
                                                 r.ctypes.data_as(FLOAT_PTR) if r is not None else None, ks, generation, y.ctypes.data_as(FLOAT_PTR))
        if rc:
            raise RuntimeError(f"amd_test_mmq2 failed ({rc}): " + self.library.minigpt4_amd_last_error().decode())
        return y

    def amd_test_matvec(self, type1: int, raw1: np.ndarray, n1: int, n_in: int, n_out: int, x: np.ndarray, x2: Optional[np.ndarray] = None, prep: int = 2,
                        fuse: bool = False, epi: int = 0, residual: Optional[np.ndarray] = None, type2: int = 0, raw2: Optional[np.ndarray] = None,
                        silu_table: Optional[np.ndarray] = None, computed: bool = False) -> np.ndarray:
        x = np.ascontiguousarray(x, np.float32).reshape(n_in)
        x2c = None if x2 is None else np.ascontiguousarray(x2, np.float32).reshape(n_in)
        raw1 = np.ascontiguousarray(raw1)
        n2 = 0 if raw2 is None else 1
        raw2c = None if raw2 is None else np.ascontiguousarray(raw2)
        res = None if residual is None else np.ascontiguousarray(residual, np.float32).reshape(-1)
        y = np.empty(((1 if epi == 1 else n1 + n2), n_out), np.float32)
        args = [type1, raw1.ctypes.data_as(VOID_PTR), n1, type2, None if raw2c is None else raw2c.ctypes.data_as(VOID_PTR), n2,
                n_in, n_out, x.ctypes.data_as(FLOAT_PTR), None if x2c is None else x2c.ctypes.data_as(FLOAT_PTR), prep, int(fuse), epi,
                None if res is None else res.ctypes.data_as(FLOAT_PTR)]
        if computed or silu_table is not None:
            tab = None if computed else self._table_arg(silu_table)
            rc = self.library.minigpt4_amd_test_matvec_ex(*args, None if tab is None else tab.ctypes.data_as(VOID_PTR), y.ctypes.data_as(FLOAT_PTR))
        else:
            rc = self.library.minigpt4_amd_test_matvec(*args, y.ctypes.data_as(FLOAT_PTR))
        if rc:
            raise RuntimeError(f"test_matvec rc={rc}: " + self.library.minigpt4_amd_last_error().decode())
        return y

    def amd_test_matvec_rows(self, ggml_type: int, raw_w: np.ndarray, n_mat: int, n_in: int, n_out: int, x: np.ndarray, residual: Optional[np.ndarray] = None) -> np.ndarray:
        x = np.ascontiguousarray(x, np.float32).reshape(-1, n_in)
        raw_w = np.ascontiguousarray(raw_w)
        res = None if residual is None else np.ascontiguousarray(residual, np.float32)
        y = np.empty((n_mat, x.shape[0], n_out), np.float32)
        rc = self.library.minigpt4_amd_test_matvec_rows(ggml_type, raw_w.ctypes.data_as(VOID_PTR), n_mat, n_in, n_out, x.ctypes.data_as(FLOAT_PTR), x.shape[0],
                                                        None if res is None else res.ctypes.data_as(FLOAT_PTR), y.ctypes.data_as(FLOAT_PTR))
        if rc:
            raise RuntimeError(f"test_matvec_rows rc={rc}: " + self.library.minigpt4_amd_last_error().decode())
        return y

    def amd_test_matvec_ri(self, ggml_type: int, raw_w: np.ndarray, n_mat: int, n_in: int, n_out: int, x: np.ndarray, residual: Optional[np.ndarray] = None,
                           rms_w: Optional[np.ndarray] = None) -> np.ndarray:
        x = np.ascontiguousarray(x, np.float32).reshape(-1, n_in)
        raw_w = np.ascontiguousarray(raw_w)
        res = None if residual is None else np.ascontiguousarray(residual, np.float32)
        y = np.empty((n_mat, x.shape[0], n_out), np.float32)
        f = self.library.minigpt4_amd_test_matvec_ri
        f.argtypes = [I32, VOID_PTR, I32, ctypes.c_int64, ctypes.c_int64, FLOAT_PTR, I32, FLOAT_PTR, FLOAT_PTR, FLOAT_PTR]
        w = None if rms_w is None else np.ascontiguousarray(rms_w, np.float32)
        rc = f(ggml_type, raw_w.ctypes.data_as(VOID_PTR), n_mat, n_in, n_out, x.ctypes.data_as(FLOAT_PTR), x.shape[0], None if res is None else res.ctypes.data_as(FLOAT_PTR),
               None if w is None else w.ctypes.data_as(FLOAT_PTR), y.ctypes.data_as(FLOAT_PTR))
        if rc:
            raise RuntimeError(f"test_matvec_ri rc={rc}: " + self.library.minigpt4_amd_last_error().decode())
        return y

    def amd_test_matvec_ri_mixed(self, type_a: int, raw_a: np.ndarray, n_a: int, type_b: int, raw_b: np.ndarray, n_b: int, n_in: int, n_out: int, x: np.ndarray) -> np.ndarray:
        x = np.ascontiguousarray(x, np.float32).reshape(-1, n_in)
        raw_a, raw_b = np.ascontiguousarray(raw_a), np.ascontiguousarray(raw_b)
        y = np.empty((n_a + n_b, x.shape[0], n_out), np.float32)
        f = self.library.minigpt4_amd_test_matvec_ri_mixed
        f.argtypes = [I32, VOID_PTR, I32, I32, VOID_PTR, I32, ctypes.c_int64, ctypes.c_int64, FLOAT_PTR, I32, FLOAT_PTR]
        rc = f(type_a, raw_a.ctypes.data_as(VOID_PTR), n_a, type_b, raw_b.ctypes.data_as(VOID_PTR), n_b, n_in, n_out, x.ctypes.data_as(FLOAT_PTR), x.shape[0], y.ctypes.data_as(FLOAT_PTR))
        if rc:
            raise RuntimeError(f"test_matvec_ri_mixed rc={rc}: " + self.library.minigpt4_amd_last_error().decode())
        return y

    def amd_test_quantize(self, x: np.ndarray, rms_w: Optional[np.ndarray] = None):
        x = np.ascontiguousarray(x, np.float32)
        N, K = x.shape
        q8k, dk, bs = np.empty((N, K), np.int8), np.empty((N, K // 256), np.float32), np.empty((N, K // 16), np.int16)
        q80, d0 = np.empty((N, K), np.int8), np.empty((N, K // 32), np.float32)
# ... 256 lines not shown
```

Measured before the change: 344.1 tokens/s.

## Split decode attention across workgroups per head along the value dimension

Adds a third grid dimension to the fused decode attention kernels so that each head is served by up to four workgroups. Every workgroup recomputes the full QK scores and softmax, but accumulates and writes only its slice of the V output. Only workgroup zero writes the new K/V cache entries. By default the split factor is chosen from the head count and CU count, so that a 40-head, batch-1 decode fills more of the 256 CUs. The cost is redundant K reads and score work per head. The long-context split threshold is also raised slightly.

```diff
diff --git a/minigpt4.cpp_amd/csrc/attn_llm_body.hpp b/minigpt4.cpp_amd/csrc/attn_llm_body.hpp
--- a/minigpt4.cpp_amd/csrc/attn_llm_body.hpp
+++ b/minigpt4.cpp_amd/csrc/attn_llm_body.hpp
@@ -3,6 +3,8 @@
     constexpr int CH = HD / 8, P = AT_THREADS / CH, RM = DRAFT ? DRAFT_ROWS : 1;
     static_assert(!DRAFT || (RM <= P && RM * (HD / 2) <= AT_THREADS), "one prologue thread per (row, rotated pair); at most one LDS key per partition");
     const int h = blockIdx.x, t = blockIdx.y, tid = threadIdx.x;
+    constexpr bool VSP = LV != 0;
+    const int lvs = VSP ? __builtin_ctz(gridDim.z) : 0, z = VSP ? (int)blockIdx.z : 0;
     int pos_, p0_ = 0;
     if (BATCHED) {
         const int slot = row_slot[DRAFT ? 0 : t];
@@ -34,7 +36,7 @@
                 if (r == t) {
                     st_h2(qh + 2 * i, rope_rot_h2(q[qo + 2 * i], q[qo + 2 * i + 1], c, s));
                     const size_t co = (size_t)pos * E + (size_t)h * HD + 2 * i;
-                    st_h2(kc + co, kr); st_h2(vc + co, vr);
+                    if (!VSP || z == 0) { st_h2(kc + co, kr); st_h2(vc + co, vr); }
                 }
             }
         } else if (tid < HD / 2) {
@@ -44,7 +46,7 @@
             const __half2 vr = __floats2half2_rn(vin[qo + 2 * i], vin[qo + 2 * i + 1]);
             st_h2(qh + 2 * i, qr); st_h2(knew + 2 * i, kr); st_h2(vnew + 2 * i, vr);
             const size_t co = (size_t)pos * E + (size_t)h * HD + 2 * i;
-            st_h2(kc + co, kr); st_h2(vc + co, vr);
+            if (!VSP || z == 0) { st_h2(kc + co, kr); st_h2(vc + co, vr); }
         }
     } else {
         for (int i = tid; i < HD; i += AT_THREADS) qh[i] = f2h_rn(q[qo + i]);
@@ -70,11 +72,13 @@
     const __half *kb = kc + (size_t)h * HD + 8 * c, *vb = vc + (size_t)h * HD + 8 * c;
     constexpr int NPRE = 16;
     const int gmax = DRAFT ? max(p0 - 1, 0) : 0;
+    const bool own = !VSP || ((c << lvs) / CH == z);
+    const __half *vbo = own ? vb : vc + (size_t)h * HD + 8 * (z * (CH >> lvs));
     int4 kpre[NPRE], vpre[NPRE];
 #pragma unroll
     for (int i = 0; i < NPRE; i++) kpre[i] = ld16(kb + (size_t)min(p + i * P, DRAFT ? gmax : max(Tg - 1, 0)) * E);
 #pragma unroll
-    for (int i = 0; i < NPRE; i++) vpre[i] = ld16(vb + (size_t)min(p + i * P, DRAFT ? gmax : max(Tg - 1, 0)) * E);
+    for (int i = 0; i < NPRE; i++) vpre[i] = ld16(vbo + (size_t)min(own ? p + i * P : p, DRAFT ? gmax : max(Tg - 1, 0)) * E);
     int jl = -1;
     int4 kl = make_int4(0, 0, 0, 0), vl = kl;
     if (DRAFT) {
@@ -119,7 +123,7 @@
     for (int j0 = p + NPRE * P; j0 < Tg; j0 += 8 * P) {
         int4 vv[8];
 #pragma unroll
-        for (int i = 0; i < 8; i++) vv[i] = ld16(vb + (size_t)min(j0 + i * P, DRAFT ? gmax : Tg - 1) * E);
+        for (int i = 0; i < 8; i++) vv[i] = ld16(vbo + (size_t)min(own ? j0 + i * P : p, DRAFT ? gmax : Tg - 1) * E);
 #pragma unroll
         for (int i = 0; i < 8; i++) { const int j = j0 + i * P; if (j < Tg) pv_key(DRAFT && j == jl ? vl : vv[i], j); }
     }
@@ -129,9 +133,9 @@
         for (int e = 0; e < 8; e++) o[e] = fmaf(__half2float(vnew[(DRAFT ? t : 0) * HD + 8 * c + e]), pj, o[e]);
     }
 #pragma unroll
-    for (int e = 0; e < 8; e++) part[p * HD + 8 * c + e] = o[e];
+    for (int e = 0; e < 8; e++) if (own) part[p * HD + 8 * c + e] = o[e];
     __syncthreads();
-    for (int i = tid; i < HD; i += AT_THREADS) { float s = 0.0f;
+    for (int i = (z * HD >> lvs) + tid; i < ((z + 1) * HD >> lvs); i += AT_THREADS) { float s = 0.0f;
 #pragma unroll 8
         for (int pp = 0; pp < P; pp++) s += part[pp * HD + i];
         out[qo + i] = s; }
diff --git a/minigpt4.cpp_amd/csrc/engine.cpp b/minigpt4.cpp_amd/csrc/engine.cpp
--- a/minigpt4.cpp_amd/csrc/engine.cpp
+++ b/minigpt4.cpp_amd/csrc/engine.cpp
@@ -124,6 +124,7 @@
     batch_mix_ = !(getenv("MINIGPT4_BATCH_MIX") && atoi(getenv("MINIGPT4_BATCH_MIX")) == 0);
     if (const char *e = getenv("MINIGPT4_ATTN_SPLIT_T")) attn_split_t_ = atoi(e);
     n_cus_ = prop.multiProcessorCount;
+    if (const char *e = getenv("MINIGPT4_ATTN_VSPLIT")) attn_vsplit_ = atoi(e);
     if (const char *e = getenv("MINIGPT4_MMQH")) set_mmqh(atoi(e));
     if (const char *e = getenv("MINIGPT4_COMPUTED_TABLES")) computed_tables_ = atoi(e) != 0;
     if (const char *e = getenv("MINIGPT4_RI_FUSE")) ri_fuse_ = atoi(e) != 0;
@@ -283,6 +284,11 @@
     const int E = (int)llm_.n_embd, L = (int)llm_.n_layer, V = (int)llm_.n_vocab, F = (int)llm_.n_ff();
     const int hd = E / (int)llm_.n_head;
     if (!attn_head_size_supported(hd)) { set_last_error("unsupported head size (supported: 32, 64, 128)"); return E_LoadLanguageModel; }
+    if (attn_vsplit_ && attn_vsplit_choice((int)llm_.n_head, 1, hd, n_cus_, attn_vsplit_) != attn_vsplit_) {
+        set_last_error("MINIGPT4_ATTN_VSPLIT=" + std::to_string(attn_vsplit_) + ": not a power of two that divides the head size / 8 (" + std::to_string(hd / 8) + ")");
+        MG4_ERR("%s", last_error().c_str());
+        return E_LoadLanguageModel;
+    }
     if (parity_) attn_ref_prepare();
     auto ctx_too_long = [&](const char *which, int lim) {
         set_last_error(std::string(which) + "n_ctx " + std::to_string(n_ctx_) + " exceeds what the attention kernel's LDS score rows hold (" + std::to_string(lim) + ")");
@@ -844,7 +850,7 @@
         std::optional<SiteScope> att_sc;
         if (prof_on_) att_sc.emplace(this, "attention", 4.0 * (double)E * (sg ? sg->key_rows : (double)(conv_[sl].n_committed + N)), s);
         if (dec && p.split) launch_attn_llm_split(q_, k_, v_, kc, vc, H, hd, d_npast, n_ctx_, cos_, sin_, tabs_dec_, att_, attn_ws_, attn_splits_, s);
-        else if (dec) launch_attn_llm(q_, k_, v_, kc, vc, 1, H, hd, d_npast, n_ctx_, cos_, sin_, tabs_dec_, att_, true, s);
+        else if (dec) launch_attn_llm(q_, k_, v_, kc, vc, 1, H, hd, d_npast, n_ctx_, cos_, sin_, tabs_dec_, att_, true, s, attn_form(1));
         else {
             if (pend_.ks > 1 && pend_.n == 3 && pend_.y[0] == q_ && pend_.y[1] == k_ && pend_.y[2] == v_ && !pend_.res[0] && !pend_.res[1] && !pend_.res[2] && pend_.stride == (long long)N * E) {
                 if (sg) launch_rope_kv_seg_slabs(pend_, N, H, hd, sg->rows, seq_stride, cos_, sin_, kc, vc, s);
@@ -961,8 +967,8 @@
         return same_shape(Ws.begin(), (int)Ws.size()) && matvec_rows_prologue_ok(w0->type, w0->cols);
     };
     auto attn = [&](__half *kc, __half *vc) {
-        if (verify) launch_attn_llm_draft(q_, k_, v_, kc, vc, B, H, hd, d_npast_, d_bslot_, seq_stride, n_ctx_, cos_, sin_, tabs_dec_, att_, s);
-        else launch_attn_llm_batched(q_, k_, v_, kc, vc, B, H, hd, d_npast_, d_bslot_, seq_stride, n_ctx_, cos_, sin_, tabs_dec_, att_, s);
+        if (verify) launch_attn_llm_draft(q_, k_, v_, kc, vc, B, H, hd, d_npast_, d_bslot_, seq_stride, n_ctx_, cos_, sin_, tabs_dec_, att_, s, attn_form(B));
+        else launch_attn_llm_batched(q_, k_, v_, kc, vc, B, H, hd, d_npast_, d_bslot_, seq_stride, n_ctx_, cos_, sin_, tabs_dec_, att_, s, attn_form(B));
     };
     float *const row_logits = verify ? spec_logits_ : blogits_;
     launch_get_rows(tok_type_, tok_raw_, E, d_btok_, B, x_, s);
diff --git a/minigpt4.cpp_amd/csrc/engine.hpp b/minigpt4.cpp_amd/csrc/engine.hpp
--- a/minigpt4.cpp_amd/csrc/engine.hpp
+++ b/minigpt4.cpp_amd/csrc/engine.hpp
@@ -245,8 +245,10 @@
     int *h_argmax_ = nullptr, *h_bstage_ = nullptr; float *h_logits_ = nullptr; int logits_host_slot_ = -1;
     bool use_graph_ = true, use_v2_ = true, attn_prefill_ = true, parity_ = false;
     FILE *trace_file_ = nullptr;
-    void *attn_ws_ = nullptr; int attn_splits_ = 6; int attn_split_t_ = 768; int attn_splits_forced_ = 0;
+    void *attn_ws_ = nullptr; int attn_splits_ = 6; int attn_split_t_ = 816; int attn_splits_forced_ = 0;
     int batch_rows_max_ = 4; int batch_fuse_ = -1; int n_cus_ = 256;
+    int attn_vsplit_ = 0;
+    AttnForm attn_form(int rows) const { AttnForm f; f.vsplit = attn_vsplit_ ? attn_vsplit_ : std::max(1, attn_vsplit_choice((int)llm_.n_head, rows, (int)(llm_.n_embd / llm_.n_head), n_cus_, 0)); return f; }
     bool computed_tables_ = true;
     bool pair_silu_computed_ = true;
     bool computed_gelu_ = true;
diff --git a/minigpt4.cpp_amd/csrc/kernels.hpp b/minigpt4.cpp_amd/csrc/kernels.hpp
--- a/minigpt4.cpp_amd/csrc/kernels.hpp
+++ b/minigpt4.cpp_amd/csrc/kernels.hpp
@@ -94,19 +94,22 @@
 constexpr int KV_COPY_MAX_DST = 64;
 struct KvCopyDst { __half *k[KV_COPY_MAX_DST]; __half *v[KV_COPY_MAX_DST]; };
 void launch_kv_copy(const __half *src_k, const __half *src_v, int src_rows, const KvCopyDst &dst, int n_dst, int dst_rows, int n_layer, int E, int n_rows, hipStream_t s);
-void launch_attn_llm(float *q, const float *k, const float *v, __half *kcache, __half *vcache, int N, int n_head, int hd, const int *n_past, int n_ctx,
-                     const float *cos_tab, const float *sin_tab, const Tables &tb, float *out, bool fused, hipStream_t s);
+struct AttnForm { int vsplit = 1; };
+struct AttnLaunched { int grid_z = 1; int form = 0; };
+int attn_vsplit_choice(int n_head, int rows, int hd, int n_cus, int forced);
+AttnLaunched launch_attn_llm(float *q, const float *k, const float *v, __half *kcache, __half *vcache, int N, int n_head, int hd, const int *n_past, int n_ctx,
+                             const float *cos_tab, const float *sin_tab, const Tables &tb, float *out, bool fused, hipStream_t s, const AttnForm &form = {});
 size_t attn_split_workspace_bytes(int n_head, int hd, int n_ctx, int splits);
 int attn_split_count(int n_head, int cus);
 void launch_attn_llm_split(float *q, const float *k, const float *v, __half *kcache, __half *vcache, int n_head, int hd, const int *n_past, int n_ctx, const float *cos_tab,
                            const float *sin_tab, const Tables &tb, float *out, void *ws, int splits, hipStream_t s);
-void launch_attn_llm_batched(float *q, const float *k, const float *v, __half *kcache, __half *vcache, int B, int n_head, int hd, const int *n_past, const int *row_slot,
-                             size_t seq_stride, int n_ctx, const float *cos_tab, const float *sin_tab, const Tables &tb, float *out, hipStream_t s);
+AttnLaunched launch_attn_llm_batched(float *q, const float *k, const float *v, __half *kcache, __half *vcache, int B, int n_head, int hd, const int *n_past, const int *row_slot,
+                                     size_t seq_stride, int n_ctx, const float *cos_tab, const float *sin_tab, const Tables &tb, float *out, hipStream_t s, const AttnForm &form = {});
 void launch_batch_finish(const float *logits, int n_vocab, int B, const int *row_slot, int *n_past, int *argmax, int *feed, float *slot_logits, hipStream_t s);
 void launch_batch_begin(int *n_past, const int *row_slot, const int *row_pos, int B, hipStream_t s);
 constexpr int DRAFT_ROWS = 8;
-void launch_attn_llm_draft(float *q, const float *k, const float *v, __half *kcache, __half *vcache, int R, int n_head, int hd, const int *n_past, const int *row_slot,
-                           size_t seq_stride, int n_ctx, const float *cos_tab, const float *sin_tab, const Tables &tb, float *out, hipStream_t s);
+AttnLaunched launch_attn_llm_draft(float *q, const float *k, const float *v, __half *kcache, __half *vcache, int R, int n_head, int hd, const int *n_past, const int *row_slot,
+                                   size_t seq_stride, int n_ctx, const float *cos_tab, const float *sin_tab, const Tables &tb, float *out, hipStream_t s, const AttnForm &form = {});
 void launch_draft_begin(int *n_past, const int *row_slot, const int *row_pos, hipStream_t s);
 void launch_draft_finish(const float *logits, int n_vocab, int R, const int *tok, const int *row_slot, int *n_past, int *argmax, int *feed, float *slot_logits, int *res, hipStream_t s);
 void launch_rope_kv_seg(float *q, const float *k, const float *v, int N, int n_head, int hd, const int *rows, size_t seq_stride, const float *cos_tab, const float *sin_tab,
diff --git a/minigpt4.cpp_amd/csrc/llm_kernels.hip b/minigpt4.cpp_amd/csrc/llm_kernels.hip
--- a/minigpt4.cpp_amd/csrc/llm_kernels.hip
+++ b/minigpt4.cpp_amd/csrc/llm_kernels.hip
@@ -1609,6 +1609,7 @@
                                                          size_t seq_stride = 0) {
     constexpr bool DRAFT = false;
     constexpr int n_ctx = 0;
+    constexpr int LV = 0;
 #include "attn_llm_body.hpp"
 }
 template <int HD>
@@ -1617,7 +1618,36 @@
                                                                const float *__restrict__ sin_tab, const Tables tb, float *__restrict__ out, const int *__restrict__ row_slot,
                                                                size_t seq_stride) {
     constexpr bool FUSED = true, BATCHED = true, DRAFT = true;
+    constexpr int LV = 0;
 #include "attn_llm_body.hpp"
+}
+template <int HD, bool BATCHED, int LV>
+__global__ __launch_bounds__(AT_THREADS) void k_attn_llm_f(float *__restrict__ q, const float *__restrict__ kin, const float *__restrict__ vin, __half *__restrict__ kc,
+                                                           __half *__restrict__ vc, int E, const int *__restrict__ n_past, const float *__restrict__ cos_tab,
+                                                           const float *__restrict__ sin_tab, const Tables tb, float *__restrict__ out, const int *__restrict__ row_slot,
+                                                           size_t seq_stride) {
+    static_assert(LV != 0, "LV == 0 is k_attn_llm");
+    constexpr bool FUSED = true, DRAFT = false;
+    constexpr int n_ctx = 0;
+#include "attn_llm_body.hpp"
+}
+template <int HD, int LV>
+__global__ __launch_bounds__(AT_THREADS) void k_attn_llm_draft_f(float *__restrict__ q, const float *__restrict__ kin, const float *__restrict__ vin, __half *__restrict__ kc,
+                                                                 __half *__restrict__ vc, int E, const int *__restrict__ n_past, int n_ctx, const float *__restrict__ cos_tab,
+                                                                 const float *__restrict__ sin_tab, const Tables tb, float *__restrict__ out,
+                                                                 const int *__restrict__ row_slot, size_t seq_stride) {
+    static_assert(LV != 0, "LV == 0 is k_attn_llm_draft");
+    constexpr bool FUSED = true, BATCHED = true, DRAFT = true;
+#include "attn_llm_body.hpp"
+}
+constexpr int ATTN_VSPLIT_MAX = 4;
+int attn_vsplit_choice(int n_head, int rows, int hd, int n_cus, int forced) {
+    if (!attn_head_size_supported(hd) || n_head < 1 || rows < 1 || n_cus < 1 || forced < 0) return -1;
+    const int ch = hd / 8;
+    if (forced) return ((forced & (forced - 1)) == 0 && ch % forced == 0) ? forced : -1;
+    int vs = 1;
+    while (2 * vs <= ATTN_VSPLIT_MAX && ch % (2 * vs) == 0 && (long long)n_head * rows * 2 * vs <= n_cus) vs *= 2;
+    return vs;
 }
 
 template <class F> static bool attn_for_head_size(int hd, F &&f) {
@@ -1631,42 +1661,61 @@
 template <class F> static void attn_for_head_size_or_throw(int hd, F &&f) {
     if (!attn_for_head_size(hd, f)) throw HipError{hipErrorInvalidValue, "unsupported head size", __FILE__, __LINE__};
 }
+template <class K> static void attn_optin_once(K kern) { static bool done = false; if (!done) { HIP_IGNORE(lds_optin_max(kern)); done = true; } }
 template <int HD, bool BATCHED, bool DRAFT>
-static void launch_attn_body(bool fused, float *q, const float *k, const float *v, __half *kc, __half *vc, int rows, int n_head, const int *n_past, const int *row_slot,
-                             size_t seq_stride, int n_ctx, const float *cos_tab, const float *sin_tab, const Tables &tb, float *out, hipStream_t s) {
+static AttnLaunched launch_attn_body(bool fused, float *q, const float *k, const float *v, __half *kc, __half *vc, int rows, int n_head, const int *n_past, const int *row_slot,
+                                     size_t seq_stride, int n_ctx, const float *cos_tab, const float *sin_tab, const Tables &tb, float *out, const AttnForm &form, hipStream_t s) {
     const size_t lds = attn_lds_bytes(n_ctx, HD, DRAFT ? DRAFT_ROWS : 1);
-    const dim3 grid((unsigned)n_head, (unsigned)rows);
-    static bool attr = false;
+    const int vs = fused ? form.vsplit : 1, lv = vs > 1 ? 1 : 0;
+    if (attn_vsplit_choice(n_head, rows, HD, 1 << 30, vs) != vs) throw HipError{hipErrorInvalidValue, "decode attention: workgroups per head must be a power of two dividing hd / 8", __FILE__, __LINE__};
+    const dim3 grid((unsigned)n_head, (unsigned)rows, (unsigned)vs);
     if constexpr (DRAFT) {
+        if (lv) { auto kern = &k_attn_llm_draft_f<HD, 1>; attn_optin_once(kern); note_kernel("k_attn_llm_draft_f<%d, 1>", HD);
+                  hipLaunchKernelGGL(kern, grid, dim3(AT_THREADS), lds, s, q, k, v, kc, vc, n_head * HD, n_past, n_ctx, cos_tab, sin_tab, tb, out, row_slot, seq_stride);
+                  return {vs, lv}; }
+        static bool attr = false;
         if (!attr) { HIP_IGNORE(lds_optin_max(&k_attn_llm_draft<HD>)); attr = true; }
         note_kernel("k_attn_llm_draft<%d>", HD);
         hipLaunchKernelGGL((k_attn_llm_draft<HD>), grid, dim3(AT_THREADS), lds, s, q, k, v, kc, vc, n_head * HD, n_past, n_ctx, cos_tab, sin_tab, tb, out, row_slot, seq_stride);
-    } else if constexpr (BATCHED) {
-        if (!attr) { HIP_IGNORE(lds_optin_max(&k_attn_llm<HD, true, true>)); attr = true; }
-        hipLaunchKernelGGL((k_attn_llm<HD, true, true>), grid, dim3(AT_THREADS), lds, s, q, k, v, kc, vc, n_head * HD, n_past, cos_tab, sin_tab, tb, out, row_slot, seq_stride);
     } else {
-        if (!attr) { HIP_IGNORE(lds_optin_max(&k_attn_llm<HD, true>));
-                     HIP_IGNORE(lds_optin_max(&k_attn_llm<HD, false>)); attr = true; }
-        note_kernel("k_attn_llm<%d, %s, false>", HD, fused ? "true" : "false");
-        hipLaunchKernelGGL((fused ? k_attn_llm<HD, true> : k_attn_llm<HD, false>), grid, dim3(AT_THREADS), lds, s, q, k, v, kc, vc, n_head * HD, n_past, cos_tab, sin_tab, tb, out,
-                           row_slot, seq_stride);
-    }
-}
-void launch_attn_llm(float *q, const float *k, const float *v, __half *kcache, __half *vcache, int N, int n_head, int hd, const int *n_past, int n_ctx,
-                     const float *cos_tab, const float *sin_tab, const Tables &tb, float *out, bool fused, hipStream_t s) {
+        if (lv) { auto kern = &k_attn_llm_f<HD, BATCHED, 1>; attn_optin_once(kern); note_kernel("k_attn_llm_f<%d, %s, 1>", HD, BATCHED ? "true" : "false");
+                  hipLaunchKernelGGL(kern, grid, dim3(AT_THREADS), lds, s, q, k, v, kc, vc, n_head * HD, n_past, cos_tab, sin_tab, tb, out, row_slot, seq_stride);
+                  return {vs, lv}; }
+        static bool attr = false;
+        if constexpr (BATCHED) {
+            if (!attr) { HIP_IGNORE(lds_optin_max(&k_attn_llm<HD, true, true>)); attr = true; }
+            hipLaunchKernelGGL((k_attn_llm<HD, true, true>), grid, dim3(AT_THREADS), lds, s, q, k, v, kc, vc, n_head * HD, n_past, cos_tab, sin_tab, tb, out, row_slot, seq_stride);
+        } else {
+            if (!attr) { HIP_IGNORE(lds_optin_max(&k_attn_llm<HD, true>));
+                         HIP_IGNORE(lds_optin_max(&k_attn_llm<HD, false>)); attr = true; }
+            note_kernel("k_attn_llm<%d, %s, false>", HD, fused ? "true" : "false");
+            hipLaunchKernelGGL((fused ? k_attn_llm<HD, true> : k_attn_llm<HD, false>), grid, dim3(AT_THREADS), lds, s, q, k, v, kc, vc, n_head * HD, n_past, cos_tab, sin_tab, tb, out,
+                               row_slot, seq_stride);
+        }
+    }
+    return {1, 0};
+}
+AttnLaunched launch_attn_llm(float *q, const float *k, const float *v, __half *kcache, __half *vcache, int N, int n_head, int hd, const int *n_past, int n_ctx,
+                             const float *cos_tab, const float *sin_tab, const Tables &tb, float *out, bool fused, hipStream_t s, const AttnForm &form) {
+    AttnLaunched l;
     attn_for_head_size_or_throw(hd, [&](auto tag) {
-        launch_attn_body<decltype(tag)::value, false, false>(fused, q, k, v, kcache, vcache, fused ? 1 : N, n_head, n_past, nullptr, 0, n_ctx, cos_tab, sin_tab, tb, out, s); });
-}
-void launch_attn_llm_batched(float *q, const float *k, const float *v, __half *kcache, __half *vcache, int B, int n_head, int hd, const int *n_past, const int *row_slot,
-                             size_t seq_stride, int n_ctx, const float *cos_tab, const float *sin_tab, const Tables &tb, float *out, hipStream_t s) {
+        l = launch_attn_body<decltype(tag)::value, false, false>(fused, q, k, v, kcache, vcache, fused ? 1 : N, n_head, n_past, nullptr, 0, n_ctx, cos_tab, sin_tab, tb, out, form, s); });
+    return l;
+}
+AttnLaunched launch_attn_llm_batched(float *q, const float *k, const float *v, __half *kcache, __half *vcache, int B, int n_head, int hd, const int *n_past, const int *row_slot,
+                                     size_t seq_stride, int n_ctx, const float *cos_tab, const float *sin_tab, const Tables &tb, float *out, hipStream_t s, const AttnForm &form) {
+    AttnLaunched l;
     attn_for_head_size_or_throw(hd, [&](auto tag) {
-        launch_attn_body<decltype(tag)::value, true, false>(true, q, k, v, kcache, vcache, B, n_head, n_past, row_slot, seq_stride, n_ctx, cos_tab, sin_tab, tb, out, s); });
-}
-void launch_attn_llm_draft(float *q, const float *k, const float *v, __half *kcache, __half *vcache, int R, int n_head, int hd, const int *n_past, const int *row_slot,
-                           size_t seq_stride, int n_ctx, const float *cos_tab, const float *sin_tab, const Tables &tb, float *out, hipStream_t s) {
+        l = launch_attn_body<decltype(tag)::value, true, false>(true, q, k, v, kcache, vcache, B, n_head, n_past, row_slot, seq_stride, n_ctx, cos_tab, sin_tab, tb, out, form, s); });
+    return l;
+}
+AttnLaunched launch_attn_llm_draft(float *q, const float *k, const float *v, __half *kcache, __half *vcache, int R, int n_head, int hd, const int *n_past, const int *row_slot,
+                                   size_t seq_stride, int n_ctx, const float *cos_tab, const float *sin_tab, const Tables &tb, float *out, hipStream_t s, const AttnForm &form) {
     if (R < 1 || R > DRAFT_ROWS) throw HipError{hipErrorInvalidValue, "launch_attn_llm_draft: row count out of range", __FILE__, __LINE__};
+    AttnLaunched l;
     attn_for_head_size_or_throw(hd, [&](auto tag) {
-        launch_attn_body<decltype(tag)::value, true, true>(true, q, k, v, kcache, vcache, R, n_head, n_past, row_slot, seq_stride, n_ctx, cos_tab, sin_tab, tb, out, s); });
+        l = launch_attn_body<decltype(tag)::value, true, true>(true, q, k, v, kcache, vcache, R, n_head, n_past, row_slot, seq_stride, n_ctx, cos_tab, sin_tab, tb, out, form, s); });
+    return l;
 }
 constexpr int AS_THREADS = 256;
 template <int HD>
diff --git a/minigpt4.cpp_amd/minigpt4_library.py b/minigpt4.cpp_amd/minigpt4_library.py
--- a/minigpt4.cpp_amd/minigpt4_library.py
+++ b/minigpt4.cpp_amd/minigpt4_library.py
@@ -240,6 +240,8 @@
         L.minigpt4_amd_test_penalise_host.argtypes = [FLOAT_PTR, I32, INT_PTR, I32, I32, I32, F32, F32, F32, I32, INT_PTR, FLOAT_PTR, I32, INT_PTR, I32, INT_PTR]
         L.minigpt4_amd_test_pen_pick.argtypes = [FLOAT_PTR, I32, I32, I32, INT_PTR, I32, INT_PTR, I32, INT_PTR, FLOAT_PTR, FLOAT_PTR]
         L.minigpt4_amd_test_attn_draft.argtypes = [I32, I32, I32, I32, I32, I32, I32, I32, I32, FLOAT_PTR, FLOAT_PTR, FLOAT_PTR, VOID_PTR, VOID_PTR, FLOAT_PTR]
+        L.minigpt4_amd_test_attn_decode.argtypes = [I32, I32, I32, I32, I32, I32, INT_PTR, INT_PTR, I32, I32, FLOAT_PTR, FLOAT_PTR, FLOAT_PTR, VOID_PTR, VOID_PTR, FLOAT_PTR, INT_PTR]
+        L.minigpt4_amd_test_attn_vsplit.argtypes = [I32, I32, I32, I32, I32]
         L.minigpt4_amd_test_ngram_draft.argtypes = [INT_PTR, I32, I32, I32, I32, INT_PTR]
         L.minigpt4_amd_test_attn_prefill_seg.argtypes = [I32, I32, I32, I32, VOID_PTR, VOID_PTR, I32, INT_PTR, FLOAT_PTR, I32, FLOAT_PTR, FLOAT_PTR, INT_PTR, VOID_PTR, VOID_PTR, INT_PTR]
         L.minigpt4_amd_test_rope_kv_seg.argtypes = [I32, I32, I32, I32, I32, INT_PTR, FLOAT_PTR, FLOAT_PTR, FLOAT_PTR, I32, FLOAT_PTR, VOID_PTR, VOID_PTR, FLOAT_PTR, VOID_PTR, VOID_PTR]
@@ -687,6 +689,25 @@
             raise RuntimeError(f"test_attn_draft rc={rc}: " + self.library.minigpt4_amd_last_error().decode("utf-8", errors="replace"))
         return out, kc, vc
 
+    def amd_test_attn_decode(self, kind: int, q: np.ndarray, k: np.ndarray, v: np.ndarray, kc: np.ndarray, vc: np.ndarray, n_head: int, row_slot: Sequence[int],
+                             n_past: Sequence[int], vsplit: int = 1, computed_exp: bool = True):
+        q, k, v = (np.ascontiguousarray(x, np.float32) for x in (q, k, v))
+        kc, vc = np.array(kc, np.uint16, order="C"), np.array(vc, np.uint16, order="C")
+        rows, E = q.shape
+        S, C, _ = kc.shape
+        rs, npast = np.ascontiguousarray(row_slot, np.int32), np.ascontiguousarray(n_past, np.int32)
+        assert npast.shape == (S,) and rs.ndim == 1 and rs.size >= 1
+        out, launched = np.zeros_like(q), np.zeros(2, np.int32)
+        rc = self.library.minigpt4_amd_test_attn_decode(int(kind), n_head, E // n_head, C, S, rows, rs.ctypes.data_as(INT_PTR), npast.ctypes.data_as(INT_PTR), int(vsplit),
+                                                        int(computed_exp), q.ctypes.data_as(FLOAT_PTR), k.ctypes.data_as(FLOAT_PTR), v.ctypes.data_as(FLOAT_PTR),
+                                                        kc.ctypes.data_as(VOID_PTR), vc.ctypes.data_as(VOID_PTR), out.ctypes.data_as(FLOAT_PTR), launched.ctypes.data_as(INT_PTR))
+        if rc:
+            raise RuntimeError(f"test_attn_decode rc={rc}: " + self.library.minigpt4_amd_last_error().decode("utf-8", errors="replace"))
+        return out, kc, vc, (int(launched[0]), int(launched[1]))
+
+    def amd_test_attn_vsplit(self, n_head: int, rows: int, hd: int, n_cus: int, forced: int = 0) -> int:
+        return int(self.library.minigpt4_amd_test_attn_vsplit(n_head, rows, hd, n_cus, forced))
+
     def amd_test_ngram_draft(self, history: Sequence[int], ngram_max: int, ngram_min: int, n_draft: int) -> List[int]:
         h = np.ascontiguousarray(history, np.int32)
         out = np.zeros(max(int(n_draft), 1), np.int32)
```

Result: no change. 346.7 tokens/s (median of 6 runs) (+0.8%).
